# li199603/easy_gaussian_splatting

Measured on AMD Instinct MI355X. Metric: train iters/sec + forward render fps, 1M Gaussians @ 1080p, higher is better.
Workload: dtype f32

## Files before the change

easy_gaussian_splatting_amd/csrc/gs_binning.hip:

```cpp

#include "gs_common.h"

namespace gs {

#define GS_BIN_PER_GROUP 4096
#define GS_BIN_MAX_GROUPS 256
constexpr int kBinThreads = 1024;
constexpr int kCoopTiles = 32;

BinLayout bin_layout(int C, int64_t N, int tiles) {
    BinLayout L;
    int64_t g = (N + GS_BIN_PER_GROUP - 1) / GS_BIN_PER_GROUP;
    if (g < 1) g = 1;
    if (g > GS_BIN_MAX_GROUPS) g = GS_BIN_MAX_GROUPS;
    L.groups = (int)g;
    L.per_group = (N + g - 1) / g;
    auto align = [](size_t x) { return (x + 255) & ~(size_t)255; };
    size_t off = 0;
    L.hist_off = off; off = align(off + sizeof(uint32_t) * (size_t)C * L.groups * tiles);
    L.tile_cnt_off = off; off = align(off + sizeof(uint32_t) * (size_t)C * tiles);
    L.grp_tot_off = off; off = align(off + sizeof(uint32_t) * (size_t)C * L.groups);
    L.grp_base_off = off; off = align(off + sizeof(uint32_t) * (size_t)C * L.groups);
    L.items_off = off; off = align(off + sizeof(int32_t) * (64 + (size_t)10 * (size_t)C * tiles));
    L.total = off;
    return L;
}

__device__ __forceinline__ void unpack_bbox(uint4 b, int& x0, int& x1, int& y0, int& y1) {
    x0 = b.x & 0xffff; x1 = b.x >> 16; y0 = b.y & 0xffff; y1 = b.y >> 16;
}

__global__ __launch_bounds__(kBinThreads) void bin_hist_kernel(int64_t N, int tw, int tiles,
                                                               int64_t per_group,
                                                               const uint4* __restrict__ bbox,
                                                               uint32_t* __restrict__ hist_mat,
                                                               uint32_t* __restrict__ grp_tot, const int64_t* __restrict__ rblk, int phase) {
    extern __shared__ __attribute__((aligned(16))) uint32_t lds[];
    if (round_idle(rblk, phase)) return;
    uint32_t* hist = lds;
    uint32_t* scratch = lds + tiles;
    const int grp = blockIdx.x, c = blockIdx.y, G = gridDim.x;
    for (int t = threadIdx.x; t < tiles; t += blockDim.x) hist[t] = 0;
    __syncthreads();
    const int64_t g0 = grp * per_group, g1 = min(N, g0 + per_group);
    uint32_t local = 0;
    for (int64_t base = g0; base < g1; base += blockDim.x) {
        const int64_t n = base + threadIdx.x;
        int x0 = 0, x1 = 0, y0 = 0, y1 = 0;
        uint4 fp = make_uint4(0u, 0u, 0u, 0u);
        if (n < g1) { fp = bbox[(int64_t)c * N + n]; unpack_bbox(fp, x0, x1, y0, y1); }
        const int w = x1 - x0, rect = w * (y1 - y0), cnt = (int)fp.w;
        const float inv_w = 1.0f / (float)max(w, 1);
        local += cnt;
        if (rect <= kCoopTiles)
            for (uint32_t mb = fp.z; mb; mb &= mb - 1) {
                const int i = __ffs((int)mb) - 1, yy = div_by_width(i, inv_w);
                atomicAdd(&hist[(y0 + yy) * tw + x0 + (i - yy * w)], 1u);
            }
        unsigned long long big = __ballot(rect > kCoopTiles);
        while (big) {
            const int src = __ffsll((long long)big) - 1;
            big &= big - 1;
            const int bx0 = __shfl(x0, src, 64), by0 = __shfl(y0, src, 64), bw = __shfl(w, src, 64),
                      bcnt = __shfl(cnt, src, 64);
            const float binv = __shfl(inv_w, src, 64);
            for (int i = lane_id(); i < bcnt; i += 64) {
                const int yy = div_by_width(i, binv);
                atomicAdd(&hist[(by0 + yy) * tw + bx0 + (i - yy * bw)], 1u);
            }
        }
    }
    __syncthreads();
    uint32_t* out = hist_mat + ((size_t)c * G + grp) * tiles;
    for (int t = threadIdx.x; t < tiles; t += blockDim.x) out[t] = hist[t];
    uint32_t wsum = wave_reduce_add(local);
    if (lane_id() == 0) scratch[threadIdx.x >> 6] = wsum;
    __syncthreads();
    if (threadIdx.x == 0) {
        uint32_t s = 0;
        for (int i = 0; i < (int)(blockDim.x >> 6); ++i) s += scratch[i];
        grp_tot[c * G + grp] = s;
    }
}

constexpr int kColTiles = GS_BIN_MAX_GROUPS > 256 ? 32 : 64, kColChunks = GS_BIN_MAX_GROUPS > 256 ? 32 : 16;
__global__ __launch_bounds__(kColTiles * kColChunks) void bin_colscan_kernel(int C, int G, int tiles, uint32_t* __restrict__ hist_mat,
                                                                              uint32_t* __restrict__ tile_cnt) {
    __shared__ uint32_t part[kColChunks][kColTiles + 1];
    const int tl = threadIdx.x % kColTiles, ch = threadIdx.x / kColTiles;
    const int64_t i = (int64_t)blockIdx.x * kColTiles + tl;
    const bool in = i < (int64_t)C * tiles;
    const int c = in ? (int)(i / tiles) : 0, t = in ? (int)(i % tiles) : 0;
    const int per = (G + kColChunks - 1) / kColChunks;
    const int g0 = ch * per, g1 = min(G, g0 + per);
    uint32_t* col = hist_mat + (size_t)c * G * tiles + t;
    constexpr int kMax = 16;
    uint32_t v[kMax];
    uint32_t sum = 0;
#pragma unroll
    for (int k = 0; k < kMax; ++k) {
        v[k] = (in && g0 + k < g1) ? col[(size_t)(g0 + k) * tiles] : 0u;
        sum += v[k];
    }
    uint32_t extra = 0;
    for (int g = g0 + kMax; in && g < g1; ++g) extra += col[(size_t)g * tiles];
    part[ch][tl] = sum + extra;
    __syncthreads();
    uint32_t run = 0, total = 0;
#pragma unroll
    for (int k = 0; k < kColChunks; ++k) {
        const uint32_t p = part[k][tl];
        run += k < ch ? p : 0u;
        total += p;
    }
    if (in) {
#pragma unroll
        for (int k = 0; k < kMax; ++k) {
            if (g0 + k < g1) col[(size_t)(g0 + k) * tiles] = run;
            run += v[k];
        }
        for (int g = g0 + kMax; g < g1; ++g) { const uint32_t x = col[(size_t)g * tiles]; col[(size_t)g * tiles] = run; run += x; }
        if (ch == 0) tile_cnt[i] = total;
    }
}

constexpr int kScanItems = 16;
__global__ __launch_bounds__(kBinThreads) void bin_tilescan_kernel(
    int n_tiles_total, int n_groups_total, const uint32_t* __restrict__ tile_cnt,
    const uint32_t* __restrict__ grp_tot, int32_t* __restrict__ isect_offsets,
    int32_t* __restrict__ bucket_offsets, uint32_t* __restrict__ grp_base,
    int64_t* __restrict__ info, int32_t* __restrict__ tile_order, int64_t cap_isects, int64_t cap_tile,
    int64_t keep_mask, int32_t* __restrict__ sort_counts, int64_t* __restrict__ info_mirror, int per_call,
    int64_t* __restrict__ rblk, int phase) {
    __shared__ unsigned long long scratch[17];
    const int chunk = kBinThreads * kScanItems;
    if (round_idle(rblk, phase)) return;
    if (blockIdx.x == 2) {
        if (sort_counts && threadIdx.x < 64) sort_counts[threadIdx.x] = 0;
        unsigned long long gcarry = 0;
        for (int base = 0; base < n_groups_total; base += kBinThreads) {
            const int i = base + threadIdx.x;
            unsigned long long v = i < n_groups_total ? grp_tot[i] : 0ull, total;
            unsigned long long ex = block_excl_scan_add(v, scratch, &total);
            if (i < n_groups_total) grp_base[i] = (uint32_t)(gcarry + ex);
            gcarry += total;
        }
        return;
    }
    if (blockIdx.x == 1) {
        if (!tile_order) return;
        if (n_tiles_total > chunk) {
            for (int i = threadIdx.x; i < n_tiles_total; i += kBinThreads) tile_order[i] = i;
            return;
        }
        constexpr int kW = kBinThreads / 64;
        __shared__ uint32_t cls_cnt[64][kW + 1];
        auto cls_of = [](uint32_t x) -> int {
            if (x < 2u) return 0;
            const int lg = 31 - __clz((int)x);
            return min(63, (lg << 2) | (int)((x << (31 - lg)) >> 29 & 3u));
        };
        const int wv = threadIdx.x >> 6;
        const int first = threadIdx.x * kScanItems;
        uint32_t v[kScanItems];
#pragma unroll
        for (int k = 0; k < kScanItems; ++k) v[k] = (first + k < n_tiles_total) ? tile_cnt[first + k] : 0u;
        for (int i = threadIdx.x; i < 64 * (kW + 1); i += kBinThreads) (&cls_cnt[0][0])[i] = 0u;
        __syncthreads();
#pragma unroll
        for (int k = 0; k < kScanItems; ++k)
            if (first + k < n_tiles_total) atomicAdd(&cls_cnt[cls_of(v[k])][wv], 1u);
        __syncthreads();
        if (threadIdx.x < 64) {
            const int c = 63 - (int)threadIdx.x;
            uint32_t n = 0, cw[kW];
#pragma unroll
            for (int w = 0; w < kW; ++w) { cw[w] = cls_cnt[c][w]; n += cw[w]; }
            uint32_t run = wave_incl_scan_add(n) - n;
#pragma unroll
            for (int w = 0; w < kW; ++w) { cls_cnt[c][w] = run; run += cw[w]; }
        }
        __syncthreads();
#pragma unroll
        for (int k = 0; k < kScanItems; ++k)
            if (first + k < n_tiles_total) tile_order[atomicAdd(&cls_cnt[cls_of(v[k])][wv], 1u)] = first + k;
        return;
    }
    unsigned long long carry_i = phase == 2 ? (unsigned long long)rblk[GS_ROUND_BASE] : 0ull, carry_b = 0;
    uint32_t max_cnt = 0;
    for (int base = 0; base < n_tiles_total; base += chunk) {
        const int first = base + threadIdx.x * kScanItems;
        uint32_t v[kScanItems];
        unsigned long long si = 0, sb = 0;
#pragma unroll
        for (int k = 0; k < kScanItems; ++k) {
            v[k] = (first + k < n_tiles_total) ? tile_cnt[first + k] : 0u;
            si += v[k];
            sb += (v[k] + GS_BUCKET - 1) / GS_BUCKET;
            max_cnt = max(max_cnt, v[k]);
        }
        unsigned long long packed = si | (sb << 36), total;
        unsigned long long ex = block_excl_scan_add(packed, scratch, &total);
        unsigned long long ri = carry_i + (ex & ((1ull << 36) - 1)), rb = carry_b + (ex >> 36);
#pragma unroll
        for (int k = 0; k < kScanItems; ++k) {
            if (first + k < n_tiles_total) {
                isect_offsets[first + k] = (int32_t)ri;
                bucket_offsets[first + k] = (int32_t)rb;
            }
            ri += v[k];
            rb += (v[k] + GS_BUCKET - 1) / GS_BUCKET;
        }
        carry_i += total & ((1ull << 36) - 1);
        carry_b += total >> 36;
    }
    uint32_t m = max_cnt;
#pragma unroll
    for (int d = 32; d > 0; d >>= 1) m = max(m, (uint32_t)__shfl_xor((int)m, d, 64));
    __shared__ uint32_t smax[16];
    if (lane_id() == 0) smax[threadIdx.x >> 6] = m;
    __syncthreads();
    if (threadIdx.x == 0) {
        uint32_t mm = 0;
        for (int i = 0; i < kBinThreads / 64; ++i) mm = max(mm, smax[i]);
        isect_offsets[n_tiles_total] = (int32_t)carry_i;
        bucket_offsets[n_tiles_total] = (int32_t)carry_b;
        if (phase == 1) rblk[GS_ROUND_BASE] = (int64_t)carry_i;
        if (phase != 0) {
            info[7] = rblk[GS_ROUND_LISTED_ALL];
            info[6] = phase == 2 ? rblk[GS_ROUND_LIVE] : 0;
        }
        if (phase == 2) mm = max(mm, (uint32_t)info[2]);
        info[0] = (int64_t)carry_i; info[1] = (int64_t)carry_b; info[2] = (int64_t)mm;
        if (cap_isects > 0) {
            const int64_t f = ((int64_t)carry_i > cap_isects ? 1 : 0) | ((int64_t)mm > cap_tile ? 2 : 0);
            if (per_call && phase != 2) info[3] = (info[3] & keep_mask) | f;
            else if (f) info[3] |= f;
        } else {
            info[3] = keep_mask ? (info[3] & keep_mask) : 0;
        }
        if (info_mirror) {
#pragma unroll
            for (int i = 0; i < 8; ++i) info_mirror[i] = info[i];
            __threadfence_system();
        }
    }
}

__global__ __launch_bounds__(kBinThreads) void bin_emit_kernel(
    int64_t N, int tw, int tiles, int64_t per_group, const uint4* __restrict__ bbox,
    const float* __restrict__ depths, const uint32_t* __restrict__ hist_mat,
    const int32_t* __restrict__ isect_offsets, const uint32_t* __restrict__ grp_base,
    unsigned long long* __restrict__ keys, int32_t* __restrict__ slot_gid,
    int32_t* __restrict__ cum_tiles, const int64_t* __restrict__ guard, const int64_t* __restrict__ rblk, int phase) {
    extern __shared__ __attribute__((aligned(16))) uint32_t lds[];
    if (guard_tripped(guard) || round_idle(rblk, phase)) return;
    uint32_t* cursor = lds;
    uint32_t* scratch = lds + tiles;
    const int grp = blockIdx.x, c = blockIdx.y, G = gridDim.x;
    const uint32_t* mine = hist_mat + ((size_t)c * G + grp) * tiles;
    const int32_t* toff = isect_offsets + (size_t)c * tiles;
    for (int t0 = 0; t0 < tiles; t0 += 8 * (int)blockDim.x) {
        uint32_t v[8];
#pragma unroll
        for (int k = 0; k < 8; ++k) {
            const int t = t0 + k * (int)blockDim.x + (int)threadIdx.x;
            v[k] = t < tiles ? mine[t] + (uint32_t)toff[t] : 0u;
        }
#pragma unroll
        for (int k = 0; k < 8; ++k) {
            const int t = t0 + k * (int)blockDim.x + (int)threadIdx.x;
            if (t < tiles) cursor[t] = v[k];
        }
    }
    __syncthreads();
    uint32_t running = grp_base[c * G + grp] + (phase == 2 ? (uint32_t)rblk[GS_ROUND_BASE] : 0u);
    const int64_t g0 = grp * per_group, g1 = min(N, g0 + per_group);
    uint4 fp_next = make_uint4(0u, 0u, 0u, 0u);
    float d_next = 0.f;
    if (g0 + threadIdx.x < g1) { fp_next = bbox[(int64_t)c * N + g0 + threadIdx.x]; d_next = depths[(int64_t)c * N + g0 + threadIdx.x]; }
    for (int64_t base = g0; base < g1; base += blockDim.x) {
        const int64_t n = base + threadIdx.x;
        const int64_t f = (int64_t)c * N + n;
        int x0 = 0, x1 = 0, y0 = 0, y1 = 0;
        const uint4 fp = fp_next;
        const float dcur = d_next;
        if (n < g1) unpack_bbox(fp, x0, x1, y0, y1);
        const int w = x1 - x0, rect = w * (y1 - y0), cnt = (int)fp.w;
        const float inv_w = 1.0f / (float)max(w, 1);
        uint32_t total;
        const uint32_t slot0 = running + block_excl_scan_add((uint32_t)cnt, scratch, &total);
        running += total;
        fp_next = make_uint4(0u, 0u, 0u, 0u);
        if (n + blockDim.x < g1) { fp_next = bbox[f + blockDim.x]; d_next = depths[f + blockDim.x]; }
        if (n < g1 && (phase != 2 || cnt > 0)) cum_tiles[f] = (int32_t)slot0;
        const uint32_t dbits = cnt > 0 ? __float_as_uint(dcur) : 0u;
        if (rect <= kCoopTiles) {
            uint32_t k = 0;
            for (uint32_t mb = fp.z; mb; mb &= mb - 1, ++k) {
                const int i = __ffs((int)mb) - 1, yy = div_by_width(i, inv_w);
                const uint32_t pos = atomicAdd(&cursor[(y0 + yy) * tw + x0 + (i - yy * w)], 1u);
                keys[pos] = ((unsigned long long)dbits << 32) | (slot_gid ? slot0 + k : (uint32_t)f);
                if (slot_gid) slot_gid[slot0 + k] = (int32_t)f;
            }
        }
        unsigned long long big = __ballot(rect > kCoopTiles);
        while (big) {
            const int src = __ffsll((long long)big) - 1;
            big &= big - 1;
            const int bx0 = __shfl(x0, src, 64), by0 = __shfl(y0, src, 64), bw = __shfl(w, src, 64),
                      bcnt = __shfl(cnt, src, 64);
            const uint32_t bslot = __shfl((int)slot0, src, 64), bd = __shfl((int)dbits, src, 64);
            const int32_t bf = (int32_t)(c * N + base) + (src + (threadIdx.x & ~63));
            const float binv = __shfl(inv_w, src, 64);
            for (int i = lane_id(); i < bcnt; i += 64) {
                const int yy = div_by_width(i, binv);
                const uint32_t pos = atomicAdd(&cursor[(by0 + yy) * tw + bx0 + (i - yy * bw)], 1u);
                keys[pos] = ((unsigned long long)bd << 32) | (slot_gid ? bslot + i : (uint32_t)bf);
                if (slot_gid) slot_gid[bslot + i] = bf;
            }
        }
    }
}

template <typename KeyPtr>
__device__ __forceinline__ void bitonic_sort_keys(KeyPtr key, int n, int P) {
    for (int k = 2; k <= P; k <<= 1) {
        const int half = k >> 1;
        for (int idx = threadIdx.x; idx < (P >> 1); idx += blockDim.x) {
            const int blk = idx / half, off = idx - blk * half;
            const int a = blk * k + off, b = blk * k + k - 1 - off;
            if (b < n) {
                const unsigned long long ka = key[a], kb = key[b];
                if (ka > kb) { key[a] = kb; key[b] = ka; }
            }
        }
        __syncthreads();
        for (int j = half >> 1; j > 0; j >>= 1) {
            for (int idx = threadIdx.x; idx < (P >> 1); idx += blockDim.x) {
                const int a = ((idx & ~(j - 1)) << 1) | (idx & (j - 1)), b = a + j;
                if (b < n) {
                    const unsigned long long ka = key[a], kb = key[b];
                    if (ka > kb) { key[a] = kb; key[b] = ka; }
                }
            }
            __syncthreads();
        }
    }
}

struct SortArgs {
    int tiles, tile_bits, lo_excl, hi_incl;
    const int32_t* isect_offsets;
    unsigned long long* keys;
    const int32_t* slot_gid;
    int64_t* isect_ids;
    int32_t* flatten_ids;
    int32_t* slots;
    const int64_t* guard;
    int coarse;
    int seg;
    unsigned long long* merged;
    const int64_t* rblk;
    int phase;
};
__device__ __forceinline__ bool sort_off(const SortArgs& a) { return guard_tripped(a.guard) || round_idle(a.rblk, a.phase); }

constexpr int kSegLen = 8192;
constexpr int kSegMax = 8;

template <bool IN_LDS>
__global__ void tile_sort_kernel(const SortArgs a) {
    extern __shared__ __attribute__((aligned(16))) unsigned long long skeys[];
    const int t = blockIdx.x;
    if (sort_off(a)) return;
    const int lo = a.isect_offsets[t], hi = a.isect_offsets[t + 1];
    const int n = hi - lo;
    if (n <= a.lo_excl || n > a.hi_incl) return;
    int P = 1;
    while (P < n) P <<= 1;
    unsigned long long* gk = a.keys + lo;
    if (IN_LDS) {
        for (int i = threadIdx.x; i < n; i += blockDim.x) skeys[i] = gk[i];
        __syncthreads();
        bitonic_sort_keys(skeys, n, P);
    } else {
        bitonic_sort_keys(gk, n, P);
    }
    if (a.coarse) {
        if (IN_LDS) for (int i = threadIdx.x; i < n; i += blockDim.x) gk[i] = skeys[i];
        return;
    }
    const int cam = t / a.tiles, tid = t - cam * a.tiles;
    const long long hi_bits = ((long long)cam << (32 + a.tile_bits)) | ((long long)tid << 32);
    for (int i = threadIdx.x; i < n; i += blockDim.x) {
        const unsigned long long k = IN_LDS ? skeys[i] : gk[i];
        const uint32_t slot = (uint32_t)k;
        if (a.slot_gid) { a.slots[lo + i] = (int32_t)slot; a.flatten_ids[lo + i] = a.slot_gid[slot]; }
        else a.flatten_ids[lo + i] = (int32_t)slot;
        if (a.isect_ids) a.isect_ids[lo + i] = hi_bits | (long long)(k >> 32);
    }
}

template <int T>
__device__ __forceinline__ void radix_sort_list(const SortArgs& a, const int vblock) {
    extern __shared__ __attribute__((aligned(16))) unsigned long long skeys[];
    constexpr int W = T / 64;
    const int tile = a.seg ? vblock / kSegMax : vblock;
    int lo = a.isect_offsets[tile], n = a.isect_offsets[tile + 1] - lo;
    if (n <= a.lo_excl || n > a.hi_incl) return;
    if (a.seg) {
        const int sg = vblock - tile * kSegMax;
        lo += sg * kSegLen;
        n = min(kSegLen, n - sg * kSegLen);
        if (n <= 0) return;
    }
    const int cap = a.seg ? kSegLen : a.hi_incl;
    unsigned long long* src = skeys;
    unsigned long long* dst = skeys + cap;
    uint32_t* cnt = reinterpret_cast<uint32_t*>(skeys + 2 * cap);
    uint32_t* nxt = cnt + W * 256;
    __shared__ int s_flag;
    const int tid = threadIdx.x, lane = tid & 63, wave = tid >> 6;
    const unsigned long long* gk = a.keys + lo;
    const int per_wave = ((n + W * 64 - 1) / (W * 64)) * 64;
    const int w_lo = min(n, wave * per_wave), w_hi = min(n, w_lo + per_wave);
    const float inv_pw64 = 1.0f / (float)(per_wave >> 6);
    auto owner = [inv_pw64](int pos) { return (int)(((float)(pos >> 6) + 0.5f) * inv_pw64); };
    const unsigned long long lt_mask = (1ull << lane) - 1ull;
    for (int i = tid; i < 2 * W * 256; i += T) cnt[i] = 0u;
    __syncthreads();
    for (int i = tid; i < n; i += T) {
        const unsigned long long k = gk[i];
        src[i] = k;
        atomicAdd(&cnt[owner(i) * 256 + (int)((k >> 32) & 255ull)], 1u);
    }
    for (int pass = 0; pass < 4; ++pass) {
        const int shift = 32 + 8 * pass;
        __syncthreads();
        if (wave == 0) {
            uint32_t c[4][W], tot[4], mine = 0;
            bool all_in_one = false;
#pragma unroll
            for (int q = 0; q < 4; ++q) {
                tot[q] = 0;
#pragma unroll
                for (int w = 0; w < W; ++w) { c[q][w] = cnt[w * 256 + 4 * lane + q]; tot[q] += c[q][w]; }
                all_in_one |= (int)tot[q] == n;
                mine += tot[q];
            }
            uint32_t run = wave_incl_scan_add(mine) - mine;
#pragma unroll
            for (int q = 0; q < 4; ++q)
#pragma unroll
                for (int w = 0; w < W; ++w) { cnt[w * 256 + 4 * lane + q] = run; run += c[q][w]; }
            const bool skip = __any(all_in_one);
            if (lane == 0) s_flag = skip ? 1 : 0;
        } else {
            for (int i = tid - 64; i < W * 256; i += T - 64) nxt[i] = 0u;
        }
        __syncthreads();
        const bool skip = s_flag != 0;
        const int nshift = shift + 8;
        if (skip) {
            if (pass < 3)
                for (int i = w_lo + lane; i < w_hi; i += 64) atomicAdd(&nxt[wave * 256 + (int)((src[i] >> nshift) & 255ull)], 1u);
        } else {
            for (int base = w_lo; base < w_hi; base += 64) {
                const int i = base + lane;
                const bool valid = i < w_hi;
                const unsigned long long k = valid ? src[i] : 0ull;
                const int d = (int)((k >> shift) & 255ull);
                uint32_t mlo = 0u, mhi = 0u;
#pragma unroll
                for (int b = 0; b < 8; ++b) {
                    const int e = __builtin_amdgcn_sbfe(d, b, 1);
                    const unsigned long long bm = __ballot(e != 0);
                    mlo |= (uint32_t)bm ^ (uint32_t)e;
                    mhi |= (uint32_t)(bm >> 32) ^ (uint32_t)e;
                }
                const unsigned long long peers = __ballot(valid) & ~(((unsigned long long)mhi << 32) | (unsigned long long)mlo);
                if (valid) {
                    const int rank = __popcll(peers & lt_mask);
                    const uint32_t off = cnt[wave * 256 + d];
                    const uint32_t pos = off + (uint32_t)rank;
                    dst[pos] = k;
                    if (rank == 0) cnt[wave * 256 + d] = off + (uint32_t)__popcll(peers);
                    if (pass < 3) atomicAdd(&nxt[owner((int)pos) * 256 + (int)((k >> nshift) & 255ull)], 1u);
                }
            }
            unsigned long long* t = src; src = dst; dst = t;
        }
        uint32_t* tc = cnt; cnt = nxt; nxt = tc;
    }
    __syncthreads();
    if (tid == 0) s_flag = 0;
    __syncthreads();
    bool bad = false;
    for (int i = tid + 1; i < n; i += T) bad |= src[i] < src[i - 1];
    if (bad) s_flag = 1;
    __syncthreads();
    if (s_flag) {
        int P = 1;
        while (P < n) P <<= 1;
        bitonic_sort_keys(src, n, P);
    }
    if (a.coarse || a.seg) {
        unsigned long long* out = a.keys + lo;
        for (int i = tid; i < n; i += T) out[i] = src[i];
        return;
    }
    const int cam = tile / a.tiles, tix = tile - cam * a.tiles;
    const long long hi_bits = ((long long)cam << (32 + a.tile_bits)) | ((long long)tix << 32);
    for (int i = tid; i < n; i += T) {
        const unsigned long long k = src[i];
        const uint32_t slot = (uint32_t)k;
        if (a.slot_gid) { a.slots[lo + i] = (int32_t)slot; a.flatten_ids[lo + i] = a.slot_gid[slot]; }
        else a.flatten_ids[lo + i] = (int32_t)slot;
        if (a.isect_ids) a.isect_ids[lo + i] = hi_bits | (long long)(k >> 32);
    }
}

template <int T>
__global__ __launch_bounds__(T) void tile_radix_sort_kernel(const SortArgs a) {
    if (sort_off(a)) return;
    radix_sort_list<T>(a, blockIdx.x);
}

template <int T>
__global__ __launch_bounds__(T) void tile_radix_sort_items_kernel(const SortArgs a, const int32_t* __restrict__ items,
                                                                  const int32_t* __restrict__ n_items) {
    if (sort_off(a)) return;
    const int n = *n_items;
    for (int it = blockIdx.x; it < n; it += gridDim.x) {
        radix_sort_list<T>(a, items[it]);
        __syncthreads();
    }
}

__global__ __launch_bounds__(256) void class_items_kernel(int n_lists, const int32_t* __restrict__ offsets,
                                                          int32_t* __restrict__ items, int32_t* __restrict__ counts,
                                                          const int64_t* __restrict__ guard, const int64_t* __restrict__ rblk, int phase) {
    if (guard_tripped(guard) || round_idle(rblk, phase)) return;
    const int i = blockIdx.x * blockDim.x + threadIdx.x;
    if (i >= n_lists) return;
    const int n = offsets[i + 1] - offsets[i];
    if (n > 1024 && n <= 4096) items[atomicAdd(&counts[0], 1)] = i;
    else if (n > 4096 && n <= kSegLen) items[n_lists + atomicAdd(&counts[1], 1)] = i;
    else if (n > kSegLen && n <= kSegLen * kSegMax) {
        const int ns = (n + kSegLen - 1) / kSegLen;
        const int p = atomicAdd(&counts[2], ns);
        for (int sg = 0; sg < ns; ++sg) items[2 * n_lists + p + sg] = i * kSegMax + sg;
    }
}

static size_t sort_items_bytes(int64_t n_lists) {
    return sizeof(int32_t) * (64 + (size_t)(2 + kSegMax) * (size_t)n_lists);
}


struct BinsLayout {
    int groups, shift, bw, bh, nbins;
    int64_t per_group;
    size_t hist_off;
    size_t bin_cnt_off;
    size_t grp_tot_off;
    size_t grp_base_off;
    size_t coff_off;
    size_t choff_off;
    size_t tile_cnt_off;
    size_t chunk_bin_off;
    int chunk_shift;
    size_t rec_off;
    size_t staged_off;
    size_t cnt_ct_off;
    size_t items_off;
    int64_t max_chunks;
    size_t total;
};

static BinsLayout bins_layout(int C, int64_t N, int tw, int th, int bin_shift, int64_t coarse_cap) {
    BinsLayout L;
    int64_t g = (N + GS_BIN_PER_GROUP - 1) / GS_BIN_PER_GROUP;
    if (g < 1) g = 1;
    if (g > GS_BIN_MAX_GROUPS) g = GS_BIN_MAX_GROUPS;
    L.groups = (int)g;
    L.per_group = (N + g - 1) / g;
    const int64_t nb2 = (int64_t)((tw + 3) / 4) * ((th + 3) / 4);
    L.shift = bin_shift ? bin_shift : ((N / nb2 > 2500) ? 1 : 2);
    const int B = 1 << L.shift;
    L.bw = (tw + B - 1) / B; L.bh = (th + B - 1) / B; L.nbins = L.bw * L.bh;
    auto align = [](size_t x) { return (x + 255) & ~(size_t)255; };
    size_t off = 0;
    L.hist_off = off; off = align(off + sizeof(uint32_t) * (size_t)C * L.groups * L.nbins);
    L.bin_cnt_off = off; off = align(off + sizeof(uint32_t) * (size_t)C * L.nbins);
    L.grp_tot_off = off; off = align(off + sizeof(uint32_t) * (size_t)C * L.groups);
    L.grp_base_off = off; off = align(off + sizeof(uint32_t) * (size_t)C * L.groups);
    L.coff_off = off; off = align(off + sizeof(int32_t) * ((size_t)C * L.nbins + 1));
    L.choff_off = off; off = align(off + sizeof(int32_t) * ((size_t)C * L.nbins + 1));
    L.tile_cnt_off = off; off = align(off + sizeof(uint32_t) * (size_t)C * tw * th);
    L.chunk_shift = 10 + (L.shift - 1);
    L.max_chunks = (coarse_cap >> L.chunk_shift) + (int64_t)C * L.nbins;
    L.chunk_bin_off = off; off = align(off + sizeof(int4) * (size_t)L.max_chunks);
    L.rec_off = off; off = align(off + sizeof(uint4) * (size_t)C * (size_t)N);
    L.staged_off = off; off = align(off + sizeof(uint4) * (size_t)coarse_cap);
    L.cnt_ct_off = off; off = align(off + sizeof(uint32_t) * (size_t)L.max_chunks * B * B);
    L.items_off = off; off = align(off + sort_items_bytes((int64_t)C * L.nbins));
    L.total = off;
    return L;
}

__device__ __forceinline__ void coarse_rect(uint4 fp, int shift, int& cx0, int& cw, int& cy0, int& crect) {
    int x0, x1, y0, y1;
    unpack_bbox(fp, x0, x1, y0, y1);
    if (fp.w == 0u) { cx0 = cy0 = cw = crect = 0; return; }
    const int r = (1 << shift) - 1;
    cx0 = x0 >> shift; cy0 = y0 >> shift;
    cw = ((x1 + r) >> shift) - cx0;
    crect = cw * (((y1 + r) >> shift) - cy0);
}

__global__ __launch_bounds__(kBinThreads) void bins_hist_kernel(int64_t N, int shift, int bw, int nbins, int64_t per_group,
                                                                const uint4* __restrict__ bbox,
                                                                uint32_t* __restrict__ hist_mat,
                                                                uint32_t* __restrict__ grp_tot, const int64_t* __restrict__ rblk, int phase) {
    extern __shared__ __attribute__((aligned(16))) uint32_t lds[];
    if (round_idle(rblk, phase)) return;
    uint32_t* hist = lds;
    uint32_t* scratch = lds + nbins;
    const int grp = blockIdx.x, c = blockIdx.y, G = gridDim.x;
    for (int t = threadIdx.x; t < nbins; t += blockDim.x) hist[t] = 0;
    __syncthreads();
    const int64_t g0 = grp * per_group, g1 = min(N, g0 + per_group);
    uint32_t local = 0;
    for (int64_t base = g0; base < g1; base += blockDim.x) {
        const int64_t n = base + threadIdx.x;
        uint4 fp = make_uint4(0u, 0u, 0u, 0u);
        if (n < g1) fp = bbox[(int64_t)c * N + n];
        int cx0, cw, cy0, crect;
        coarse_rect(fp, shift, cx0, cw, cy0, crect);
        local += fp.w;
        if (crect <= kCoopTiles)
            for (int i = 0, xx = 0, row = cy0 * bw + cx0; i < crect; ++i) {
                atomicAdd(&hist[row + xx], 1u);
                if (++xx == cw) { xx = 0; row += bw; }
            }
        unsigned long long big = __ballot(crect > kCoopTiles);
        while (big) {
            const int src = __ffsll((long long)big) - 1;
            big &= big - 1;
            const int bx0 = __shfl(cx0, src, 64), by0 = __shfl(cy0, src, 64), bcw = __shfl(cw, src, 64), bcnt = __shfl(crect, src, 64);
            for (int i = lane_id(); i < bcnt; i += 64) {
                const int yy = i / bcw;
                atomicAdd(&hist[(by0 + yy) * bw + bx0 + (i - yy * bcw)], 1u);
            }
        }
    }
    __syncthreads();
    uint32_t* out = hist_mat + ((size_t)c * G + grp) * nbins;
    for (int t = threadIdx.x; t < nbins; t += blockDim.x) out[t] = hist[t];
    uint32_t wsum = wave_reduce_add(local);
    if (lane_id() == 0) scratch[threadIdx.x >> 6] = wsum;
    __syncthreads();
    if (threadIdx.x == 0) {
        uint32_t s = 0;
        for (int i = 0; i < (int)(blockDim.x >> 6); ++i) s += scratch[i];
        grp_tot[c * G + grp] = s;
    }
}

__global__ __launch_bounds__(256) void bins_colscan_kernel(int C, int G, int nbins, uint32_t* __restrict__ hist_mat,
                                                          uint32_t* __restrict__ bin_cnt) {
    const int64_t i = (int64_t)blockIdx.x * 4 + (threadIdx.x >> 6);
    if (i >= (int64_t)C * nbins) return;
    const int c = (int)(i / nbins), t = (int)(i % nbins), lane = lane_id();
    uint32_t* col = hist_mat + (size_t)c * G * nbins + t;
    uint32_t v[4];
#pragma unroll
    for (int k = 0; k < 4; ++k) { const int g = 64 * k + lane; v[k] = g < G ? col[(size_t)g * nbins] : 0u; }
    uint32_t carry = 0;
#pragma unroll
    for (int k = 0; k < 4; ++k) {
        const uint32_t incl = wave_incl_scan_add(v[k]);
        const int g = 64 * k + lane;
        if (g < G) col[(size_t)g * nbins] = carry + incl - v[k];
        carry += __shfl(incl, 63, 64);
    }
    if (lane == 0) bin_cnt[i] = carry;
}

__global__ __launch_bounds__(kBinThreads) void bins_scan_kernel(int n_bins_total, int n_groups_total,
                                                                const uint32_t* __restrict__ bin_cnt,
                                                                const uint32_t* __restrict__ grp_tot,
                                                                int32_t* __restrict__ coff, int32_t* __restrict__ choff,
                                                                int4* __restrict__ chunk_desc, int64_t max_chunks,
                                                                int chunk_shift, uint32_t* __restrict__ grp_base,
                                                                int64_t* __restrict__ info, int64_t coarse_cap, int64_t list_cap,
                                                                int guarded, int32_t* __restrict__ sort_counts,
                                                                const int64_t* __restrict__ rblk, int phase) {
    __shared__ unsigned long long scratch[17];
    __shared__ uint32_t smax[16];
    if (round_idle(rblk, phase)) return;
    if (blockIdx.x == 1) {
        if (threadIdx.x < 64) sort_counts[threadIdx.x] = 0;
        unsigned long long gcarry = 0;
        for (int base = 0; base < n_groups_total; base += kBinThreads) {
// ... 177 lines not shown
    }
    if (!WRITE) {
#pragma unroll
        for (int p = 0; p < PER; ++p) {
            const int e = p * T + (int)threadIdx.x;
            fp[p] = e < m ? a.rec[(uint32_t)key[p]] : make_uint4(0u, 0u, 0u, 0u);
        }
    }
#pragma unroll
    for (int p = 0; p < PER; ++p) {
        const int e = p * T + (int)threadIdx.x;
        if (e < m) {
            if (!WRITE) a.staged[base + e] = fp[p];
            if (WRITE) { s_cum[e] = fp[p].w; s_d[e] = (uint32_t)(key[p] >> 32); }
            fp[p].w = (uint32_t)key[p];
            s_box[e] = fp[p];
        }
    }
    __syncthreads();
    if (!tile_ok) return;
    const unsigned long long lt_mask = (1ull << lane) - 1ull;
    const long long hi_bits = ((long long)cam << (32 + a.tile_bits)) | ((long long)(ty * a.tw + tx) << 32);
    uint32_t count = 0;
    for (int j = 0; j < m; j += 64) {
        const int e = j + lane;
        bool hit = false;
        int k = 0;
        uint32_t f = 0;
        if (e < m) {
            const uint4 q = s_box[e];
            int x0, x1, y0, y1;
            unpack_bbox(q, x0, x1, y0, y1);
            f = q.w;
            if (tx >= x0 && tx < x1 && ty >= y0 && ty < y1) {
                const int w = x1 - x0, idx = (ty - y0) * w + (tx - x0);
                if (w * (y1 - y0) <= kCoopTiles) { hit = (q.z >> idx) & 1u; k = __popc(q.z & ((1u << idx) - 1u)); }
                else { hit = true; k = idx; }
            }
        }
        const unsigned long long bal = __ballot(hit);
        if (WRITE) {
            if (hit) {
                const int64_t pos = out + __popcll(bal & lt_mask);
                a.flatten_ids[pos] = (int32_t)f;
                if (a.isect_ids) a.isect_ids[pos] = hi_bits | (long long)s_d[e];
                if (a.slots) a.slots[pos] = (int32_t)(s_cum[e] + (uint32_t)k);
            }
            out += __popcll(bal);
        } else {
            count += (uint32_t)__popcll(bal);
        }
    }
    if (!WRITE && lane == 0) a.cnt_ct[(size_t)chunk * (B * B) + wave] = count;
}

template <int SHIFT>
__global__ __launch_bounds__(256) void bins_chunkscan_kernel(const RefineArgs a, int C) {
    constexpr int B = 1 << SHIFT;
    const int i = blockIdx.x * blockDim.x + threadIdx.x;
    if (i >= C * a.tiles) return;
    if (a.info[3] != 0 || round_idle(a.rblk, a.phase)) return;
    const int cam = i / a.tiles, t = i - cam * a.tiles;
    const int ty = t / a.tw, tx = t - ty * a.tw;
    const int bin = cam * a.nbins + (ty >> SHIFT) * a.bw + (tx >> SHIFT);
    const int w = ((ty & (B - 1)) << SHIFT) | (tx & (B - 1));
    const int c0 = a.choff[bin], c1 = a.choff[bin + 1];
    uint32_t run = 0;
    constexpr int kBatch = 8;
    for (int c = c0; c < c1; c += kBatch) {
        uint32_t v[kBatch];
#pragma unroll
        for (int k = 0; k < kBatch; ++k) v[k] = c + k < c1 ? a.cnt_ct[(size_t)(c + k) * (B * B) + w] : 0u;
#pragma unroll
        for (int k = 0; k < kBatch; ++k) {
            if (c + k < c1) a.cnt_ct[(size_t)(c + k) * (B * B) + w] = run;
            run += v[k];
        }
    }
    a.tile_cnt[i] = run;
}

__global__ __launch_bounds__(1024) void seg_merge_kernel(const SortArgs a, const int32_t* __restrict__ items,
                                                         const int32_t* __restrict__ n_items) {
    if (sort_off(a)) return;
    const int n_it = *n_items;
    for (int it = blockIdx.x; it < n_it; it += gridDim.x) {
    const int vblock = items[it];
    const int list = vblock / kSegMax, sg = vblock - list * kSegMax;
    const int lo = a.isect_offsets[list], n = a.isect_offsets[list + 1] - lo;
    const int s_lo = sg * kSegLen, s_n = min(kSegLen, n - s_lo);
    const int n_seg = (n + kSegLen - 1) / kSegLen;
    const unsigned long long* gk = a.keys + lo;
    const int cam = list / max(a.tiles, 1), tix = list - cam * a.tiles;
    const long long hi_bits = ((long long)cam << (32 + a.tile_bits)) | ((long long)tix << 32);
    for (int i = threadIdx.x; i < s_n; i += blockDim.x) {
        const unsigned long long k = gk[s_lo + i];
        int pos = i;
        for (int o = 0; o < n_seg; ++o) {
            if (o == sg) continue;
            const unsigned long long* seg = gk + o * kSegLen;
            int l = 0, r = min(kSegLen, n - o * kSegLen);
            while (l < r) {
                const int mid = (l + r) >> 1;
                if (seg[mid] < k) l = mid + 1; else r = mid;
            }
            pos += l;
        }
        if (a.coarse) {
            a.merged[lo + pos] = k;
        } else {
            const uint32_t slot = (uint32_t)k;
            if (a.slot_gid) { a.slots[lo + pos] = (int32_t)slot; a.flatten_ids[lo + pos] = a.slot_gid[slot]; }
            else a.flatten_ids[lo + pos] = (int32_t)slot;
            if (a.isect_ids) a.isect_ids[lo + pos] = hi_bits | (long long)(k >> 32);
        }
    }
    }
}

__global__ __launch_bounds__(1024) void seg_copy_kernel(const SortArgs a, const int32_t* __restrict__ items,
                                                        const int32_t* __restrict__ n_items) {
    if (sort_off(a)) return;
    const int n_it = *n_items;
    for (int it = blockIdx.x; it < n_it; it += gridDim.x) {
        const int vblock = items[it];
        const int list = vblock / kSegMax, sg = vblock - list * kSegMax;
        const int lo = a.isect_offsets[list], n = a.isect_offsets[list + 1] - lo;
        const int s_lo = sg * kSegLen, s_n = min(kSegLen, n - s_lo);
        for (int i = threadIdx.x; i < s_n; i += blockDim.x) a.keys[lo + s_lo + i] = a.merged[lo + s_lo + i];
    }
}

constexpr int kSortLarge = kSegLen * kSegMax;

}

using namespace gs;

extern "C" int gs_bin_groups(int64_t N) { return bin_layout(1, N, 1).groups; }

static int list_round(int64_t*& rblk) {
    const Rounds R = current_rounds();
    const int phase = (R.phase == 1 || R.phase == 4) ? 1 : (R.phase == 2 ? 2 : 0);
    rblk = phase ? R.blk : nullptr;
    return phase;
}

extern "C" size_t gs_bin_workspace_bytes(int C, int64_t N, int tile_w, int tile_h) {
    return bin_layout(C, N, tile_w * tile_h).total;
}

#define GS_SORT1K_THREADS 256
#define GS_SORT4K_THREADS 256
static int launch_list_sorts(hipStream_t st, SortArgs& a, unsigned grid, int64_t max_tile_count, int32_t* items_ws) {
    int lo_excl = 0;
    int32_t* counts = items_ws;
    int32_t* items = items_ws + 64;
    const size_t radix_lds = 2 * sizeof(uint32_t) * 256;
    a.lo_excl = 0; a.hi_incl = 1024;
    if (max_tile_count > 0) {
        const size_t lds_k = 2 * sizeof(uint64_t) * 1024 + radix_lds * (GS_SORT1K_THREADS / 64);
        hipLaunchKernelGGL(tile_radix_sort_kernel<GS_SORT1K_THREADS>, dim3(grid), dim3(GS_SORT1K_THREADS), lds_k, st, a);
        GS_LAUNCH_CHECK("tile_radix_sort_kernel");
    }
    if (max_tile_count <= 1024) return GS_OK;
    hipLaunchKernelGGL(class_items_kernel, dim3((grid + 255) / 256), dim3(256), 0, st, (int)grid, a.isect_offsets, items, counts, a.guard, a.rblk, a.phase);
    GS_LAUNCH_CHECK("class_items_kernel");
    {
        a.lo_excl = 1024; a.hi_incl = 4096;
        const size_t lds_k = 2 * sizeof(uint64_t) * 4096 + radix_lds * (GS_SORT4K_THREADS / 64);
        if (int rc = ensure_lds((const void*)tile_radix_sort_items_kernel<GS_SORT4K_THREADS>, lds_k)) return rc;
        hipLaunchKernelGGL(tile_radix_sort_items_kernel<GS_SORT4K_THREADS>, dim3(grid < 512u ? grid : 512u), dim3(GS_SORT4K_THREADS), lds_k, st, a,
                           (const int32_t*)items, (const int32_t*)counts);
        GS_LAUNCH_CHECK("tile_radix_sort_items_kernel<4096>");
    }
    if (max_tile_count > 4096) {
        a.lo_excl = 4096; a.hi_incl = kSegLen;
        const size_t lds_k = 2 * sizeof(uint64_t) * (size_t)kSegLen + radix_lds * (768 / 64);
        if (int rc = ensure_lds((const void*)tile_radix_sort_items_kernel<768>, lds_k)) return rc;
        hipLaunchKernelGGL(tile_radix_sort_items_kernel<768>, dim3(grid < 256u ? grid : 256u), dim3(768), lds_k, st, a,
                           (const int32_t*)(items + grid), (const int32_t*)(counts + 1));
        GS_LAUNCH_CHECK("tile_radix_sort_items_kernel<8192>");
    }
    if (max_tile_count > kSegLen) {
        a.lo_excl = kSegLen; a.hi_incl = kSortLarge; a.seg = 1;
        const size_t lds_k = 2 * sizeof(uint64_t) * (size_t)kSegLen + radix_lds * (768 / 64);
        if (int rc = ensure_lds((const void*)tile_radix_sort_items_kernel<768>, lds_k)) return rc;
        const int32_t* it = items + 2 * (size_t)grid;
        const int32_t* nit = counts + 2;
        hipLaunchKernelGGL(tile_radix_sort_items_kernel<768>, dim3(256), dim3(768), lds_k, st, a, it, nit);
        GS_LAUNCH_CHECK("tile_radix_sort_items_kernel<segments>");
        hipLaunchKernelGGL(seg_merge_kernel, dim3(512), dim3(1024), 0, st, a, it, nit);
        GS_LAUNCH_CHECK("seg_merge_kernel");
        if (a.coarse) {
            hipLaunchKernelGGL(seg_copy_kernel, dim3(512), dim3(1024), 0, st, a, it, nit);
            GS_LAUNCH_CHECK("seg_copy_kernel");
        }
        a.seg = 0;
    }
    if (max_tile_count > kSortLarge) {
        a.lo_excl = kSortLarge; a.hi_incl = 0x7fffffff;
        hipLaunchKernelGGL(tile_sort_kernel<false>, dim3(grid), dim3(1024), 0, st, a);
        GS_LAUNCH_CHECK("tile_sort_kernel<global>");
    }
    (void)lo_excl;
    return GS_OK;
}

extern "C" int gs_bin_count(void* stream, int C, int64_t N, int tile_w, int tile_h, const uint32_t* bbox,
                            void* workspace, size_t workspace_bytes, int32_t* isect_offsets,
                            int32_t* bucket_offsets, int32_t* tile_order, int64_t* info_dev, int64_t* info_host) {
    GS_REQUIRE(C >= 1 && N >= 0 && tile_w > 0 && tile_h > 0, "C>=1, N>=0, positive tile grid");
    const int tiles = tile_w * tile_h;
    GS_REQUIRE((size_t)tiles * 4 + 128 <= 160 * 1024, "tile grid too large for the LDS histogram (max 40928 tiles per camera)");
    GS_REQUIRE((int64_t)C * tiles < (1ll << 31), "too many tiles");
    const BinLayout L = bin_layout(C, N, tiles);
    GS_REQUIRE(workspace && workspace_bytes >= L.total, "workspace too small (see gs_bin_workspace_bytes)");
    GS_REQUIRE(isect_offsets && bucket_offsets && info_dev, "null output pointer");
    GS_REQUIRE(N == 0 || bbox, "null bbox");
    int64_t* rblk;
    const int phase = list_round(rblk);
    GS_REQUIRE(phase == 0 || C == 1, "depth rounds: one camera per call");
    hipStream_t st = (hipStream_t)stream;
    char* ws = (char*)workspace;
    uint32_t* hist = (uint32_t*)(ws + L.hist_off);
    uint32_t* tile_cnt = (uint32_t*)(ws + L.tile_cnt_off);
    uint32_t* grp_tot = (uint32_t*)(ws + L.grp_tot_off);
    uint32_t* grp_base = (uint32_t*)(ws + L.grp_base_off);
    const size_t lds = sizeof(uint32_t) * ((size_t)tiles + 32);
    if (int rc = ensure_lds((const void*)bin_hist_kernel, lds)) return rc;
    hipLaunchKernelGGL(bin_hist_kernel, dim3(L.groups, C), dim3(kBinThreads), lds, st, N, tile_w, tiles,
                       L.per_group, (const uint4*)bbox, hist, grp_tot, (const int64_t*)rblk, phase);
    GS_LAUNCH_CHECK("bin_hist_kernel");
    const int64_t ct = (int64_t)C * tiles;
    hipLaunchKernelGGL(bin_colscan_kernel, dim3((unsigned)((ct + kColTiles - 1) / kColTiles)), dim3(kColTiles * kColChunks), 0, st, C, L.groups,
                       tiles, hist, tile_cnt);
    GS_LAUNCH_CHECK("bin_colscan_kernel");
    const Guard gd = current_guard();
    GS_REQUIRE(gd.info == nullptr || gd.info == info_dev, "the guard set by gs_guard_set must be this call's info_dev");
    hipLaunchKernelGGL(bin_tilescan_kernel, dim3(3), dim3(kBinThreads), 0, st, (int)ct, C * L.groups, tile_cnt,
                       grp_tot, isect_offsets, bucket_offsets, grp_base, info_dev, tile_order, gd.cap_isects, gd.cap_tile,
                       (int64_t)0, (int32_t*)(ws + L.items_off), current_info_mirror(), gd.per_call, rblk, phase);
    GS_LAUNCH_CHECK("bin_tilescan_kernel");
    if (info_host) {
        GS_HIP_CHECK(hipMemcpyAsync(info_host, info_dev, 4 * sizeof(int64_t), hipMemcpyDeviceToHost, st));
        GS_HIP_CHECK(hipStreamSynchronize(st));
    }
    return GS_OK;
}

extern "C" int gs_bin_emit_sort(void* stream, int C, int64_t N, int tile_w, int tile_h, const uint32_t* bbox,
                                const float* depths, void* workspace, size_t workspace_bytes,
                                const int32_t* isect_offsets, int64_t n_isects, int64_t max_tile_count,
                                uint64_t* keys_tmp, int32_t* slot_gid, int32_t* cum_tiles,
                                int64_t* isect_ids, int32_t* flatten_ids, int32_t* slots) {
    GS_REQUIRE(C >= 1 && N >= 0 && tile_w > 0 && tile_h > 0, "C>=1, N>=0, positive tile grid");
    const int tiles = tile_w * tile_h;
    const BinLayout L = bin_layout(C, N, tiles);
    GS_REQUIRE(workspace && workspace_bytes >= L.total, "workspace too small (see gs_bin_workspace_bytes)");
    GS_REQUIRE(n_isects >= 0 && n_isects < (1ll << 31), "intersection count must fit int32");
    if (N == 0) return GS_OK;
    GS_REQUIRE(bbox && depths && isect_offsets && cum_tiles, "null pointer");
    GS_REQUIRE(n_isects == 0 || (keys_tmp && flatten_ids), "null intersection buffer");
    GS_REQUIRE((slot_gid == nullptr) == (slots == nullptr), "slot_gid and slots: both (training lists) or neither (inference lists)");
    int64_t* rblk;
    const int phase = list_round(rblk);
    GS_REQUIRE(phase == 0 || C == 1, "depth rounds: one camera per call");
    hipStream_t st = (hipStream_t)stream;
    char* ws = (char*)workspace;
    const uint32_t* hist = (const uint32_t*)(ws + L.hist_off);
    const uint32_t* grp_base = (const uint32_t*)(ws + L.grp_base_off);
    const size_t lds = sizeof(uint32_t) * ((size_t)tiles + 32);
    if (int rc = ensure_lds((const void*)bin_emit_kernel, lds)) return rc;
    hipLaunchKernelGGL(bin_emit_kernel, dim3(L.groups, C), dim3(kBinThreads), lds, st, N, tile_w, tiles,
                       L.per_group, (const uint4*)bbox, depths, hist, isect_offsets, grp_base,
                       (unsigned long long*)keys_tmp, slot_gid, cum_tiles, current_guard().info, (const int64_t*)rblk, phase);
    GS_LAUNCH_CHECK("bin_emit_kernel");
    if (n_isects == 0) return GS_OK;
    SortArgs a;
    a.tiles = tiles;
    int tb = 0;
    for (int v = tiles; v > 0; v >>= 1) ++tb;
    a.tile_bits = tb;
    a.isect_offsets = isect_offsets; a.keys = (unsigned long long*)keys_tmp; a.slot_gid = slot_gid;
    a.isect_ids = isect_ids; a.flatten_ids = flatten_ids; a.slots = slots;
    a.guard = current_guard().info;
    a.coarse = 0; a.seg = 0; a.merged = nullptr; a.rblk = rblk; a.phase = phase;
    static_assert(2 + kSegMax == 10, "bin_layout sizes the work lists for kSegMax == 8");
    return launch_list_sorts(st, a, (unsigned)(C * tiles), max_tile_count, (int32_t*)(ws + L.items_off));
}

extern "C" size_t gs_bins_workspace_bytes(int C, int64_t N, int tile_w, int tile_h, int bin_shift, int64_t coarse_cap) {
    if (bin_shift < 0 || bin_shift > 2 || coarse_cap < 0) return 0;
    return bins_layout(C, N, tile_w, tile_h, bin_shift, coarse_cap).total;
}

template <bool WRITE>
static int launch_refine(hipStream_t st, const BinsLayout& L, const RefineArgs& a) {
    const unsigned grid = (unsigned)L.max_chunks;
    if (L.shift == 2) hipLaunchKernelGGL((bins_refine_kernel<WRITE, 2>), dim3(grid), dim3(1024), 0, st, a);
    else hipLaunchKernelGGL((bins_refine_kernel<WRITE, 1>), dim3(grid), dim3(256), 0, st, a);
    GS_LAUNCH_CHECK("bins_refine_kernel");
    return GS_OK;
}

static void fill_refine_args(RefineArgs& r, const BinsLayout& L, int C, int tile_w, int tile_h, char* ws, const uint64_t* coarse_keys,
                             const uint32_t* bbox, const int64_t* info_dev) {
    r.tw = tile_w; r.th = tile_h; r.tiles = tile_w * tile_h; r.n_bins_total = C * L.nbins;
    r.choff = (const int32_t*)(ws + L.choff_off);
    r.chunk_desc = (const int4*)(ws + L.chunk_bin_off);
    r.cnt_ct = (uint32_t*)(ws + L.cnt_ct_off);
    int tb = 0;
    for (int v = r.tiles; v > 0; v >>= 1) ++tb;
    r.tile_bits = tb; r.bw = L.bw; r.nbins = L.nbins;
    r.coff = (const int32_t*)(ws + L.coff_off);
    r.keys = (const unsigned long long*)coarse_keys;
    r.rec = (const uint4*)(ws + L.rec_off);
    r.staged = (uint4*)(ws + L.staged_off);
    r.tile_cnt = (uint32_t*)(ws + L.tile_cnt_off);
    r.isect_offsets = nullptr; r.isect_ids = nullptr; r.flatten_ids = nullptr; r.slots = nullptr;
    r.info = info_dev;
    int64_t* rblk;
    r.phase = list_round(rblk);
    r.rblk = rblk;
}

extern "C" int gs_bins_count(void* stream, int C, int64_t N, int tile_w, int tile_h, int bin_shift, const uint32_t* bbox,
                             const float* depths, void* workspace, size_t workspace_bytes, uint64_t* coarse_keys,
                             int64_t coarse_cap, int64_t coarse_list_cap,
                             int32_t* cum_tiles, int32_t* isect_offsets, int32_t* bucket_offsets, int32_t* tile_order,
                             int64_t* info_dev, int64_t* info_host) {
    GS_REQUIRE(C >= 1 && N >= 0 && tile_w > 0 && tile_h > 0, "C>=1, N>=0, positive tile grid");
    const int tiles = tile_w * tile_h;
    GS_REQUIRE((int64_t)C * tiles < (1ll << 31) && (int64_t)C * N < (1ll << 31), "too many tiles or flatten ids");
    GS_REQUIRE(bin_shift >= 0 && bin_shift <= 2, "bin_shift: 0 (library default), 1 (2x2 tiles) or 2 (4x4 tiles)");
    GS_REQUIRE(coarse_cap >= 0 && coarse_cap < (1ll << 31) && (coarse_cap == 0 || coarse_keys), "coarse key buffer");
    const BinsLayout L = bins_layout(C, N, tile_w, tile_h, bin_shift, coarse_cap);
    GS_REQUIRE((size_t)L.nbins * 4 + 128 <= 160 * 1024, "tile grid too large for the LDS bin histogram");
    GS_REQUIRE(workspace && workspace_bytes >= L.total, "workspace too small (see gs_bins_workspace_bytes)");
    GS_REQUIRE(isect_offsets && bucket_offsets && info_dev, "null output pointer");
    GS_REQUIRE(N == 0 || (bbox && depths && cum_tiles), "null bbox / depths / cum_tiles");
    hipStream_t st = (hipStream_t)stream;
    char* ws = (char*)workspace;
    uint32_t* hist = (uint32_t*)(ws + L.hist_off);
    uint32_t* bin_cnt = (uint32_t*)(ws + L.bin_cnt_off);
    uint32_t* grp_tot = (uint32_t*)(ws + L.grp_tot_off);
    uint32_t* grp_base = (uint32_t*)(ws + L.grp_base_off);
    int32_t* coff = (int32_t*)(ws + L.coff_off);
    uint32_t* tile_cnt = (uint32_t*)(ws + L.tile_cnt_off);
    const Guard gd = current_guard();
    GS_REQUIRE(gd.info == nullptr || gd.info == info_dev, "the guard set by gs_guard_set must be this call's info_dev");
    int64_t* rblk;
    const int phase = list_round(rblk);
    GS_REQUIRE(phase == 0 || C == 1, "depth rounds: one camera per call");
    int64_t list_cap = 0x7fffffff;
    if (coarse_list_cap > 0) list_cap = coarse_list_cap <= 1024 ? 1024 : coarse_list_cap <= 4096 ? 4096 : coarse_list_cap <= kSegLen ? kSegLen
                                        : coarse_list_cap <= kSortLarge ? kSortLarge : 0x7fffffff;
    const size_t lds = sizeof(uint32_t) * ((size_t)L.nbins + 32);
    if (int rc = ensure_lds((const void*)bins_hist_kernel, lds)) return rc;
    hipLaunchKernelGGL(bins_hist_kernel, dim3(L.groups, C), dim3(kBinThreads), lds, st, N, L.shift, L.bw, L.nbins, L.per_group,
                       (const uint4*)bbox, hist, grp_tot, (const int64_t*)rblk, phase);
    GS_LAUNCH_CHECK("bins_hist_kernel");
    const int64_t cb = (int64_t)C * L.nbins;
    hipLaunchKernelGGL(bins_colscan_kernel, dim3((unsigned)((cb + 3) / 4)), dim3(256), 0, st, C, L.groups, L.nbins, hist, bin_cnt);
    GS_LAUNCH_CHECK("bins_colscan_kernel");
    hipLaunchKernelGGL(bins_scan_kernel, dim3(2), dim3(kBinThreads), 0, st, (int)cb, C * L.groups, bin_cnt, grp_tot, coff,
                       (int32_t*)(ws + L.choff_off), (int4*)(ws + L.chunk_bin_off), L.max_chunks, L.chunk_shift, grp_base,
                       info_dev, coarse_cap, list_cap,
                       (gd.info != nullptr && !gd.per_call) ? 1 : 0, (int32_t*)(ws + L.items_off), (const int64_t*)rblk, phase);
    GS_LAUNCH_CHECK("bins_scan_kernel");
    if (N > 0) {
        if (int rc = ensure_lds((const void*)bins_emit_kernel, lds)) return rc;
        hipLaunchKernelGGL(bins_emit_kernel, dim3(L.groups, C), dim3(kBinThreads), lds, st, N, L.shift, L.bw, L.nbins, L.per_group,
                           (const uint4*)bbox, depths, hist, coff, grp_base, (unsigned long long*)coarse_keys, cum_tiles,
                           (uint4*)(ws + L.rec_off), (const int64_t*)info_dev, (const int64_t*)rblk, phase);
        GS_LAUNCH_CHECK("bins_emit_kernel");
        SortArgs a;
        a.tiles = L.nbins; a.tile_bits = 0;
        a.isect_offsets = coff; a.keys = (unsigned long long*)coarse_keys; a.slot_gid = nullptr;
        a.isect_ids = nullptr; a.flatten_ids = nullptr; a.slots = nullptr;
        a.guard = info_dev; a.coarse = 1; a.seg = 0; a.rblk = rblk; a.phase = phase;
        a.merged = (unsigned long long*)(ws + L.staged_off);
        if (int rc = launch_list_sorts(st, a, (unsigned)cb, list_cap < coarse_cap ? list_cap : coarse_cap, (int32_t*)(ws + L.items_off))) return rc;
    }
    RefineArgs r;
    fill_refine_args(r, L, C, tile_w, tile_h, ws, coarse_keys, bbox, info_dev);
    if (int rc = launch_refine<false>(st, L, r)) return rc;
    {
        const unsigned g = (unsigned)(((int64_t)C * tiles + 255) / 256);
        if (L.shift == 2) hipLaunchKernelGGL(bins_chunkscan_kernel<2>, dim3(g), dim3(256), 0, st, r, C);
        else hipLaunchKernelGGL(bins_chunkscan_kernel<1>, dim3(g), dim3(256), 0, st, r, C);
        GS_LAUNCH_CHECK("bins_chunkscan_kernel");
    }
    hipLaunchKernelGGL(bin_tilescan_kernel, dim3(2), dim3(kBinThreads), 0, st, C * tiles, 0, tile_cnt, (const uint32_t*)nullptr,
                       isect_offsets, bucket_offsets, (uint32_t*)nullptr, info_dev, tile_order, gd.cap_isects,
                       (int64_t)0x7fffffffffffffffll, (int64_t)12, (int32_t*)nullptr, current_info_mirror(), gd.per_call, rblk, phase);
    GS_LAUNCH_CHECK("bin_tilescan_kernel");
    if (info_host) {
        GS_HIP_CHECK(hipMemcpyAsync(info_host, info_dev, 8 * sizeof(int64_t), hipMemcpyDeviceToHost, st));
        GS_HIP_CHECK(hipStreamSynchronize(st));
    }
    return GS_OK;
}

extern "C" int gs_bins_lists(void* stream, int C, int64_t N, int tile_w, int tile_h, int bin_shift, const uint32_t* bbox, void* workspace,
                             size_t workspace_bytes, const uint64_t* coarse_keys, int64_t coarse_cap, const int32_t* cum_tiles,
                             const int32_t* isect_offsets, int64_t* isect_ids, int32_t* flatten_ids, int32_t* slots,
                             const int64_t* info_dev) {
    GS_REQUIRE(C >= 1 && N >= 0 && tile_w > 0 && tile_h > 0, "C>=1, N>=0, positive tile grid");
    GS_REQUIRE(bin_shift >= 0 && bin_shift <= 2 && coarse_cap >= 0, "bin_shift: 0, 1 or 2; coarse_cap as given to gs_bins_count");
    const BinsLayout L = bins_layout(C, N, tile_w, tile_h, bin_shift, coarse_cap);
    GS_REQUIRE(workspace && workspace_bytes >= L.total, "workspace too small (see gs_bins_workspace_bytes)");
    GS_REQUIRE(info_dev && isect_offsets, "null pointer");
    if (N == 0) return GS_OK;
    GS_REQUIRE(cum_tiles && bbox && flatten_ids, "null list buffer");
    RefineArgs r;
    fill_refine_args(r, L, C, tile_w, tile_h, (char*)workspace, coarse_keys, bbox, info_dev);
    r.isect_offsets = isect_offsets; r.isect_ids = isect_ids; r.flatten_ids = flatten_ids; r.slots = slots;
    return launch_refine<true>((hipStream_t)stream, L, r);
}
```

easy_gaussian_splatting_amd/csrc/gs_blend.hip:

```cpp
#include <algorithm>

#include "gs_common.h"
#include "gs_math.h"

namespace gs {

#ifdef GS_BWD_CHECK
struct BwdCheck {
    float* fwd_T;
    int32_t* fwd_cnt;
    float2* unit_out;
    int2* unit_hdr;
};
static BwdCheck g_bwd_check = {nullptr, nullptr, nullptr, nullptr};
#define GS_IF_CHECK(...) __VA_ARGS__
#else
#define GS_IF_CHECK(...)
#endif

constexpr int kUnit = GS_UNIT;
constexpr int kChunk = 8;
constexpr int kUnitLog = 128;
constexpr int kWalkUnits = GS_WALK_UNITS, kWalkStorage = GS_WALK_STORAGE, kWalkRows = GS_WALK_ROWS,
              kWalkFlags = GS_WALK_FLAGS, kWalkSkip = GS_WALK_SKIP;
// ... 113 lines not shown
        const int64_t tail0 = head + (n16 << 4);
        if (tail0 + (int64_t)threadIdx.x < n) q[tail0 + threadIdx.x] = 0;
    }
}

template <bool CKPT, int WAVES, int ROUND, int NC>
__device__ __forceinline__ void blend_fwd_body(const BlendFwdArgs& a, float* __restrict__ ckpt_ext) {
    static_assert(NC >= 1 && NC <= 4 && (NC == 3 || ROUND == 0), "channels 1..4; depth rounds with 3 channels only");
    __shared__ float4 srec_all[WAVES][GS_BUCKET * 3];
    __shared__ int2 ulog_all[CKPT ? WAVES : 1][CKPT ? kUnitLog : 1];
    __shared__ int uring_all[CKPT ? WAVES : 1][CKPT ? 16 : 1];
    float4* srec = srec_all[threadIdx.x >> 6];
    int2* ulog = ulog_all[CKPT ? (threadIdx.x >> 6) : 0];
    int* uring = uring_all[CKPT ? (threadIdx.x >> 6) : 0];
    const int ti = CKPT ? __builtin_amdgcn_readfirstlane((int)blockIdx.x * WAVES + (int)(threadIdx.x >> 6))
                        : (int)blockIdx.x * WAVES + (int)(threadIdx.x >> 6);
    if (ti >= a.C * a.tiles) return;
    if (CKPT ? a.walk[kWalkSkip] != 0 : guard_tripped(a.guard)) return;
    if (ROUND == 2 && a.rblk[GS_ROUND_LIVE] == 0) return;
    GS_CLOCK_PROBE_SCOPE(0);
    const int t = a.tile_order ? a.tile_order[ti] : ti;
    const int cam = t / a.tiles, tt = t - cam * a.tiles;
    const int tyi = tt / a.tw, txi = tt - tyi * a.tw;
    const int lane = threadIdx.x & 63;
    const int x0 = txi * GS_TILE, y0 = tyi * GS_TILE;
    const int px0 = x0 + (lane & 7), py0 = y0 + (lane >> 3);
    const float fx0 = (float)px0 + 0.5f, fy0 = (float)py0 + 0.5f, fx1 = fx0 + 8.f, fy1 = fy0 + 8.f;
    const int lo = a.isect_offsets[t], hi = a.isect_offsets[t + 1];
    const int len = hi - lo;
    const int nb = (len + GS_BUCKET - 1) / GS_BUCKET;
    const unsigned long long lt_mask = (1ull << lane) - 1ull;
    if (ROUND == 2 && (len == 0 || a.live[t] == 0)) return;

    float T[4], cr[4], cg[4], cb[4];
    float ca[4];
    int cnt[4] = {0, 0, 0, 0};
    int pool_next = 0, pool_left = 0, log_n = 0;
    int room[4] = {0, 0, 0, 0};
    const int range_len = (a.cap_units / GS_WALK_RANGES) & ~(kChunk - 1), range0 = (ti & (GS_WALK_RANGES - 1)) * range_len;
    int32_t* range_ctr = a.walk + GS_WALK_RANGE0 + 32 * (ti & (GS_WALK_RANGES - 1));
    GS_IF_CHECK(int taken[4] = {0, 0, 0, 0};)
#pragma unroll
    for (int k = 0; k < 4; ++k) {
        cr[k] = cg[k] = cb[k] = 0.f;
        ca[k] = 0.f;
        T[k] = ((px0 + 8 * (k & 1)) < a.W && (py0 + 8 * (k >> 1)) < a.H) ? 1.f : kDoneScale;
    }
    if (ROUND == 2) {
#pragma unroll
        for (int k = 0; k < 4; ++k) {
            const float4 s4 = a.tstate[((size_t)t * 4 + k) * 64 + lane];
            T[k] = s4.x; cr[k] = s4.y; cg[k] = s4.z; cb[k] = s4.w;
        }
        if (CKPT) {
            const int4 rc = a.trec[2 * (size_t)t], ru = a.trec[2 * (size_t)t + 1];
            cnt[0] = __builtin_amdgcn_readfirstlane(rc.x); cnt[1] = __builtin_amdgcn_readfirstlane(rc.y);
            cnt[2] = __builtin_amdgcn_readfirstlane(rc.z); cnt[3] = __builtin_amdgcn_readfirstlane(rc.w);
            const int ru4[4] = {ru.x, ru.y, ru.z, ru.w};
#pragma unroll
            for (int k = 0; k < 4; ++k) {
                room[k] = -cnt[k] & (kUnit - 1);
                if (lane == 0 && cnt[k] > 0) uring[4 * k + (((cnt[k] - 1) / kUnit) & 3)] = ru4[k];
            }
        }
    }
    const float qxlo[2] = {(float)x0 + 0.5f, (float)x0 + 8.5f}, qxhi[2] = {(float)x0 + 7.5f, (float)x0 + 15.5f};
    const float qylo[2] = {(float)y0 + 0.5f, (float)y0 + 8.5f}, qyhi[2] = {(float)y0 + 7.5f, (float)y0 + 15.5f};

    auto publish = [&]() {
        if (log_n == 0) return;
        int base = 0;
        if (lane == 0) base = atomicAdd(a.walk + kWalkUnits, log_n);
        base = __builtin_amdgcn_readfirstlane(base);
        __builtin_amdgcn_wave_barrier();
        for (int j = lane; j < log_n; j += 64) {
            const int2 e = ulog[j];
            if (base + j < a.cap_units) a.unit_desc[base + j] = make_int4(4 * t + (e.y & 3), e.y >> 2, e.x, 0);
        }
        __builtin_amdgcn_wave_barrier();
        log_n = 0;
    };

    for (int b = 0; b < nb; ++b) {
        bool qa[4];
#pragma unroll
        for (int k = 0; k < 4; ++k) qa[k] = __builtin_amdgcn_ballot_w64(px_live(T[k])) != 0ull;
        if (!(qa[0] || qa[1] || qa[2] || qa[3])) break;
        if (CKPT && log_n > kUnitLog - 8) publish();
        const int first = lo + b * GS_BUCKET;
        const int m = min(GS_BUCKET, hi - first);
        bool hx[2] = {false, false}, hy[2] = {false, false};
        int my_gid = 0, my_slot = 0;
        if (lane < m) {
            my_gid = a.flatten_ids[first + lane];
            if (CKPT) my_slot = a.slots[first + lane];
            const float4* r = a.rec + 3 * (size_t)my_gid;
            const float4 q0 = r[0], q1 = r[1], q2 = r[2];
            srec[lane * 3] = q0; srec[lane * 3 + 1] = q1; srec[lane * 3 + 2] = q2;
            const float ex = q1.z, ey = q1.w;
#pragma unroll
            for (int h = 0; h < 2; ++h) {
                hx[h] = ex >= 0.f && q0.x + ex >= qxlo[h] && q0.x - ex <= qxhi[h];
                hy[h] = ey >= 0.f && q0.y + ey >= qylo[h] && q0.y - ey <= qyhi[h];
            }
        }
        bool bit[4] = {qa[0] && hx[0] && hy[0], qa[1] && hx[1] && hy[0], qa[2] && hx[0] && hy[1], qa[3] && hx[1] && hy[1]};
        if (bit[0] || bit[1] || bit[2] || bit[3]) {
            const float4 q0 = srec[lane * 3], q1 = srec[lane * 3 + 1];
            const float tau = __log2f(255.f * q1.y) + 0.02f;
#pragma unroll
            for (int k = 0; k < 4; ++k) {
                if (bit[k]) {
                    const float ms = quad_min_on_rect(q0.z, q0.w, q1.x, qxlo[k & 1] - q0.x, qxhi[k & 1] - q0.x,
                                                      qylo[k >> 1] - q0.y, qyhi[k >> 1] - q0.y);
                    bit[k] = ms <= tau + 1e-4f * fabsf(tau);
                }
            }
        }
        unsigned long long mq[4], cq[4] = {0ull, 0ull, 0ull, 0ull};
#pragma unroll
        for (int k = 0; k < 4; ++k) mq[k] = __ballot(bit[k]);
        __builtin_amdgcn_wave_barrier();
        for (unsigned long long rem = mq[0] | mq[1] | mq[2] | mq[3]; rem; rem &= rem - 1) {
            const int j = __builtin_ctzll(rem);
            const float4 q0 = srec[j * 3], q1 = srec[j * 3 + 1], q2 = srec[j * 3 + 2];
            const float op = q1.y, r = q2.x, g = q2.y, bl = q2.z;
#pragma unroll
            for (int k = 0; k < 4; ++k) {
                if ((mq[k] >> j) & 1) {
                    const float dx = q0.x - ((k & 1) ? fx1 : fx0), dy = q0.y - ((k >> 1) ? fy1 : fy0);
                    const float sigma = fmaf(dy, fmaf(q1.x, dy, q0.w * dx), q0.z * dx * dx);
                    const float alpha = fminf(kAlphaMax, op * fast_exp2(-sigma));
                    const bool ok = px_live(T[k]) && sigma >= 0.f && alpha >= kAlphaMin;
                    const float am = ok ? alpha : 0.f;
                    if (CKPT) {
                        if (__builtin_amdgcn_ballot_w64(ok) != 0ull) {
                            if (__builtin_expect(room[k] == 0, 0)) {
                                const int pos = cnt[k] + (int)__popcll(cq[k]);
                                if (pool_left == 0) {
                                    int base = 0;
                                    if (lane == 0) base = atomicAdd(range_ctr, kChunk);
                                    base = __builtin_amdgcn_readfirstlane(base);
                                    if (base + kChunk > range_len) {
                                        if (lane == 0) {
                                            atomicOr(a.walk + kWalkFlags, GS_FLAG_UNITS);
                                            if (ROUND != 1 && a.flags) atomicOr(a.flags, (unsigned long long)GS_FLAG_UNITS);
                                        }
                                        base = 0;
                                    }
                                    pool_next = range0 + base; pool_left = kChunk;
                                }
                                const int su = pool_next++;
                                --pool_left;
                                a.ckpt[(size_t)su * 64 + lane] = make_float4(px_live(T[k]) ? T[k] : -1.f, cr[k], cg[k], cb[k]);
                                if constexpr (NC == 4) ckpt_ext[(size_t)su * 64 + lane] = ca[k];
                                if (lane == 0) ulog[log_n] = make_int2(su, (pos / kUnit) * 4 + k);
                                ++log_n;
                                if (lane == 0) uring[4 * k + ((pos / kUnit) & 3)] = su;
                                room[k] = kUnit;
                            }
                            --room[k];
                            cq[k] |= 1ull << j;
                        }
                    }
                    GS_IF_CHECK(const float T_before = T[k];)
                    if constexpr (NC == 4) blend_masked4(am, r, g, bl, q2.w, T[k], cr[k], cg[k], cb[k], ca[k]);
                    else blend_masked(am, r, g, bl, T[k], cr[k], cg[k], cb[k]);
                    GS_IF_CHECK(taken[k] += T[k] < T_before ? 1 : 0;)
                }
            }
        }
        if (CKPT) {
            int mybits = 0;
#pragma unroll
            for (int k = 0; k < 4; ++k) {
                const int n_new = (int)__popcll(cq[k]);
                if ((cq[k] >> lane) & 1) {
                    const int p = cnt[k] + (int)__popcll(cq[k] & lt_mask);
                    const int su = uring[4 * k + ((p / kUnit) & 3)];
                    a.qlist[(size_t)su * kUnit + (p & (kUnit - 1))] = make_int2(my_gid, my_slot);
                    mybits |= 1 << k;
                }
                cnt[k] += n_new;
            }
            if (mybits) a.qmask[my_slot] = (uint8_t)mybits;
        }
        __builtin_amdgcn_wave_barrier();
    }
    if (CKPT) {
        if (lane < 4) a.qcnt[4 * t + lane] = lane == 0 ? cnt[0] : (lane == 1 ? cnt[1] : (lane == 2 ? cnt[2] : cnt[3]));
        publish();
    }
    if (ROUND == 1) {
        const bool lv = __builtin_amdgcn_ballot_w64(px_live(T[0]) || px_live(T[1]) || px_live(T[2]) || px_live(T[3])) != 0ull;
        if (lane == 0) {
            a.live[t] = lv ? 1 : 0;
            if (lv) atomicAdd(reinterpret_cast<unsigned long long*>(a.rblk + GS_ROUND_LIVE), 1ull);
            if (lv && a.solo && a.flags) atomicOr(a.flags, (unsigned long long)GS_FLAG_BACK);
        }
        if (lv && !a.solo) {
#pragma unroll
            for (int k = 0; k < 4; ++k) a.tstate[((size_t)t * 4 + k) * 64 + lane] = make_float4(T[k], cr[k], cg[k], cb[k]);
            if (CKPT && lane == 0) {
                a.trec[2 * (size_t)t] = make_int4(cnt[0], cnt[1], cnt[2], cnt[3]);
                int ru[4];
#pragma unroll
                for (int k = 0; k < 4; ++k) ru[k] = cnt[k] > 0 ? uring[4 * k + (((cnt[k] - 1) / kUnit) & 3)] : 0;
                a.trec[2 * (size_t)t + 1] = make_int4(ru[0], ru[1], ru[2], ru[3]);
            }
        }
    }
    float bgr = 0.f, bgg = 0.f, bgb = 0.f, bga = 0.f;
    if (a.bg) {
        bgr = a.bg[NC * cam];
        if (NC > 1) bgg = a.bg[NC * cam + 1];
        if (NC > 2) bgb = a.bg[NC * cam + 2];
        if (NC > 3) bga = a.bg[NC * cam + 3];
    }
#pragma unroll
    for (int k = 0; k < 4; ++k) {
        const int px = px0 + 8 * (k & 1), py = py0 + 8 * (k >> 1);
        if (px < a.W && py < a.H) {
            const size_t o = ((size_t)cam * a.H + py) * a.W + px;
            const float Tf = px_final_T(T[k]);
            a.out_colors[NC * o] = cr[k] + Tf * bgr;
            if (NC > 1) a.out_colors[NC * o + 1] = cg[k] + Tf * bgg;
            if (NC > 2) a.out_colors[NC * o + 2] = cb[k] + Tf * bgb;
            if (NC > 3) a.out_colors[NC * o + 3] = ca[k] + Tf * bga;
            a.out_alphas[o] = 1.f - Tf;
            GS_IF_CHECK(if (CKPT && a.chk.fwd_T) { a.chk.fwd_T[o] = Tf; a.chk.fwd_cnt[o] = taken[k]; })
        }
    }
}

template <bool CKPT, int WAVES, int ROUND>
__global__ __launch_bounds__(64 * WAVES) GS_FWD_ATTR void blend_fwd_kernel(const BlendFwdArgs a) {
    blend_fwd_body<CKPT, WAVES, ROUND, 3>(a, nullptr);
}
template <bool CKPT, int WAVES, int NC>
__global__ __launch_bounds__(64 * WAVES) __attribute__((amdgpu_waves_per_eu(CKPT ? (NC == 4 ? 4 : 5) : 1, 8))) void chan_fwd_kernel(const BlendFwdArgs a, float* ckpt_ext) {
    blend_fwd_body<CKPT, WAVES, 0, NC>(a, ckpt_ext);
}

struct RowScanArgs {
    const uint8_t* qmask;
    int32_t* row_base;
    int32_t* walk;
    int64_t n_cap, cap_rows;
    unsigned long long* flags;
    const int64_t* guard;
    volatile int64_t* mirror;
};

__device__ __forceinline__ int32_t row_counts32(const uint8_t* __restrict__ qmask, int64_t i0, int64_t n, uint32_t (&w)[8]) {
#pragma unroll
    for (int j = 0; j < 8; ++j) w[j] = 0u;
    if (i0 + kScanPerThread <= n) {
        const uint4 x = reinterpret_cast<const uint4*>(qmask + i0)[0], y = reinterpret_cast<const uint4*>(qmask + i0)[1];
        w[0] = x.x; w[1] = x.y; w[2] = x.z; w[3] = x.w; w[4] = y.x; w[5] = y.y; w[6] = y.z; w[7] = y.w;
    } else {
        for (int j = 0; j < kScanPerThread; ++j)
            if (i0 + j < n) w[j >> 2] |= (uint32_t)qmask[i0 + j] << (8 * (j & 3));
    }
    int32_t tot = 0;
#pragma unroll
    for (int j = 0; j < 8; ++j) {
        uint32_t v = w[j] & 0x0f0f0f0fu;
        v = v - ((v >> 1) & 0x55555555u);
        v = (v & 0x33333333u) + ((v >> 2) & 0x33333333u);
        w[j] = v;
        tot += (int32_t)((v * 0x01010101u) >> 24);
    }
    return tot;
}

__global__ __launch_bounds__(kScanThreads) void row_count_kernel(const RowScanArgs a) {
    __shared__ int32_t scratch[20];
    if (a.walk[kWalkSkip] != 0) return;
    const int64_t n = slots_in_use(a.n_cap, a.guard);
    const int64_t c0 = (int64_t)blockIdx.x * kScanChunk;
    if (c0 > n) return;
    uint32_t w[8];
    const int32_t tot = row_counts32(a.qmask, c0 + (int64_t)threadIdx.x * kScanPerThread, n, w);
    int32_t block_tot;
    block_excl_scan_add<int32_t>(tot, scratch, &block_tot);
    if (threadIdx.x == 0) a.walk[GS_WALK_WORDS + blockIdx.x] = block_tot;
}

__global__ __launch_bounds__(1024) void row_chunk_scan_kernel(const RowScanArgs a) {
    __shared__ int32_t scratch[20];
    if (a.walk[kWalkSkip] != 0) return;
    const int64_t n = slots_in_use(a.n_cap, a.guard);
    const int nb = (int)(n / kScanChunk) + 1;
    int32_t* part = a.walk + GS_WALK_WORDS;
    const int per = (nb + 1023) / 1024;
    const int j0 = (int)threadIdx.x * per, j1 = min(nb, j0 + per);
    int32_t mine = 0;
    for (int j = j0; j < j1; ++j) mine += part[j];
    int32_t total;
    int32_t run = block_excl_scan_add<int32_t>(mine, scratch, &total);
    for (int j = j0; j < j1; ++j) { const int32_t c = part[j]; part[j] = run; run += c; }
    if (threadIdx.x == 0) {
        int32_t fullest = 0;
        for (int r = 0; r < GS_WALK_RANGES; ++r) fullest = max(fullest, a.walk[GS_WALK_RANGE0 + 32 * r]);
        a.walk[kWalkStorage] = GS_WALK_RANGES * fullest;
        a.walk[kWalkRows] = total;
        int fl = a.walk[kWalkFlags];
        if (a.flags && (fl & GS_FLAG_UNITS)) atomicOr(a.flags, (unsigned long long)GS_FLAG_UNITS);
        if ((int64_t)total > a.cap_rows) {
            fl |= GS_FLAG_ROWS;
            a.walk[kWalkFlags] = fl;
            if (a.flags) atomicOr(a.flags, (unsigned long long)GS_FLAG_ROWS);
        }
        if (a.mirror) {
            a.mirror[0] = a.walk[kWalkUnits]; a.mirror[1] = a.walk[kWalkStorage]; a.mirror[2] = total; a.mirror[3] = fl;
            __threadfence_system();
        }
    }
}

__global__ __launch_bounds__(kScanThreads) void row_base_kernel(const RowScanArgs a) {
    __shared__ int32_t scratch[20];
    if (a.walk[kWalkSkip] != 0) return;
    const int64_t n = slots_in_use(a.n_cap, a.guard);
    const int64_t c0 = (int64_t)blockIdx.x * kScanChunk;
    if (c0 > n) return;
    const int64_t i0 = c0 + (int64_t)threadIdx.x * kScanPerThread;
    uint32_t w[8];
    const int32_t tot = row_counts32(a.qmask, i0, n, w);
    int32_t block_tot;
    const int32_t run = block_excl_scan_add<int32_t>(tot, scratch, &block_tot) + a.walk[GS_WALK_WORDS + blockIdx.x];
    int32_t first16 = 0;
#pragma unroll
    for (int j = 0; j < 4; ++j) first16 += (int32_t)((w[j] * 0x01010101u) >> 24);
    if (i0 <= n) a.row_base[i0 >> 4] = run;
    if (i0 + 16 <= n) a.row_base[(i0 >> 4) + 1] = run + first16;
}

struct BlendBwdArgs {
    int C, W, H, tw, tiles;
    const float4* rec;
    const int32_t* walk;
    const int2* qlist;
    const int32_t* qcnt;
    const int4* unit_desc;
    const float4* ckpt;
    const uint8_t* qmask;
    const int32_t* row_base;
    int cap_units;
    const int32_t* cls_hdr;
    const int4* cls_desc;
    int cls_cap;
    const float *out_colors, *out_alphas, *v_colors, *v_alphas;
    float4* rows;
    const int64_t* guard;
    GS_IF_CHECK(BwdCheck chk;)
};

constexpr int kBwdWaves = 4;
constexpr int kPipeLanes = 8;
constexpr int kPerLane = kUnit / kPipeLanes;
static_assert(kPerLane == 4, "bwd_wave is instantiated for 1 .. 4 entries per lane");
constexpr int kUnitsPerWave = 64 / kPipeLanes;
constexpr int kUnitPixels = 64;
constexpr int kBwdSteps = kUnitPixels + kPipeLanes - 1;

__device__ __forceinline__ float dpp_row_shr1(float v) {
    return __builtin_bit_cast(float, __builtin_amdgcn_update_dpp(__builtin_bit_cast(int, v), __builtin_bit_cast(int, v), 0x111, 0xf, 0xf, false));
}


#ifdef GS_BWD_ACC64
typedef double acc_t;
#define GS_ACC_FMA(a, b, c) ((double)(a) * (double)(b) + (c))
#else
typedef float acc_t;
#define GS_ACC_FMA(a, b, c) fmaf((a), (b), (c))
#endif
struct EntryState {
    float mx, my, hA, Bc, hC, op, colr, colg, colb, At, Bt, Ct;
    acc_t s_mx, s_my, s_ax, s_ay, s_A, s_B, s_C, s_vs, s_r, s_g, s_b;
    bool has;
    float col3; acc_t s_3;
};

template <int NC>
__device__ __forceinline__ void bwd_pair(EntryState& e, const float4 d0, const float v3, const float2 d1, float& T, float& P) {
    const float dx = e.mx - d1.x, dy = e.my - d1.y;
    const float sigma = fmaf(dy, fmaf(e.hC, dy, e.Bc * dx), e.hA * dx * dx);
    const float vis = fast_exp2(-sigma);
    const float ov = e.op * vis;
    const float alpha = fminf(kAlphaMax, ov);
    const bool ok = T > 0.f && sigma >= 0.f && alpha >= kAlphaMin;
    const float w = alpha * T;
    const float Tn = fmaf(-alpha, T, T);
    const bool stop = ok && Tn <= kTMin;
    const bool contrib = ok && !stop;
    float cv = e.colr * d0.x + e.colg * d0.y + e.colb * d0.z;
    if constexpr (NC == 4) cv = fmaf(e.col3, v3, cv);
    const float wm = contrib ? w : 0.f;
    const float Pn = fmaf(wm, cv, P);
    const float ra = fast_rcp(1.f - alpha);
    const float v_alpha = fmaf(T, cv, ra * (d0.w + Pn));
    e.s_r = GS_ACC_FMA(wm, d0.x, e.s_r); e.s_g = GS_ACC_FMA(wm, d0.y, e.s_g); e.s_b = GS_ACC_FMA(wm, d0.z, e.s_b);
    if constexpr (NC == 4) e.s_3 = GS_ACC_FMA(wm, v3, e.s_3);
    const float vs = (contrib && ov <= kAlphaMax) ? -ov * v_alpha : 0.f;
    const float hx = vs * dx, hy = vs * dy;
    e.s_A = GS_ACC_FMA(hx, dx, e.s_A); e.s_B = GS_ACC_FMA(hx, dy, e.s_B); e.s_C = GS_ACC_FMA(hy, dy, e.s_C);
    const float gx = fmaf(e.At, hx, e.Bt * hy), gy = fmaf(e.Bt, hx, e.Ct * hy);
    e.s_mx += (acc_t)gx; e.s_my += (acc_t)gy; e.s_ax += (acc_t)fabsf(gx); e.s_ay += (acc_t)fabsf(gy);
    e.s_vs += (acc_t)vs;
    T = contrib ? Tn : (stop ? -1.f : T);
    P = Pn;
}

template <int E, int NC>
__device__ __forceinline__ void bwd_wave(const BlendBwdArgs& a, const int4 ud, const bool valid, const int unit, float4* sd0, float* sd1,
                                         float2* sck, const int r, const float* __restrict__ ckpt_ext) {
    const int tq = ud.x, su = ud.z;
    const bool first_unit = ud.y == 0;
    const int t = tq >> 2, q = tq & 3;
    const int cam = t / a.tiles, tt = t - cam * a.tiles;
    const int tyi = tt / a.tw, txi = tt - tyi * a.tw;
    const int qx0 = txi * GS_TILE + 8 * (q & 1), qy0 = tyi * GS_TILE + 8 * (q >> 1);
    const float fx0 = (float)qx0 + 0.5f, fy0 = (float)qy0 + 0.5f;
    const float4* ckp = a.ckpt + (size_t)su * 64;

    const int n_sub = valid ? a.qcnt[tq] : 0;
    int2 gs[E];
    {
        const int2* qp2 = a.qlist + (size_t)su * kUnit + E * r;
        if constexpr (E == 4) {
            const int4* qp = reinterpret_cast<const int4*>(qp2);
            const int4 g0 = qp[0], g1 = qp[1];
            gs[0] = make_int2(g0.x, g0.y); gs[1] = make_int2(g0.z, g0.w); gs[2] = make_int2(g1.x, g1.y); gs[3] = make_int2(g1.z, g1.w);
        } else if constexpr (E == 2) {
            const int4 g0 = *reinterpret_cast<const int4*>(qp2);
            gs[0] = make_int2(g0.x, g0.y); gs[1] = make_int2(g0.z, g0.w);
        } else {
#pragma unroll
            for (int i = 0; i < E; ++i) gs[i] = qp2[i];
        }
    }
    constexpr int kPix = kUnitPixels / kPipeLanes;
    float l_vr[kPix], l_vg[kPix], l_vb[kPix], l_oa[kPix], l_cr[kPix], l_cg[kPix], l_cb[kPix], l_va[kPix];
    float l_v3[kPix], l_c3[kPix], l_k3[kPix];
    float4 l_ck[kPix];
    const float* vap = a.v_alphas ? a.v_alphas : a.out_alphas;
#pragma unroll
    for (int i = 0; i < kPix; ++i) {
        const int p = r + kPipeLanes * i;
        const int px = min(qx0 + (p & 7), a.W - 1), py = min(qy0 + (p >> 3), a.H - 1);
        const size_t o = ((size_t)cam * a.H + py) * a.W + px;
        l_vr[i] = a.v_colors[NC * o];
        l_vg[i] = NC > 1 ? a.v_colors[NC * o + 1] : 0.f;
        l_vb[i] = NC > 2 ? a.v_colors[NC * o + 2] : 0.f;
        l_oa[i] = a.out_alphas[o];
        l_cr[i] = a.out_colors[NC * o];
        l_cg[i] = NC > 1 ? a.out_colors[NC * o + 1] : 0.f;
        l_cb[i] = NC > 2 ? a.out_colors[NC * o + 2] : 0.f;
        l_va[i] = vap[o];
        l_ck[i] = ckp[p];
        if constexpr (NC == 4) { l_v3[i] = a.v_colors[NC * o + 3]; l_c3[i] = a.out_colors[NC * o + 3]; l_k3[i] = ckpt_ext[(size_t)su * 64 + p]; }
    }
    const int n_in = min(kPipeLanes * E, n_sub - ud.y * kUnit);
    float4 rq[E][3];
#pragma unroll
    for (int i = 0; i < E; ++i) {
        const bool has = E * r + i < n_in;
        const float4* rp = a.rec + 3 * (size_t)(has ? gs[i].x : 0);
        rq[i][0] = rp[0]; rq[i][1] = rp[1]; rq[i][2] = rp[2];
    }
#pragma unroll
    for (int i = 0; i < kPix; ++i) {
        const int p = r + kPipeLanes * i;
        const bool inside = valid && (qx0 + (p & 7)) < a.W && (qy0 + (p >> 3)) < a.H;
        const float vr = l_vr[i], vg = l_vg[i], vb = l_vb[i];
        const float Tf = 1.f - l_oa[i];
        const float va = a.v_alphas ? l_va[i] : 0.f;
        float Ev = Tf * va - (l_cr[i] * vr + l_cg[i] * vg + l_cb[i] * vb);
        const float4 ck = first_unit ? make_float4(1.f, 0.f, 0.f, 0.f) : l_ck[i];
        float Pk = ck.y * vr + ck.z * vg + ck.w * vb;
        if constexpr (NC == 4) {
            const float v3 = l_v3[i];
            Ev = Tf * va - fmaf(l_c3[i], v3, l_cr[i] * vr + l_cg[i] * vg + l_cb[i] * vb);
            Pk = fmaf(first_unit ? 0.f : l_k3[i], v3, Pk);
            sd1[p] = inside ? v3 : 0.f;
        }
        sd0[p] = inside ? make_float4(vr, vg, vb, Ev) : make_float4(0.f, 0.f, 0.f, 0.f);
        sck[p] = inside ? make_float2(ck.x, Pk) : make_float2(-1.f, 0.f);
    }

    EntryState e[E];
    int slot[E];
#pragma unroll
    for (int i = 0; i < E; ++i) {
        const int en = E * r + i;
        e[i].has = en < n_in;
        slot[i] = e[i].has ? gs[i].y : 0;
        const float4 z4 = make_float4(0.f, 0.f, 0.f, 0.f);
        const float4 q0 = e[i].has ? rq[i][0] : z4, q1 = e[i].has ? rq[i][1] : z4, q2 = e[i].has ? rq[i][2] : z4;
        e[i].mx = q0.x; e[i].my = q0.y; e[i].hA = q0.z; e[i].Bc = q0.w; e[i].hC = q1.x; e[i].op = q1.y;
        e[i].colr = q2.x; e[i].colg = q2.y; e[i].colb = q2.z;
        e[i].col3 = q2.w; e[i].s_3 = (acc_t)0;
        e[i].At = 2.f * kLn2 * q0.z; e[i].Bt = kLn2 * q0.w; e[i].Ct = 2.f * kLn2 * q1.x;
        e[i].s_mx = e[i].s_my = e[i].s_ax = e[i].s_ay = e[i].s_A = e[i].s_B = e[i].s_C = e[i].s_vs = (acc_t)0;
        e[i].s_r = e[i].s_g = e[i].s_b = (acc_t)0;
    }
    __builtin_amdgcn_wave_barrier();

    float T_out = -1.f, P_out = 0.f;
    GS_IF_CHECK(float D_out = -1.f, C_out = 0.f; if (valid && r == 0 && a.chk.unit_hdr) a.chk.unit_hdr[unit] = make_int2(tq, ud.y);)
    for (int s = 0; s < kBwdSteps; ++s) {
        float T = dpp_row_shr1(T_out), P = dpp_row_shr1(P_out);
        const int p = s - r;
        const bool act = (unsigned)p < (unsigned)kUnitPixels;
        const int pc = min(max(p, 0), kUnitPixels - 1);
        const float4 d0 = sd0[pc];
        const float v3 = NC == 4 ? sd1[pc] : 0.f;
        const float2 ck = sck[pc];
        const float2 d1 = make_float2(fx0 + (float)(pc & 7), fy0 + (float)(pc >> 3));
        if (r == 0) { T = ck.x; P = ck.y; }
        T = act ? T : -1.f;
        GS_IF_CHECK(float D = dpp_row_shr1(D_out), Cn = dpp_row_shr1(C_out); if (r == 0) { D = ck.x; Cn = 0.f; } if (!act) { D = -1.f; Cn = 0.f; })
#pragma unroll
        for (int i = 0; i < E; ++i) {
            GS_IF_CHECK(const float T_before = T;)
            bwd_pair<NC>(e[i], d0, v3, d1, T, P);
            GS_IF_CHECK(if (T > 0.f && T < T_before) { D = T; Cn += 1.f; })
        }
        GS_IF_CHECK(D_out = D; C_out = Cn;
                    if (valid && act && r == kPipeLanes - 1 && a.chk.unit_out) a.chk.unit_out[(size_t)unit * 64 + p] = make_float2(D, Cn);)
        T_out = T; P_out = P;
    }

    int row[E];
#pragma unroll
    for (int i = 0; i < E; ++i) {
        int m;
        row[i] = rows_before(a.row_base, a.qmask, slot[i], &m);
        row[i] += __popc((unsigned)m & ((1u << q) - 1u));
    }
#pragma unroll
    for (int i = 0; i < E; ++i) {
        if (e[i].has) {
            float4* rp = a.rows + (GS_ROW_FLOATS / 4) * (size_t)row[i];
            const float v_op = e[i].op > 0.f ? (float)(-e[i].s_vs / (acc_t)e[i].op) : 0.f;
            rp[0] = make_float4((float)e[i].s_mx, (float)e[i].s_my, (float)e[i].s_ax, (float)e[i].s_ay);
            rp[1] = make_float4((float)((acc_t)0.5f * e[i].s_A), (float)e[i].s_B, (float)((acc_t)0.5f * e[i].s_C), v_op);
            rp[2] = make_float4((float)e[i].s_r, (float)e[i].s_g, (float)e[i].s_b, NC == 4 ? (float)e[i].s_3 : 0.f);
        }
    }
}

constexpr int kClsHdrInts = 16, kClsThreads = 1024;
__global__ __launch_bounds__(64) void unit_classes_clear_kernel(int32_t* __restrict__ hdr) {
    if (threadIdx.x < kClsHdrInts) hdr[threadIdx.x] = 0;
}
__global__ __launch_bounds__(kClsThreads) void unit_classes_kernel(const int32_t* __restrict__ walk, const int4* __restrict__ unit_desc,
                                                                   const int32_t* __restrict__ qcnt, int cap_units, int cls_cap,
                                                                   int32_t* __restrict__ hdr, int4* __restrict__ cls, const int64_t* __restrict__ guard) {
    __shared__ int s_cnt[kClsThreads / 64][4], s_base[kClsThreads / 64][4];
    if (guard_tripped(guard)) return;
    const int n_units = min(walk[kWalkUnits], cap_units);
    if ((int)blockIdx.x * kClsThreads >= n_units) return;
    const int u = (int)blockIdx.x * kClsThreads + (int)threadIdx.x, wave = threadIdx.x >> 6, lane = threadIdx.x & 63;
    int c = 0;
    int4 ud = make_int4(0, 0, 0, 0);
    if (u < n_units) {
        ud = unit_desc[u];
        const int n_in = min(kUnit, qcnt[ud.x] - ud.y * kUnit);
        c = min(max((n_in + kPipeLanes - 1) / kPipeLanes, 1), 4);
        ud.w = u;
    }
    unsigned long long m[4];
#pragma unroll
    for (int k = 0; k < 4; ++k) m[k] = __ballot(c == k + 1);
    if (lane < 4) s_cnt[wave][lane] = (int)__popcll(lane == 0 ? m[0] : (lane == 1 ? m[1] : (lane == 2 ? m[2] : m[3])));
    __syncthreads();
    if (threadIdx.x < 4) {
        int tot = 0;
        for (int w = 0; w < kClsThreads / 64; ++w) { s_base[w][threadIdx.x] = tot; tot += s_cnt[w][threadIdx.x]; }
        const int base = tot ? atomicAdd(hdr + 1 + threadIdx.x, tot) : 0;
        for (int w = 0; w < kClsThreads / 64; ++w) s_base[w][threadIdx.x] += base;
    }
    __syncthreads();
    if (c) {
        const unsigned long long mine = c == 1 ? m[0] : (c == 2 ? m[1] : (c == 3 ? m[2] : m[3]));
        const int i = s_base[wave][c - 1] + (int)__popcll(mine & ((1ull << lane) - 1ull));
        if (i < (c == 4 ? cap_units : cls_cap)) cls[(c == 4 ? 0 : cap_units + (3 - c) * cls_cap) + i] = ud;
    }
}

template <int NC>
__device__ __forceinline__ void blend_bwd_body(const BlendBwdArgs& a, const float* __restrict__ ckpt_ext) {
    __shared__ float4 sd0_all[kBwdWaves][kUnitsPerWave][64];
    __shared__ float2 sck_all[kBwdWaves][kUnitsPerWave][64];
    const int wave = threadIdx.x >> 6, lane = threadIdx.x & 63;
    const int pipe = lane / kPipeLanes, r = lane & (kPipeLanes - 1);
    if (guard_tripped(a.guard)) return;
    constexpr int kPerBlock = kBwdWaves * kUnitsPerWave;
    int cls = 4, blk = (int)blockIdx.x, n_units, first = 0;
    if (a.cls_hdr == nullptr) {
        n_units = min(a.walk[kWalkUnits], a.cap_units);
    } else {
        const int b4 = (a.cap_units + kPerBlock - 1) / kPerBlock, bt = (a.cls_cap + kPerBlock - 1) / kPerBlock;
        if (blk >= b4) {
            const int k = (blk - b4) / bt;
            cls = 3 - k; blk -= b4 + k * bt; first = a.cap_units + k * a.cls_cap;
        }
        n_units = min(a.cls_hdr[cls], cls == 4 ? a.cap_units : a.cls_cap);
    }
    const int in_class = (blk * kBwdWaves + wave) * kUnitsPerWave + pipe;
    if ((blk * kBwdWaves + wave) * kUnitsPerWave >= n_units) return;
    GS_CLOCK_PROBE_SCOPE(2);
    const bool valid = in_class < n_units;
    float4* sd0 = sd0_all[wave][pipe];
    float2* sck = sck_all[wave][pipe];
    float* sd1 = nullptr;
    if constexpr (NC == 4) {
        __shared__ float sd1_all[kBwdWaves][kUnitsPerWave][64];
        sd1 = sd1_all[wave][pipe];
    }

    int4 ud = make_int4(0, 0, 0, 0);
    if (valid) ud = a.cls_hdr ? a.cls_desc[first + in_class] : a.unit_desc[in_class];
    const int unit = a.cls_hdr ? ud.w : in_class;
    if (cls == 4) bwd_wave<4, NC>(a, ud, valid, unit, sd0, sd1, sck, r, ckpt_ext);
    else if (cls == 3) bwd_wave<3, NC>(a, ud, valid, unit, sd0, sd1, sck, r, ckpt_ext);
    else if (cls == 2) bwd_wave<2, NC>(a, ud, valid, unit, sd0, sd1, sck, r, ckpt_ext);
    else bwd_wave<1, NC>(a, ud, valid, unit, sd0, sd1, sck, r, ckpt_ext);
}

__global__ __launch_bounds__(kBwdWaves * 64) void blend_bwd_kernel(const BlendBwdArgs a) {
    blend_bwd_body<3>(a, nullptr);
}
template <int NC>
__global__ __launch_bounds__(kBwdWaves * 64) void chan_bwd_kernel(const BlendBwdArgs a, const float* ckpt_ext) {
    blend_bwd_body<NC>(a, ckpt_ext);
}

}

using namespace gs;

#ifdef GS_BWD_CHECK
extern "C" int gs_debug_bwd_check_set(float* fwd_T, int32_t* fwd_cnt, float* unit_out, int32_t* unit_hdr) {
    g_bwd_check.fwd_T = fwd_T; g_bwd_check.fwd_cnt = fwd_cnt;
    g_bwd_check.unit_out = reinterpret_cast<float2*>(unit_out); g_bwd_check.unit_hdr = reinterpret_cast<int2*>(unit_hdr);
    return GS_OK;
}
#endif

#ifdef GS_CLOCK_PROBE
extern "C" int gs_debug_clock_probe(int64_t* out4, int reset) {
    unsigned long long h[4] = {0, 0, 0, 0};
    if (out4) { GS_HIP_CHECK(hipMemcpyFromSymbol(h, HIP_SYMBOL(gs_clk_acc), sizeof(h))); for (int i = 0; i < 4; ++i) out4[i] = (int64_t)h[i]; }
    if (reset) { unsigned long long z[4] = {0, 0, 0, 0}; GS_HIP_CHECK(hipMemcpyToSymbol(HIP_SYMBOL(gs_clk_acc), z, sizeof(z))); }
    return GS_OK;
}
#endif

extern "C" size_t gs_walk_state_ints(int64_t n_isects) {
    if (n_isects < 0) return 0;
    return (size_t)GS_WALK_WORDS + (size_t)(n_isects / kScanChunk + 1);
}

template <int NC>
static int blend_fwd_launch(void* stream, int C, int width, int height, const float* rec,
                            const float* backgrounds, const int32_t* isect_offsets, const int32_t* tile_order,
                            const int32_t* flatten_ids, const int32_t* slots, int64_t n_isects, float* render_colors,
                            float* render_alphas, float* ckpt, int32_t* qlist, int32_t* qcnt, uint8_t* qmask,
                            int32_t* unit_desc, int64_t cap_units, int32_t* row_base, int64_t cap_rows, int32_t* walk_state,
                            float* ckpt_ext) {
    GS_REQUIRE(C >= 1 && width > 0 && height > 0 && n_isects >= 0, "C>=1, positive image size, n_isects>=0");
    GS_REQUIRE(isect_offsets && render_colors && render_alphas, "null pointer");
    const bool train = ckpt != nullptr;
    GS_REQUIRE(!train || (qlist && qcnt && qmask && unit_desc && row_base && walk_state && slots), "training mode needs every list output");
    GS_REQUIRE(!train || (cap_units >= kChunk * GS_WALK_RANGES && cap_units < (1ll << 26) && cap_rows >= 0 && cap_rows < (1ll << 31)),
               "training mode: 256 <= cap_units < 2^26 work units, cap_rows < 2^31 gradient rows");
    GS_REQUIRE(!train || n_isects < (1ll << 31) - kScanChunk, "training mode: the slots of a call are indexed by int32");
    static_assert(kScanPerThread == 32, "row_base_kernel writes two groups of 16 slots per thread");
    GS_REQUIRE(!train || (((uintptr_t)qmask & 15) == 0 && ((uintptr_t)row_base & 15) == 0 && ((uintptr_t)walk_state & 7) == 0),
               "training mode: qmask / row_base 16-byte aligned, walk_state 8-byte aligned");
    BlendFwdArgs a;
    a.C = C; a.W = width; a.H = height;
    a.tw = (width + GS_TILE - 1) / GS_TILE;
    a.tiles = a.tw * ((height + GS_TILE - 1) / GS_TILE);
    a.rec = reinterpret_cast<const float4*>(rec); a.bg = backgrounds; a.isect_offsets = isect_offsets;
    a.flatten_ids = flatten_ids; a.slots = slots;
    a.out_colors = render_colors; a.out_alphas = render_alphas;
    a.ckpt = reinterpret_cast<float4*>(ckpt); a.qlist = reinterpret_cast<int2*>(qlist); a.qcnt = qcnt; a.qmask = qmask;
    a.unit_desc = reinterpret_cast<int4*>(unit_desc); a.walk = walk_state; a.cap_units = (int)cap_units;
    a.tile_order = tile_order;
    a.guard = current_guard().info;
    a.flags = a.guard ? reinterpret_cast<unsigned long long*>(const_cast<int64_t*>(a.guard) + 3) : nullptr;
    const Rounds R = current_rounds();
    const int phase = (R.phase == 1 || R.phase == 4) ? 1 : (R.phase == 2 ? 2 : 0);
    a.solo = R.phase == 4 ? 1 : 0;
    GS_REQUIRE(R.phase != 4 || a.flags != nullptr, "depth rounds, front round alone: needs a step guard (gs_guard_set)");
    GS_REQUIRE(phase == 0 || C == 1, "depth rounds: one camera per call");
    GS_REQUIRE(phase == 0 || !train || R.tile_rec, "depth rounds, training mode: gs_rounds_set needs tile_rec");
    GS_REQUIRE(NC == 3 || phase == 0, "depth rounds render 3 channels only (tile_state holds T, r, g, b): clear gs_rounds_set");
    GS_REQUIRE(NC != 4 || !train || ckpt_ext, "channels = 4, training mode: ckpt_ext (cap_units * 64 floats) is required");
    a.rblk = R.blk; a.live = R.live; a.tstate = R.state; a.trec = reinterpret_cast<int4*>(R.tile_rec);
    GS_IF_CHECK(a.chk = g_bwd_check;)
    const unsigned n_tiles = (unsigned)(C * a.tiles);
    hipStream_t st = (hipStream_t)stream;
    constexpr int kFwdWaves = 4;
    const dim3 grid((n_tiles + kFwdWaves - 1) / kFwdWaves), block(64 * kFwdWaves);
    if (train) {
        const int walk_ints = (int)gs_walk_state_ints(n_isects);
        const unsigned cg = (unsigned)std::min<int64_t>(1024, std::max<int64_t>(1, (n_isects / 16 + 255) / 256));
        hipLaunchKernelGGL(qmask_clear_kernel, dim3(cg), dim3(256), 0, st, qmask, n_isects, walk_state, walk_ints, a.guard,
                           (const int64_t*)R.blk, phase);
        GS_LAUNCH_CHECK("qmask_clear_kernel");
        if constexpr (NC != 3) hipLaunchKernelGGL((chan_fwd_kernel<true, kFwdWaves, NC>), grid, block, 0, st, a, ckpt_ext);
        else if (phase == 1) hipLaunchKernelGGL((blend_fwd_kernel<true, kFwdWaves, 1>), grid, block, 0, st, a);
        else if (phase == 2) hipLaunchKernelGGL((blend_fwd_kernel<true, kFwdWaves, 2>), grid, block, 0, st, a);
        else hipLaunchKernelGGL((blend_fwd_kernel<true, kFwdWaves, 0>), grid, block, 0, st, a);
        GS_LAUNCH_CHECK("blend_fwd_kernel");
        if (phase == 1 && !a.solo) return GS_OK;
        RowScanArgs s;
        s.qmask = qmask; s.row_base = row_base; s.walk = walk_state; s.n_cap = n_isects; s.cap_rows = cap_rows;
        s.flags = a.flags; s.guard = a.guard; s.mirror = current_walk_mirror();
        const unsigned chunks = (unsigned)(n_isects / kScanChunk + 1);
        hipLaunchKernelGGL(row_count_kernel, dim3(chunks), dim3(kScanThreads), 0, st, s);
        hipLaunchKernelGGL(row_chunk_scan_kernel, dim3(1), dim3(1024), 0, st, s);
        hipLaunchKernelGGL(row_base_kernel, dim3(chunks), dim3(kScanThreads), 0, st, s);
        GS_LAUNCH_CHECK("row_base_kernel");
    } else {
        if constexpr (NC != 3) hipLaunchKernelGGL((chan_fwd_kernel<false, kFwdWaves, NC>), grid, block, 0, st, a, nullptr);
        else if (phase == 1) hipLaunchKernelGGL((blend_fwd_kernel<false, kFwdWaves, 1>), grid, block, 0, st, a);
        else if (phase == 2) hipLaunchKernelGGL((blend_fwd_kernel<false, kFwdWaves, 2>), grid, block, 0, st, a);
        else hipLaunchKernelGGL((blend_fwd_kernel<false, kFwdWaves, 0>), grid, block, 0, st, a);
        GS_LAUNCH_CHECK("blend_fwd_kernel");
    }
    return GS_OK;
}

extern "C" int gs_blend_fwd(void* stream, int C, int width, int height, const float* rec,
                            const float* backgrounds, const int32_t* isect_offsets, const int32_t* tile_order,
                            const int32_t* flatten_ids, const int32_t* slots, int64_t n_isects, float* render_colors,
                            float* render_alphas, float* ckpt, int32_t* qlist, int32_t* qcnt, uint8_t* qmask,
                            int32_t* unit_desc, int64_t cap_units, int32_t* row_base, int64_t cap_rows, int32_t* walk_state) {
    return blend_fwd_launch<3>(stream, C, width, height, rec, backgrounds, isect_offsets, tile_order, flatten_ids, slots, n_isects,
                               render_colors, render_alphas, ckpt, qlist, qcnt, qmask, unit_desc, cap_units, row_base, cap_rows,
                               walk_state, nullptr);
}

extern "C" int gs_blend_fwd_ch(void* stream, int C, int width, int height, int channels, const float* rec,
                               const float* backgrounds, const int32_t* isect_offsets, const int32_t* tile_order,
                               const int32_t* flatten_ids, const int32_t* slots, int64_t n_isects, float* render_colors,
                               float* render_alphas, float* ckpt, int32_t* qlist, int32_t* qcnt, uint8_t* qmask,
                               int32_t* unit_desc, int64_t cap_units, int32_t* row_base, int64_t cap_rows, int32_t* walk_state,
                               float* ckpt_ext) {
    GS_REQUIRE(channels >= 1 && channels <= 4, "channels must be 1, 2, 3 or 4");
#define GS_FWD_CH(NC) blend_fwd_launch<NC>(stream, C, width, height, rec, backgrounds, isect_offsets, tile_order, flatten_ids, slots, \
                                           n_isects, render_colors, render_alphas, ckpt, qlist, qcnt, qmask, unit_desc, cap_units,   \
                                           row_base, cap_rows, walk_state, ckpt_ext)
    switch (channels) {
        case 1: return GS_FWD_CH(1);
        case 2: return GS_FWD_CH(2);
        case 3: return GS_FWD_CH(3);
        default: return GS_FWD_CH(4);
    }
#undef GS_FWD_CH
}

static int64_t cls_region(int C, int width, int height) {
    const int64_t tiles = (int64_t)((width + GS_TILE - 1) / GS_TILE) * ((height + GS_TILE - 1) / GS_TILE);
    const int64_t per_block = kBwdWaves * kUnitsPerWave;
    return (4 * (int64_t)C * tiles + per_block - 1) / per_block * per_block;
}

extern "C" size_t gs_unit_classes_ints(int64_t cap_units, int C, int width, int height) {
    if (cap_units < 0 || C < 1 || width <= 0 || height <= 0) return 0;
    return (size_t)kClsHdrInts + 4 * ((size_t)cap_units + 3 * (size_t)cls_region(C, width, height));
}

template <int NC>
static int blend_bwd_launch(void* stream, int C, int width, int height, const float* rec,
                            const int32_t* qlist, const int32_t* qcnt, const int32_t* unit_desc, int64_t cap_units,
                            const float* ckpt, const uint8_t* qmask, const int32_t* row_base, const int32_t* walk_state,
                            const float* render_colors, const float* render_alphas, const float* v_render_colors,
                            const float* v_render_alphas, float* rows, int32_t* unit_classes, const float* ckpt_ext) {
    GS_REQUIRE(C >= 1 && width > 0 && height > 0 && cap_units >= 0 && cap_units < (1ll << 26), "C>=1, positive image size, 0 <= cap_units < 2^26");
    if (cap_units == 0) return GS_OK;
    GS_REQUIRE(rec && qlist && qcnt && unit_desc && ckpt && qmask && row_base && walk_state, "null list pointer");
    GS_REQUIRE(render_colors && render_alphas && v_render_colors && rows, "null image pointer");
    GS_REQUIRE(NC != 4 || ckpt_ext, "channels = 4: ckpt_ext (gs_blend_fwd_ch's fourth-channel checkpoints) is required");
    BlendBwdArgs a;
    a.C = C; a.W = width; a.H = height;
    a.tw = (width + GS_TILE - 1) / GS_TILE;
    a.tiles = a.tw * ((height + GS_TILE - 1) / GS_TILE);
    a.rec = reinterpret_cast<const float4*>(rec);
    a.qlist = reinterpret_cast<const int2*>(qlist); a.qcnt = qcnt; a.walk = walk_state;
    a.unit_desc = reinterpret_cast<const int4*>(unit_desc); a.cap_units = (int)cap_units;
    a.ckpt = reinterpret_cast<const float4*>(ckpt); a.qmask = qmask; a.row_base = row_base;
    a.out_colors = render_colors;
    a.out_alphas = render_alphas; a.v_colors = v_render_colors; a.v_alphas = v_render_alphas;
    a.rows = reinterpret_cast<float4*>(rows);
    a.guard = current_guard().info;
    GS_IF_CHECK(a.chk = g_bwd_check;)
    unsigned grid = (unsigned)((cap_units + kUnitsPerWave * kBwdWaves - 1) / (kUnitsPerWave * kBwdWaves));
    a.cls_hdr = nullptr; a.cls_desc = nullptr; a.cls_cap = 0;
    if (unit_classes) {
        GS_REQUIRE(((uintptr_t)unit_classes & 15) == 0, "unit_classes must be 16-byte aligned");
        a.cls_hdr = unit_classes; a.cls_desc = reinterpret_cast<const int4*>(unit_classes + kClsHdrInts);
        a.cls_cap = (int)cls_region(C, width, height);
        hipLaunchKernelGGL(unit_classes_clear_kernel, dim3(1), dim3(64), 0, (hipStream_t)stream, unit_classes);
        hipLaunchKernelGGL(unit_classes_kernel, dim3((unsigned)((cap_units + kClsThreads - 1) / kClsThreads)), dim3(kClsThreads), 0, (hipStream_t)stream,
                           walk_state, a.unit_desc, qcnt, (int)cap_units, a.cls_cap, unit_classes, reinterpret_cast<int4*>(unit_classes + kClsHdrInts),
                           a.guard);
        GS_LAUNCH_CHECK("unit_classes_kernel");
        grid += 3u * (unsigned)(a.cls_cap / (kUnitsPerWave * kBwdWaves));
    }
    if constexpr (NC == 3) hipLaunchKernelGGL(blend_bwd_kernel, dim3(grid), dim3(kBwdWaves * 64), 0, (hipStream_t)stream, a);
    else hipLaunchKernelGGL((chan_bwd_kernel<NC>), dim3(grid), dim3(kBwdWaves * 64), 0, (hipStream_t)stream, a, ckpt_ext);
    GS_LAUNCH_CHECK("blend_bwd_kernel");
    return GS_OK;
}

extern "C" int gs_blend_bwd(void* stream, int C, int width, int height, const float* rec,
                            const int32_t* qlist, const int32_t* qcnt, const int32_t* unit_desc, int64_t cap_units,
                            const float* ckpt, const uint8_t* qmask, const int32_t* row_base, const int32_t* walk_state,
                            const float* render_colors, const float* render_alphas, const float* v_render_colors,
                            const float* v_render_alphas, float* rows, int32_t* unit_classes) {
    return blend_bwd_launch<3>(stream, C, width, height, rec, qlist, qcnt, unit_desc, cap_units, ckpt, qmask, row_base, walk_state,
                               render_colors, render_alphas, v_render_colors, v_render_alphas, rows, unit_classes, nullptr);
}

extern "C" int gs_blend_bwd_ch(void* stream, int C, int width, int height, int channels, const float* rec,
                               const int32_t* qlist, const int32_t* qcnt, const int32_t* unit_desc, int64_t cap_units,
                               const float* ckpt, const uint8_t* qmask, const int32_t* row_base, const int32_t* walk_state,
                               const float* render_colors, const float* render_alphas, const float* v_render_colors,
                               const float* v_render_alphas, float* rows, int32_t* unit_classes, const float* ckpt_ext) {
    GS_REQUIRE(channels >= 1 && channels <= 4, "channels must be 1, 2, 3 or 4");
#define GS_BWD_CH(NC) blend_bwd_launch<NC>(stream, C, width, height, rec, qlist, qcnt, unit_desc, cap_units, ckpt, qmask, row_base, \
                                           walk_state, render_colors, render_alphas, v_render_colors, v_render_alphas, rows,         \
                                           unit_classes, ckpt_ext)
    switch (channels) {
        case 1: return GS_BWD_CH(1);
        case 2: return GS_BWD_CH(2);
        case 3: return GS_BWD_CH(3);
        default: return GS_BWD_CH(4);
    }
#undef GS_BWD_CH
}
```

easy_gaussian_splatting_amd/csrc/gs_loss.hip:

```cpp
#include "gs_common.h"

namespace gs {

constexpr int kLT = 32;
constexpr int kHalo = 5;
constexpr int kLR = kLT + 2 * kHalo;
constexpr int kLRP = kLR + 1;
constexpr int kHP = kLT + 1;
static_assert(kLT * (kLT / 4) == 256 && kLR * 6 <= 256 && kLR % 6 == 0, "thread mapping of the staging and the separable passes");
static_assert(kLR % 2 == 0 && kLR * 3 <= 128, "backward staging: two 128-thread halves, one staged row each");
constexpr int64_t kLossMaxPixels = (int64_t)1 << 28;
constexpr int kLossMaxWidth = 1 << 20;
constexpr float kC1 = 0.01f * 0.01f, kC2 = 0.03f * 0.03f;

#define GS_WIN_TAPS {1.0283800845e-03f, 7.5987581352e-03f, 3.6000772128e-02f, 1.0936068951e-01f, 2.1300553771e-01f, \
                     2.6601172486e-01f, 2.1300553771e-01f, 1.0936068951e-01f, 3.6000772128e-02f, 7.5987581352e-03f, 1.0283800845e-03f}

struct LossArgs {
    int H, W;
    int clamp_input;
    float lambda_ssim;
    const float *render, *gt, *mask;
    const float* const* slots;
    float* maps;
    float* partial;
    const float* gout;
    float* v_render;
};

__device__ __forceinline__ int clampi(int v, int lo, int hi) { return v < lo ? lo : (v > hi ? hi : v); }
__device__ __forceinline__ float ld_off(const float* base, unsigned byte_off) {
    return *reinterpret_cast<const float*>(reinterpret_cast<const char*>(base) + byte_off);
}
__device__ __forceinline__ void st_off(float* base, unsigned byte_off, float v) {
    *reinterpret_cast<float*>(reinterpret_cast<char*>(base) + byte_off) = v;
}

struct F3 { float x, y, z; };
__device__ __forceinline__ F3 ld3_off(const float* base, unsigned byte_off) {
    return *reinterpret_cast<const F3*>(reinterpret_cast<const char*>(base) + byte_off);
}
__device__ __forceinline__ void st3_off(float* base, unsigned byte_off, float x, float y, float z) {
    *reinterpret_cast<F3*>(reinterpret_cast<char*>(base) + byte_off) = F3{x, y, z};
}

__device__ __forceinline__ bool loss_tile(const LossArgs& a, int& x0, int& y0) {
    const int ntx = (a.W + kLT - 1) / kLT, nt = ntx * ((a.H + kLT - 1) / kLT), per = (nt + 7) >> 3;
    const int id = blockIdx.x, t = (id & 7) * per + (id >> 3);
    if ((id >> 3) >= per || t >= nt) return false;
    const int ty = t / ntx;
    x0 = (t - ty * ntx) * kLT; y0 = ty * kLT;
    return true;
}

__device__ __forceinline__ bool loss_tile_channel(const LossArgs& a, int& x0, int& y0, int& ch) {
    const int ntx = (a.W + kLT - 1) / kLT, nt = ntx * ((a.H + kLT - 1) / kLT), per = (nt + 7) >> 3;
    const int id = blockIdx.x, k = id >> 3, local = k / 3, t = (id & 7) * per + local;
    ch = k - 3 * local;
    if (t >= nt) return false;
    const int ty = t / ntx;
    x0 = (t - ty * ntx) * kLT; y0 = ty * kLT;
    return true;
}

constexpr int kHOut = 6, kHWin = kHOut + 10;

template <bool MASK>
__global__ __launch_bounds__(256) void l1_ssim_fwd_kernel(const LossArgs a) {
    constexpr float kWin[11] = GS_WIN_TAPS;
    extern __shared__ __attribute__((aligned(16))) float lds[];
    float* sx = lds;
    float* sy = sx + kLR * kLRP;
    float* hp = sy + kLR * kLRP;
    __shared__ float red[2][4];
    int x0, y0;
    if (!loss_tile(a, x0, y0)) {
        if (threadIdx.x == 0) { a.partial[2 * blockIdx.x] = 0.f; a.partial[2 * blockIdx.x + 1] = 0.f; }
        return;
    }
    const int tid = threadIdx.x;
    const unsigned row_bytes = 12u * (unsigned)a.W;
    const float* gt_img = a.slots ? a.slots[0] : a.gt;
    const float* mask_img = a.slots ? a.slots[1] : a.mask;
    constexpr int kPer = kLR / 6;
    float rv[kPer][3], gv[kPer][3], mv[MASK ? kPer : 1];
    if (tid < kLR * 6) {
        const int rg = tid / kLR, col = tid - rg * kLR;
        const int cx = clampi(x0 - kHalo + col, 0, a.W - 1), ytop = y0 - kHalo + rg;
#pragma unroll
        for (int i = 0; i < kPer; ++i) {
            const unsigned cy = (unsigned)clampi(ytop + 6 * i, 0, a.H - 1);
            const unsigned o = __umul24(cy, row_bytes) + 12u * (unsigned)cx;
            const F3 g3 = ld3_off(gt_img, o), r3 = ld3_off(a.render, o);
            gv[i][0] = g3.x; gv[i][1] = g3.y; gv[i][2] = g3.z;
            rv[i][0] = r3.x; rv[i][1] = r3.y; rv[i][2] = r3.z;
            if (MASK) mv[i] = ld_off(mask_img, __umul24(cy, 4u * (unsigned)a.W) + 4u * (unsigned)cx);
        }
    }
    float l1 = 0.f, ssim_sum = 0.f;
#pragma unroll 1
    for (int ch = 0; ch < 3; ++ch) {
        int t = tid;
        asm volatile("" : "+v"(t));
        const bool st_on = t < kLR * 6;
        const int rg = t / kLR, col = t - rg * kLR;
        if (st_on) {
            const int gx = x0 - kHalo + col;
            const bool col_own = col >= kHalo && col < kHalo + kLT && gx < a.W;
            float* dx = sx + rg * kLRP + col;
            float* dy = sy + rg * kLRP + col;
#pragma unroll
            for (int i = 0; i < kPer; ++i) {
                const int row = rg + 6 * i, gy = y0 - kHalo + row;
                const float g = gv[i][0];
                float r = rv[i][0];
                if (a.clamp_input) r = fminf(fmaxf(r, 0.f), 1.f);
                if (MASK) r = mv[i] * g + (1.f - mv[i]) * r;
                dx[6 * i * kLRP] = r;
                dy[6 * i * kLRP] = g;
                if (col_own && row >= kHalo && row < kHalo + kLT && gy < a.H) l1 += fabsf(r - g);
                gv[i][0] = gv[i][1]; gv[i][1] = gv[i][2];
                rv[i][0] = rv[i][1]; rv[i][1] = rv[i][2];
            }
        }
        __syncthreads();
        float* maps_c = a.maps + (size_t)ch * a.H * a.W * 3;
        {
            const bool h_on = st_on;
            const int row = col, c0 = min(kHOut * rg, kLT - kHOut);
            if (h_on) {
                float* h = hp + row * kHP + c0;
                float xv[kHWin], yv[kHWin];
#pragma unroll
                for (int i = 0; i < kHWin; ++i) { xv[i] = sx[row * kLRP + c0 + i]; yv[i] = sy[row * kLRP + c0 + i]; }
#pragma unroll
                for (int j = 0; j < kHOut; ++j) {
                    float m0 = kWin[0] * xv[j], m1 = kWin[0] * yv[j], m2 = kWin[0] * fmaf(xv[j], xv[j], yv[j] * yv[j]),
                          m3 = kWin[0] * (xv[j] * yv[j]);
#pragma unroll
                    for (int kk = 1; kk < 11; ++kk) {
                        const float w = kWin[kk], x = xv[j + kk], y = yv[j + kk];
                        m0 = fmaf(w, x, m0); m1 = fmaf(w, y, m1); m2 = fmaf(w, fmaf(x, x, y * y), m2); m3 = fmaf(w, x * y, m3);
                    }
                    h[j] = m0; h[kLR * kHP + j] = m1; h[2 * kLR * kHP + j] = m2; h[3 * kLR * kHP + j] = m3;
                }
            }
        }
        __syncthreads();
        {
            const int q = t / kLT, vcol = t - q * kLT, r0 = 4 * q;
            float mom[4][4];
#pragma unroll
            for (int mi = 0; mi < 4; ++mi) {
                float hv[14];
#pragma unroll
                for (int i = 0; i < 14; ++i) hv[i] = hp[mi * kLR * kHP + (r0 + i) * kHP + vcol];
#pragma unroll
                for (int j = 0; j < 4; ++j) {
                    float acc = kWin[0] * hv[j];
#pragma unroll
                    for (int kk = 1; kk < 11; ++kk) acc = fmaf(kWin[kk], hv[j + kk], acc);
                    mom[mi][j] = acc;
                }
            }
            const int gx = x0 + vcol;
#pragma unroll
            for (int j = 0; j < 4; ++j) {
                const int gy = y0 + r0 + j;
                const float mu_x = mom[0][j], mu_y = mom[1][j], ess = mom[2][j], exy = mom[3][j];
                const bool interior = gy >= kHalo && gy < a.H - kHalo && gx >= kHalo && gx < a.W - kHalo;
                if (gy < a.H && gx < a.W) {
                    float dmu = 0.f, dxx = 0.f, dxy = 0.f;
                    if (interior) {
                        const float mm = mu_x * mu_x + mu_y * mu_y, sxy = exy - mu_x * mu_y;
                        const float n1 = 2.f * mu_x * mu_y + kC1, n2 = 2.f * sxy + kC2;
                        const float d1 = mm + kC1, d2 = (ess - mm) + kC2;
                        const float i1 = __builtin_amdgcn_rcpf(d1), i2 = __builtin_amdgcn_rcpf(d2), inv = i1 * i2;
                        const float sv = n1 * n2 * inv;
                        ssim_sum += sv;
                        dxx = -sv * i2;
                        dxy = 2.f * n1 * inv;
                        dmu = 2.f * mu_y * (n2 - n1) * inv + 2.f * mu_x * sv * (i2 - i1);
                    }
                    st3_off(maps_c, __umul24((unsigned)gy, row_bytes) + 12u * (unsigned)gx, dmu, dxx, dxy);
                }
            }
        }
        if (ch < 2) __syncthreads();
    }
    l1 = wave_reduce_add(l1);
    ssim_sum = wave_reduce_add(ssim_sum);
    if (lane_id() == 0) { red[0][tid >> 6] = l1; red[1][tid >> 6] = ssim_sum; }
    __syncthreads();
    if (tid == 0) {
        a.partial[2 * blockIdx.x] = red[0][0] + red[0][1] + red[0][2] + red[0][3];
        a.partial[2 * blockIdx.x + 1] = red[1][0] + red[1][1] + red[1][2] + red[1][3];
    }
}

__global__ __launch_bounds__(256) void loss_reduce_kernel(int nblocks, const float* __restrict__ partial, int H, int W,
                                                          float lambda_ssim, float* __restrict__ out) {
    __shared__ double red[2][4];
    double s0 = 0.0, s1 = 0.0;
    for (int i = threadIdx.x; i < nblocks; i += 256) { s0 += partial[2 * i]; s1 += partial[2 * i + 1]; }
#pragma unroll
    for (int d = 32; d > 0; d >>= 1) { s0 += __shfl_xor(s0, d, 64); s1 += __shfl_xor(s1, d, 64); }
    if (lane_id() == 0) { red[0][threadIdx.x >> 6] = s0; red[1][threadIdx.x >> 6] = s1; }
    __syncthreads();
    if (threadIdx.x == 0) {
        const double l1 = (red[0][0] + red[0][1] + red[0][2] + red[0][3]) / ((double)H * W * 3.0);
        const double cnt = (double)(H - 2 * kHalo) * (double)(W - 2 * kHalo) * 3.0;
        const double ssim = (red[1][0] + red[1][1] + red[1][2] + red[1][3]) / cnt;
        out[0] = (float)l1; out[1] = (float)(1.0 - ssim);
        out[2] = (float)((1.0 - lambda_ssim) * l1 + lambda_ssim * (1.0 - ssim));
    }
}

__global__ __launch_bounds__(256) void l1_ssim_bwd_kernel(const LossArgs a) {
    constexpr float kWin[11] = GS_WIN_TAPS;
    extern __shared__ __attribute__((aligned(16))) float lds[];
    float* sm = lds;
    float* hp = lds;
    int x0, y0, ch;
    if (!loss_tile_channel(a, x0, y0, ch)) return;
    const int tid = threadIdx.x;
    const size_t plane = (size_t)a.H * a.W;
    const float g = a.gout[0];
    const float cnt = (float)(a.H - 2 * kHalo) * (float)(a.W - 2 * kHalo) * 3.f;
    const float k_ssim = -g * a.lambda_ssim / cnt;
    const float k_l1 = g * (1.f - a.lambda_ssim) / ((float)a.H * (float)a.W * 3.f);
    const unsigned row_bytes = 12u * (unsigned)a.W;
    const int q = tid / kLT, ocol = tid - q * kLT, r0 = 4 * q, ogx = x0 + ocol;
    const bool col_in = ogx < a.W;
    const unsigned o0 = __umul24((unsigned)min(y0 + r0, a.H - 1), row_bytes) + 12u * (unsigned)min(ogx, a.W - 1);
    const float* mask_img = a.slots ? a.slots[1] : a.mask;
    const float* gt_c = (a.slots ? a.slots[0] : a.gt) + ch;
    const float* render_c = a.render + ch;
    float gtv[4], rr[4], mk[4];
#pragma unroll
    for (int j = 0; j < 4; ++j) {
        const unsigned o = o0 + (y0 + r0 + j < a.H ? j * row_bytes : 0u);
        gtv[j] = ld_off(gt_c, o); rr[j] = ld_off(render_c, o);
        if (mask_img) mk[j] = ld_off(mask_img, o / 3u);
    }
    {
        constexpr int kRowsPer = kLR / 2;
        const int half = __builtin_amdgcn_readfirstlane(tid >> 7), jj = tid & 127;
        const int scol = jj / 3, smi = jj - scol * 3;
        const int sgx = x0 - kHalo + scol;
        const float* maps_c = a.maps + (size_t)ch * plane * 3;
        if (jj < kLR * 3) {
            const bool col_ok = sgx >= 0 && sgx < a.W;
            const unsigned lane_off = 4u * (unsigned)(clampi(sgx, 0, a.W - 1) * 3 + smi);
            float v[kRowsPer];
            const int gy0 = y0 - kHalo + half;
            const char* rowp = reinterpret_cast<const char*>(maps_c) + (int64_t)gy0 * row_bytes;
#pragma unroll
            for (int i = 0; i < kRowsPer; ++i) {
                const int gy = gy0 + 2 * i;
                v[i] = 0.f;
                if (gy >= 0 && gy < a.H) v[i] = ld_off(reinterpret_cast<const float*>(rowp), lane_off);
                rowp += 2 * row_bytes;
            }
            float* d = sm + (smi * kLR + half) * kLRP + scol;
#pragma unroll
            for (int i = 0; i < kRowsPer; ++i) d[2 * i * kLRP] = col_ok ? v[i] : 0.f;
        }
    }
    __syncthreads();
    {
        const bool h_on = tid < kLR * 6;
        const int hg = tid / kLR, row = tid - hg * kLR, c0 = min(kHOut * hg, kLT - kHOut);
        float ho[3][kHOut];
        if (h_on) {
#pragma unroll
            for (int mi = 0; mi < 3; ++mi) {
                float w[kHWin];
#pragma unroll
                for (int i = 0; i < kHWin; ++i) w[i] = sm[(mi * kLR + row) * kLRP + c0 + i];
#pragma unroll
                for (int j = 0; j < kHOut; ++j) {
                    float acc = kWin[0] * w[j];
#pragma unroll
                    for (int k = 1; k < 11; ++k) acc = fmaf(kWin[k], w[j + k], acc);
                    ho[mi][j] = acc;
                }
            }
        }
        __syncthreads();
        if (h_on) {
#pragma unroll
            for (int mi = 0; mi < 3; ++mi)
#pragma unroll
                for (int j = 0; j < kHOut; ++j) hp[mi * kLR * kHP + row * kHP + c0 + j] = ho[mi][j];
        }
    }
    __syncthreads();
    {
        float c[3][4];
#pragma unroll
        for (int mi = 0; mi < 3; ++mi) {
            float hv[14];
#pragma unroll
            for (int i = 0; i < 14; ++i) hv[i] = hp[mi * kLR * kHP + (r0 + i) * kHP + ocol];
#pragma unroll
            for (int j = 0; j < 4; ++j) {
                float acc = kWin[0] * hv[j];
#pragma unroll
                for (int k = 1; k < 11; ++k) acc = fmaf(kWin[k], hv[j + k], acc);
                c[mi][j] = acc;
            }
        }
        float* out_c = a.v_render + ch;
#pragma unroll
        for (int j = 0; j < 4; ++j) {
            if (y0 + r0 + j >= a.H || !col_in) continue;
            float r = rr[j], keep = 1.f;
            if (a.clamp_input) { keep = (r >= 0.f && r <= 1.f) ? 1.f : 0.f; r = fminf(fmaxf(r, 0.f), 1.f); }
            if (mask_img) { r = mk[j] * gtv[j] + (1.f - mk[j]) * r; keep *= 1.f - mk[j]; }
            const float d = r - gtv[j];
            const float sgn = d > 0.f ? 1.f : (d < 0.f ? -1.f : 0.f);
            st_off(out_c, o0 + j * row_bytes, keep * (k_ssim * (c[0][j] + 2.f * r * c[1][j] + gtv[j] * c[2][j]) + k_l1 * sgn));
        }
    }
}

__global__ __launch_bounds__(256) void clamp01_kernel(int64_t n4, int64_t n, const float* __restrict__ x,
                                                      const float* __restrict__ v_out, float* __restrict__ out) {
    const int64_t i = (int64_t)blockIdx.x * blockDim.x + threadIdx.x;
    if (i < n4) {
        const float4 a = reinterpret_cast<const float4*>(x)[i];
        float4 r;
        if (v_out) {
            const float4 g = reinterpret_cast<const float4*>(v_out)[i];
            r.x = (a.x >= 0.f && a.x <= 1.f) ? g.x : 0.f; r.y = (a.y >= 0.f && a.y <= 1.f) ? g.y : 0.f;
            r.z = (a.z >= 0.f && a.z <= 1.f) ? g.z : 0.f; r.w = (a.w >= 0.f && a.w <= 1.f) ? g.w : 0.f;
        } else {
            r.x = fminf(fmaxf(a.x, 0.f), 1.f); r.y = fminf(fmaxf(a.y, 0.f), 1.f);
            r.z = fminf(fmaxf(a.z, 0.f), 1.f); r.w = fminf(fmaxf(a.w, 0.f), 1.f);
        }
        reinterpret_cast<float4*>(out)[i] = r;
    }
    if (i == 0)
        for (int64_t k = n4 * 4; k < n; ++k) {
            const float a = x[k];
            out[k] = v_out ? ((a >= 0.f && a <= 1.f) ? v_out[k] : 0.f) : fminf(fmaxf(a, 0.f), 1.f);
        }
}

}

using namespace gs;

extern "C" int gs_clamp01(void* stream, int64_t n, const float* x, const float* v_out, float* out) {
    GS_REQUIRE(n >= 0, "n >= 0");
    if (n == 0) return GS_OK;
    GS_REQUIRE(x && out, "null pointer");
    GS_REQUIRE((((uintptr_t)x | (uintptr_t)out | (uintptr_t)v_out) & 15) == 0, "buffers must be 16-byte aligned");
    const int64_t n4 = n >> 2, blocks = (n4 + 255) / 256;
    hipLaunchKernelGGL(clamp01_kernel, dim3((unsigned)(blocks > 0 ? blocks : 1)), dim3(256), 0, (hipStream_t)stream, n4, n, x, v_out, out);
    GS_LAUNCH_CHECK("clamp01_kernel");
    return GS_OK;
}

static int loss_tile_count(int height, int width) { return ((width + kLT - 1) / kLT) * ((height + kLT - 1) / kLT); }
static dim3 loss_grid(int nt) { return dim3((unsigned)(8 * ((nt + 7) / 8))); }

extern "C" size_t gs_loss_workspace_floats(int height, int width) {
    const size_t nb = (size_t)((width + kLT - 1) / kLT) * ((height + kLT - 1) / kLT);
    return 9 * (size_t)height * width + 2 * (nb + 8);
}

static int loss_fwd_launch(void* stream, int height, int width, float lambda_ssim, const float* render, const float* gt,
                           const float* mask, const float* const* slots, bool has_mask, int clamp_input, float* workspace, float* out3) {
    GS_REQUIRE(height > 2 * kHalo && width > 2 * kHalo, "image must be larger than the 11x11 window");
    GS_REQUIRE((int64_t)height * width <= kLossMaxPixels && width <= kLossMaxWidth && height <= (1 << 24),
               "image too large for the loss kernels' 32-bit byte offsets (H * W <= 2^28, W <= 2^20, H <= 2^24: row indices go through 24-bit multiplies)");
    GS_REQUIRE(render && (gt || slots) && workspace && out3, "null pointer");
    LossArgs a;
    a.H = height; a.W = width; a.lambda_ssim = lambda_ssim; a.render = render; a.gt = gt; a.mask = mask; a.slots = slots;
    a.clamp_input = clamp_input != 0;
    a.maps = workspace; a.partial = workspace + 9 * (size_t)height * width; a.gout = nullptr; a.v_render = nullptr;
    const int blocks = (int)loss_grid(loss_tile_count(height, width)).x;
    const size_t lds = sizeof(float) * (2 * kLR * kLRP + 4 * kLR * kHP);
    hipStream_t st = (hipStream_t)stream;
    if (has_mask) hipLaunchKernelGGL(l1_ssim_fwd_kernel<true>, dim3((unsigned)blocks), dim3(256), lds, st, a);
    else hipLaunchKernelGGL(l1_ssim_fwd_kernel<false>, dim3((unsigned)blocks), dim3(256), lds, st, a);
    GS_LAUNCH_CHECK("l1_ssim_fwd_kernel");
    hipLaunchKernelGGL(loss_reduce_kernel, dim3(1), dim3(256), 0, st, blocks, a.partial, height, width, lambda_ssim, out3);
    GS_LAUNCH_CHECK("loss_reduce_kernel");
    return GS_OK;
}

static int loss_bwd_launch(void* stream, int height, int width, float lambda_ssim, const float* render, const float* gt,
                           const float* mask, const float* const* slots, int clamp_input, const float* workspace,
                           const float* v_total, float* v_render) {
    GS_REQUIRE(height > 2 * kHalo && width > 2 * kHalo, "image must be larger than the 11x11 window");
    GS_REQUIRE((int64_t)height * width <= kLossMaxPixels && width <= kLossMaxWidth && height <= (1 << 24),
               "image too large for the loss kernels' 32-bit byte offsets (H * W <= 2^28, W <= 2^20, H <= 2^24: row indices go through 24-bit multiplies)");
    GS_REQUIRE(render && (gt || slots) && workspace && v_total && v_render, "null pointer");
    LossArgs a;
    a.H = height; a.W = width; a.lambda_ssim = lambda_ssim; a.render = render; a.gt = gt; a.mask = mask; a.slots = slots;
    a.clamp_input = clamp_input != 0;
    a.maps = const_cast<float*>(workspace); a.partial = nullptr; a.gout = v_total; a.v_render = v_render;
    const size_t lds = sizeof(float) * (3 * kLR * kLRP);
    hipLaunchKernelGGL(l1_ssim_bwd_kernel, dim3(3 * loss_grid(loss_tile_count(height, width)).x), dim3(256), lds, (hipStream_t)stream, a);
    GS_LAUNCH_CHECK("l1_ssim_bwd_kernel");
    return GS_OK;
}

extern "C" int gs_l1_ssim_fwd(void* stream, int height, int width, float lambda_ssim, const float* render,
                              const float* gt, const float* mask, int clamp_input, float* workspace, float* out3) {
    return loss_fwd_launch(stream, height, width, lambda_ssim, render, gt, mask, nullptr, mask != nullptr, clamp_input, workspace, out3);
}

extern "C" int gs_l1_ssim_bwd(void* stream, int height, int width, float lambda_ssim, const float* render,
                              const float* gt, const float* mask, int clamp_input, const float* workspace,
                              const float* v_total, float* v_render) {
    return loss_bwd_launch(stream, height, width, lambda_ssim, render, gt, mask, nullptr, clamp_input, workspace, v_total, v_render);
}

extern "C" int gs_l1_ssim_fwd_slots(void* stream, int height, int width, float lambda_ssim, const float* render,
                                    const float* const* slots_dev, int has_mask, int clamp_input, float* workspace, float* out3) {
    GS_REQUIRE(slots_dev != nullptr, "slots_dev is required");
    return loss_fwd_launch(stream, height, width, lambda_ssim, render, nullptr, nullptr, slots_dev, has_mask != 0, clamp_input, workspace, out3);
}

extern "C" int gs_l1_ssim_bwd_slots(void* stream, int height, int width, float lambda_ssim, const float* render,
                                    const float* const* slots_dev, int clamp_input, const float* workspace,
                                    const float* v_total, float* v_render) {
    GS_REQUIRE(slots_dev != nullptr, "slots_dev is required");
    return loss_bwd_launch(stream, height, width, lambda_ssim, render, nullptr, nullptr, slots_dev, clamp_input, workspace, v_total, v_render);
}
```

easy_gaussian_splatting_amd/train_graph.py:

```python
from __future__ import annotations

import ctypes as ct
import math
import time
from collections import deque
from collections.abc import Mapping
from typing import Any, Dict, Optional

import torch
from torch import Tensor

from . import _native as nat
from .optim import FusedAdam
from . import rendering
from .rendering import _SH_JAC


_TILE = nat.GS_TILE
_SORT_CLASSES = (1024, 4096, 8192, 16384)


def _p(t: Optional[Tensor]):
    return None if t is None else t.data_ptr()

# ... 337 lines not shown
                r.stream.wait_stream(self.outer)
            self.ctx = torch.cuda.stream(r.stream)
            self.ctx.__enter__()

        def __exit__(self, *exc):
            self.ctx.__exit__(*exc)
            if self.hand_back:
                self.outer.wait_stream(self.r.stream)
            return False

    def _on_stream(self, wait_outer: bool = True, hand_back: bool = True):
        return TrainStepGraph._OnStepStream(self, wait_outer, hand_back)

    def fence(self):
        torch.cuda.current_stream(self.dev).wait_stream(self.stream)

    class _StepOutputs(Mapping):

        def __init__(self, runner, items, lazy: bool):
            self._items, self._runner, self._pending = dict(items), runner, lazy

        def _touch(self):
            if self._pending:
                self._pending = False
                self._runner.fence()

        def __getitem__(self, k):
            self._touch()
            return self._items[k]

        def __iter__(self):
            return iter(self._items)

        def __len__(self):
            return len(self._items)

    stop_after = int(__import__('os').environ.get('GS_TG_STOP_AFTER', '0'))
    project_rebuilds = __import__('os').environ.get('GS_TG_PROJECT_REBUILDS', '1') != '0'
    debug_sync = False

    class _Stop(Exception):
        pass

    def _ck(self, rc: int, what: str) -> None:
        nat.check(rc, what)
        self._stage_no = getattr(self, "_stage_no", 0) + 1
        if self.stop_after and self._stage_no >= self.stop_after:
            raise TrainStepGraph._Stop()
        if self.debug_sync and not torch.cuda.is_current_stream_capturing():
            self.stream.synchronize()

    def _project(self):
        L, b, m = nat.lib(), self.buf, self.model
        culling = {"gsplat": 1, "tight": 1, "gsplat_eager": 0}[getattr(m, "tile_culling", "tight")]
        self._ck(L.gs_project_fwd(self._st(), 1, self.N, self.K, int(m.active_sh_degree), _p(m.means), _p(m.quats), _p(m.log_scales),
                                   _p(m.logit_opacities), _p(m.sh_0), _p(m.sh_rest) if self.K > 1 else None, 0,
                                   _p(b["viewmats"]), _p(b["Ks"]), self.W, self.H, 0.3, 0.01, 1e10, 0.0, culling, 0, 1,
                                   _p(b["radii"]), _p(b["means2d"]), _p(b["depths"]), _p(b["conics"]), _p(b["colors_post"]),
                                   _p(b["rec"]), _p(b["bbox"]), _p(b["tiles_per_gauss"]), None, _p(b["sh_jac"])), "gs_project_fwd")

    def _count(self, bbox: str = "bbox"):
        L, b = nat.lib(), self.buf
        if self.binning == "bins":
            self._ck(L.gs_bins_count(self._st(), 1, self.N, self.tw, self.th, self.bin_shift, _p(b[bbox]), _p(b["depths"]), _p(b["ws"]),
                                      self.ws_bytes, _p(b["coarse_keys"]), self.cap_coarse, self.cap_coarse_list, _p(b["cum_tiles"]),
                                      _p(b["isect_offsets"]), _p(b["bucket_offsets"]), _p(b["tile_order"]), _p(b["info"]), None),
                     "gs_bins_count")
        else:
            self._ck(L.gs_bin_count(self._st(), 1, self.N, self.tw, self.th, _p(b[bbox]), _p(b["ws"]), self.ws_bytes,
                                     _p(b["isect_offsets"]), _p(b["bucket_offsets"]), _p(b["tile_order"]), _p(b["info"]), None),
                     "gs_bin_count")

    def _probe(self):
        from .rendering import MAX_TILES_PER_TILE_PIPELINE, bin_shift_for, binning_choice
        L, b, dev = nat.lib(), self.buf, self.dev
        tiles = self.tw * self.th
        n_isects = max_tile = 0
        footprint = None
        if tiles <= MAX_TILES_PER_TILE_PIPELINE:
            self.binning = "tiles"
            self.ws_bytes = int(L.gs_bin_workspace_bytes(1, self.N, self.tw, self.th))
            b["ws"] = torch.empty((self.ws_bytes,), dtype=torch.uint8, device=dev)
            with torch.cuda.device(dev), self._on_stream():
                self._project()
                self._count()
            info = b["info"].tolist()
            n_isects, max_tile = int(info[nat.GS_INFO_ISECTS]), int(info[nat.GS_INFO_MAX_TILE])
            footprint = n_isects / max(1, self.N)
        else:
            with torch.cuda.device(dev), self._on_stream():
                self._project()
        self.binning = binning_choice(footprint, tiles)
        if self.binning == "bins":
            self.bin_shift = bin_shift_for(footprint) or 2
            self.cap_coarse, self.cap_coarse_list = 2 * self.N + 1024, 0
            while True:
                self._alloc_binning()
                with torch.cuda.device(dev), self._on_stream():
                    self._count()
                info = b["info"].tolist()
                if not int(info[nat.GS_INFO_FLAGS]) & (nat.GS_FLAG_COARSE | nat.GS_FLAG_COARSE_LIST):
                    break
                self.cap_coarse = int(int(info[nat.GS_INFO_COARSE]) * self.margin) + 4096
            self.cap_coarse = int(int(info[nat.GS_INFO_COARSE]) * self.margin) + 4096
            self.cap_coarse_list = int(int(info[nat.GS_INFO_MAX_BIN]) * 1.5) + 64
            self.probed_coarse = (int(info[nat.GS_INFO_COARSE]), int(info[nat.GS_INFO_MAX_BIN]))
            n_isects, max_tile = int(info[nat.GS_INFO_ISECTS]), int(info[nat.GS_INFO_MAX_TILE])
        b["info"].zero_()
        return n_isects, max_tile

    def _enqueue_forward(self):
        L, b = nat.lib(), self.buf
        self._project()
        if not self.rounds_on:
            self._lists_and_blend("bbox")
            return
        self._ck(L.gs_round_split(self._st(), self.N, _p(b["depths"]), _p(b["tiles_per_gauss"]), self.round_fraction, _p(b["depth_hist"]),
                                   _p(b["rounds"])), "gs_round_split")
        for phase in ((4,) if self.front_only else (1, 2)):
            self._rounds_phase(phase)
            self._ck(L.gs_round_footprints(self._st(), self.N, self.tw, self.th, _p(b["bbox"]), _p(b["depths"]), _p(b["bbox_round"]),
                                            _p(b["tpg_round"])), "gs_round_footprints")
            self._lists_and_blend("bbox_round")
        self._rounds_phase(3)

    def _lists_and_blend(self, bbox: str):
        L, b = nat.lib(), self.buf
        st = self._st()
        N, W, H = self.N, self.W, self.H
        self._count(bbox)
        if self.binning == "bins":
            self._ck(L.gs_bins_lists(st, 1, N, self.tw, self.th, self.bin_shift, _p(b[bbox]), _p(b["ws"]), self.ws_bytes,
                                      _p(b["coarse_keys"]), self.cap_coarse, _p(b["cum_tiles"]), _p(b["isect_offsets"]),
                                      None, _p(b["flatten_ids"]), _p(b["slots"]), _p(b["info"])), "gs_bins_lists")
        else:
            self._ck(L.gs_bin_emit_sort(st, 1, N, self.tw, self.th, _p(b[bbox]), _p(b["depths"]), _p(b["ws"]), self.ws_bytes,
                                         _p(b["isect_offsets"]), self.cap, self.cap_tile, _p(b["keys_tmp"]), _p(b["slot_gid"]),
                                         _p(b["cum_tiles"]), None, _p(b["flatten_ids"]), _p(b["slots"])), "gs_bin_emit_sort")
        self._ck(L.gs_blend_fwd(st, 1, W, H, _p(b["rec"]), _p(b["bg"]), _p(b["isect_offsets"]),
                                 _p(b["tile_order"]), _p(b["flatten_ids"]), _p(b["slots"]), self.cap, _p(b["render_colors"]),
                                 _p(b["render_alphas"]), _p(b["ckpt"]), _p(b["qlist"]), _p(b["qcnt"]), _p(b["qmask"]),
                                 _p(b["unit_desc"]), self.cap_units, _p(b["row_base"]), self.cap_rows, _p(b["walk_state"])),
                 "gs_blend_fwd")

    def _enqueue_step(self):
        L, b, m, opt = nat.lib(), self.buf, self.model, self.opt
        st = self._st()
        N, W, H = self.N, self.W, self.H
        nat.check(L.gs_guard_set(_p(b["info"]), self.cap, self.cap_tile), "gs_guard_set")
        self._stage_no = 0
        try:
            self._enqueue_forward()
            lam = float(self.lc.lambda_ssim)
            self._ck(L.gs_l1_ssim_fwd_slots(st, H, W, lam, _p(b["render_colors"]), _p(b["img_slots"]), int(self.has_mask), 1, _p(b["loss_ws"]),
                                             _p(b["loss3"])), "gs_l1_ssim_fwd_slots")
            self._ck(L.gs_l1_ssim_bwd_slots(st, H, W, lam, _p(b["render_colors"]), _p(b["img_slots"]), 1, _p(b["loss_ws"]),
                                             _p(b["one"]), _p(b["v_render"])), "gs_l1_ssim_bwd_slots")
            if self.scale_reg and self.fuse_adam:
                self._scale_reg(None)
            self._ck(L.gs_blend_bwd(st, 1, W, H, _p(b["rec"]), _p(b["qlist"]), _p(b["qcnt"]), _p(b["unit_desc"]), self.cap_units,
                                     _p(b["ckpt"]), _p(b["qmask"]), _p(b["row_base"]), _p(b["walk_state"]),
                                     _p(b["render_colors"]), _p(b["render_alphas"]), _p(b["v_render"]), None, _p(b["rows"]), _p(b["unit_cls"])),
                      "gs_blend_bwd")
            b1, b2 = opt.defaults["betas"]
            if self.fuse_adam:
                offs = (ct.c_int64 * 6)(*opt._offs)
                args = (st, N, self.K, int(m.active_sh_degree), _p(opt.flat_param), _p(opt.exp_avg),
                        _p(opt.exp_avg_sq), offs, _p(b["viewmats"]), _p(b["Ks"]), W, H, 0.3, 0.01, 1e10,
                        _p(b["radii"]), _p(b["colors_post"]), self._tpg(), _p(b["cum_tiles"]),
                        _p(b["rows"]), _p(b["row_base"]), _p(b["qmask"]), _p(b["v_abs"]), float(b1), float(b2),
                        float(opt.defaults["eps"]), _p(b["hyper"]), _p(b["applied"]), _p(m.max_radii),
                        _p(m.grad_norm_accum), _p(m.collecting_counts), _p(b["sh_jac"]))
                if self.scale_reg:
                    self._ck(L.gs_project_bwd_adam_reg(*args, self.max_scale_ratio, self.lambda_scale), "gs_project_bwd_adam_reg")
                else:
                    self._ck(L.gs_project_bwd_adam(*args), "gs_project_bwd_adam")
            else:
                g = self.grads
                self._ck(L.gs_project_bwd(st, 1, N, self.K, int(m.active_sh_degree), _p(m.means), _p(m.quats), _p(m.log_scales),
                                          _p(m.sh_0), _p(m.sh_rest) if self.K > 1 else None, 0, _p(b["viewmats"]), _p(b["Ks"]), W, H,
                                          0.3, 0.01, 1e10, _p(b["radii"]), _p(b["colors_post"]), self._tpg(),
                                          _p(b["cum_tiles"]), _p(b["rows"]), _p(b["row_base"]), _p(b["qmask"]), _p(g["means"]), _p(g["quats"]),
                                          _p(g["log_scales"]), _p(g["logit_opacities"]), _p(g["sh_0"]), _p(g["sh_rest"]), _p(b["v_abs"]),
                                          None, None, None, None, _p(m.logit_opacities), 1, _p(b["sh_jac"]), None, None, None), "gs_project_bwd")
                if self.scale_reg:
                    self._scale_reg(g["log_scales"])
                self._ck(L.gs_update_statistics(st, N, float(max(H, W)), _p(b["radii"]), _p(b["v_abs"]), _p(m.max_radii),
                                                _p(m.grad_norm_accum), _p(m.collecting_counts)), "gs_update_statistics")
                ns = len(opt._plist)
                ends = (ct.c_int64 * ns)(*opt._ends)
                lens = (ct.c_int64 * ns)(*opt._lens)
                gptr = (ct.c_void_p * ns)(*[_p(g[grp["name"]]) for grp, _ in opt._plist])
                self._ck(L.gs_adam_step_dev(st, opt.flat_param.numel(), _p(opt.flat_param), _p(opt.exp_avg), _p(opt.exp_avg_sq), ns,
                                            ends, lens, gptr, float(b1), float(b2), float(opt.defaults["eps"]), 1.0, _p(b["hyper"]),
                                            _p(b["applied"])), "gs_adam_step_dev")
            self._ck(L.gs_step_status(st, _p(b["info"]), _p(b["applied"]), self.status.data_ptr(), _p(b["loss3"]), _p(b["loss_ring"]),
                                      self.LOSS_RING, _p(b["walk_state"])), "gs_step_status")
        except TrainStepGraph._Stop:
            pass
        finally:
            L.gs_guard_set(None, 0, 0)
            L.gs_rounds_set(None, None, None, None, 0)

    def _scale_reg(self, v_log_scales: Optional[Any], check=None):
        b, m = self.buf, self.model
        v = v_log_scales if (v_log_scales is None or isinstance(v_log_scales, int)) else v_log_scales.data_ptr()
        (check or self._ck)(nat.lib().gs_scale_reg(self._st(), self.N, _p(m.log_scales), self.max_scale_ratio, self.lambda_scale, _p(b["loss3"]),
                                        _p(b["scale_reg"]), v), "gs_scale_reg")

    def _tail(self, t: int, lrs):
        """What a step enqueues behind its graph (nothing: the single-GPU step is the graph)."""

    def _hyper(self, t: int, lrs):
        L, opt = nat.lib(), self.opt
        ns = len(opt._plist)
        b1, b2 = opt.defaults["betas"]
        nat.check(L.gs_adam_hyper(self._st(), ns, (ct.c_float * ns)(*lrs), float(b1), float(b2), int(t), _p(self.buf["hyper"])),
                  "gs_adam_hyper")

    def _capture(self, warm_up: bool = True):
        opt, m = self.opt, self.model
        names = ("max_radii", "grad_norm_accum", "collecting_counts")
        with torch.cuda.device(self.dev), self._on_stream():
            if warm_up:
                self._warm.add((self.binning, self.cap_tile))
                saved = [opt.flat_param.clone(), opt.exp_avg.clone(), opt.exp_avg_sq.clone()] + [getattr(m, n).clone() for n in names]
                self._hyper(max(opt._step, 0) + 1, [float(grp["lr"]) for grp, _ in opt._plist])
                self._enqueue_step()
                self.stream.synchronize()
                info = self.buf["info"].tolist()
                with torch.no_grad():
                    opt.flat_param.copy_(saved[0]); opt.exp_avg.copy_(saved[1]); opt.exp_avg_sq.copy_(saved[2])
                    for n, s in zip(names, saved[3:]):
                        getattr(m, n).copy_(s)
                self.buf["applied"].zero_()
                if info[nat.GS_INFO_FLAGS] != 0:
                    self.buf["info"].zero_()
                    raise RuntimeError(f"TrainStepGraph: warm-up step overflowed its own capacities {info}")
            self.graph = None
            if self.use_graph:
                g = torch.cuda.CUDAGraph()
                with torch.cuda.graph(g, stream=self.stream):
                    self._enqueue_step()
                self.graph = g
                self.stats["captures"] += 1
            if warm_up:
                self.stream.synchronize()
        self.status.zero_()
        self.confirmed_at_build = self.confirmed

    def _issue(self, entry):
        t, lrs, w2c, K, gt, mask, ready = entry[:7]
        conv = entry[7] if len(entry) > 7 else None
        after = entry[8] if len(entry) > 8 else None
        with torch.cuda.device(self.dev), self._on_stream(wait_outer=not ready, hand_back=self.handback == "eager"):
            if conv is not None:
                self.stream.wait_event(conv)
                entry[7] = None
            if after is not None:
                for ev in (after if isinstance(after, (list, tuple)) else (after,)):
                    self.stream.wait_event(ev)
                entry[8] = None
            entry[4], entry[5] = self._stage_inputs(t, lrs, w2c, K, gt, mask)
            if self.graph is not None:
                self.graph.replay()
            else:
                self._enqueue_step()
            self._tail(t, lrs)
        self.pending.append(entry)
        self.issued += 1

    def step(self, data: Optional[Dict[str, Any]] = None, gt_img: Optional[Tensor] = None, mask: Optional[Tensor] = None,
             inputs_ready: bool = False, ready_event: Optional["torch.cuda.Event"] = None, host_src=None):
        _refuse_camera_grads(data)
        W, H = (self.W, self.H) if data is None else (int(data["width"]), int(data["height"]))
        if self._state_key(W, H) != self._key:
            self.finish()
            size_changed = (W, H) != (self.W, self.H)
            if size_changed:
                if gt_img is None or (self.has_mask and mask is None):
                    raise ValueError("TrainStepGraph.step: a change of image size needs gt_img (and mask) of the new size")
                cur = (data["w2c"], data["K"], gt_img, mask)
                self.W, self.H = W, H
            else:
                cur = self._last_inputs if data is None else (data["w2c"], data["K"], gt_img if gt_img is not None else self._last_inputs[2],
                                                              mask if mask is not None else self._last_inputs[3])
            n_new = self.model.means.shape[0]
            growth = max(1.0, n_new / max(self.N, 1))
            self.cap_floor = 0 if size_changed else min(int(self.seen_isects * growth * self.margin), (1 << 31) - (1 << 20))
            self.walk_floor = (0, 0) if size_changed else (int(self.seen_units * growth), int(self.seen_rows * growth))
            reset = getattr(self.model, "opacity_resets", 0) != self._opacity_resets
            if reset:
                self.walk_floor = (0, 0)
                self._walk_history_void = True
            projected = carried = None
            if (not size_changed and not reset and self.binning == "tiles" and self.seen_isects > 0 and growth <= 2.0 and self.project_rebuilds
                    and self._key is not None and self._state_key(W, H)[5:] == self._key[5:]):
                projected = (min(int(self.seen_isects * growth), 1 << 30), max(int(self.seen_tile * min(growth, 1.25)), 64),
                             int(self.seen_units * growth), int(self.seen_rows * growth))
                cls = next((c for c in _SORT_CLASSES if c >= int(projected[1] * self.margin)), 1 << 30)
                if (self.binning, cls) not in self._warm:
                    carried, projected = projected, None
            self.seen_isects = self.seen_tile = self.seen_units = self.seen_rows = 0
            self.cap = self.cap_units = self.cap_rows = 0
            if projected is None and carried is not None:
                self._build({"w2c": cur[0], "K": cur[1]}, cur[2], cur[3] if self.has_mask else None, min_cap=carried[0], min_cap_tile=carried[1],
                            min_walk=carried[2:4])
            else:
                self._build({"w2c": cur[0], "K": cur[1]}, cur[2], cur[3] if self.has_mask else None, projected=projected)
        b = self.buf
        w2c = b["viewmats"][0] if data is None else data["w2c"]
        K = b["Ks"][0] if data is None else data["K"]
        gt = self._last_inputs[2] if gt_img is None else gt_img
        mk = (self._last_inputs[3] if mask is None else mask) if self.has_mask else None
        gt_in, mk_in = gt, mk
        gt = self._image(gt, (self.H, self.W, 3))
        if self.has_mask:
            if mk is None:
                raise ValueError("this runner was built with a mask; pass one every step")
            mk = self._image(mk, (self.H, self.W))
        if self.copy_targets and gt_img is not None:
            gt = gt.clone() if gt is gt_in else gt
            mk = (mk.clone() if mk is mk_in else mk) if mk is not None else None
        conv = None
        if gt is not gt_in or mk is not mk_in:
            conv = torch.cuda.Event()
            conv.record(torch.cuda.current_stream(self.dev))
        self._last_inputs = (w2c, K, gt, mk)
        opt = self.opt
        opt._step += 1
        self._issue([opt._step, [float(grp["lr"]) for grp, _ in opt._plist], w2c, K, gt, mk, bool(inputs_ready), conv, ready_event, host_src])
        if self.issued % self.check_every == 0:
            self._poll(block=False)
        outs = {"render_img": b["render_colors"][0], "loss3": b["loss3"], "batch_radii": b["radii"], "absgrad": b["v_abs"]}
        if self.scale_reg:
            outs["scale_reg"] = b["scale_reg"][0]
        return TrainStepGraph._StepOutputs(self, outs, lazy=self.handback == "lazy")

    def _poll(self, block: bool):
        if block:
            self.stream.synchronize()
        n_isects, _, max_tile, flags, applied, units, rows, live = (int(v) for v in self.status[:8].tolist())
        if live >= 0 and applied > 0:
            self._live_sum, self._live_n = self._live_sum + live, self._live_n + 1
        self.seen_isects = max(self.seen_isects, n_isects)
        self.seen_tile = max(self.seen_tile, max_tile)
        self.seen_units, self.seen_rows = max(self.seen_units, units), max(self.seen_rows, rows)
        done = min(self.confirmed_at_build + applied - self.confirmed, len(self.pending))
        for _ in range(max(done, 0)):
            self.pending.popleft()
        self.confirmed += max(done, 0)
        if flags != 0:
            self._recover(n_isects, max_tile, (units, rows) if flags & (nat.GS_FLAG_UNITS | nat.GS_FLAG_ROWS) else (0, 0))

    def _recover(self, n_isects: int, max_tile: int, walk=(0, 0)):
        self.stream.synchronize()
        applied = int(self.buf["applied"].item())
        done = self.confirmed_at_build + applied - self.confirmed
        for _ in range(done):
            self.pending.popleft()
        self.confirmed += done
        redo = list(self.pending)
        self.pending.clear()
        self.issued -= len(redo)
        self.stats["overflows"] += 1
        self.stats["replayed_steps"] += len(redo)
        if int(self.status[nat.GS_INFO_FLAGS]) & nat.GS_FLAG_BACK:
            self._back_needed = True
            self.stats["back_round_needed"] = self.stats.get("back_round_needed", 0) + 1
        self.stats.setdefault("overflow_log", []).append({
            "step": self.confirmed + 1, "flags": int(self.status[nat.GS_INFO_FLAGS]), "isects": n_isects, "longest_list": max_tile, "work_units": walk[0], "rows": walk[1],
            "capacities": [self.cap, self.cap_tile, self.cap_units, self.cap_rows]})
        for e in redo:
            src = e[9] if len(e) > 9 else None
            if src is not None:
                e[2], e[3] = src["w2c"].to(self.dev, torch.float32), src["K"].to(self.dev, torch.float32)
                e[4] = HostFeed.to_target(src["image"], self.dev)
                e[5] = src["mask"].to(self.dev, torch.float32) if (self.has_mask and src.get("mask") is not None) else e[5]
        first = redo[0]
        self._build({"w2c": first[2], "K": first[3]}, first[4], first[5], min_cap=max(n_isects, 1), min_cap_tile=max_tile, min_walk=walk)
        for e in redo:
            self._issue(e)

    def finish(self):
        while self.pending:
            self._poll(block=True)

    LOSS_RING = 4096

    def loss_history(self, last_n: int) -> Tensor:
        applied = int(self.buf["applied"].item())
        n = max(0, min(int(last_n), applied, self.LOSS_RING))
        idx = (torch.arange(applied - n, applied, device=self.dev)) % self.LOSS_RING
        return self.buf["loss_ring"][idx]

    def report(self) -> Dict[str, Any]:
        extra = dict(scale_reg=True, max_scale_ratio=self.max_scale_ratio, lambda_scale=self.lambda_scale) if self.scale_reg else {}
        return dict(self.stats, **extra, binning=self.binning, probed_isects=self.probed[0], probed_longest_list=self.probed[1],
                    probed_coarse_entries=getattr(self, "probed_coarse", (0, 0))[0] if self.binning == "bins" else 0,
                    capacity_isects=self.cap, capacity_tile_list=self.cap_tile, capacity_work_units=self.cap_units,
                    capacity_rows=self.cap_rows, probed_work_units=self.probed_walk[0], probed_rows=self.probed_walk[1],
                    seen_work_units=self.seen_units, seen_rows=self.seen_rows, steps=self.confirmed,
                    graph=self.graph is not None, rounds=bool(self.rounds_on), round_fraction=self.round_fraction if self.rounds_on else None,
                    front_round_alone=bool(self.rounds_on and self.front_only))


class ViewParallelGraphStep(TrainStepGraph):

    def __init__(self, model, optimizer, loss_computer, data, gt_img, mask=None, vp=None, **kw):
        if vp is None or not vp.exchange or not vp.native or not vp.guard_words:
            raise ValueError("ViewParallelGraphStep needs a native ViewParallelStep(..., guard_words=True) with the exchange on")
        if not vp._raw_parameters():
            raise ValueError("ViewParallelGraphStep: the model must pass its raw parameters (fuse_activations)")
        self.vp = vp
        kw["fuse_adam"] = False
        super().__init__(model, optimizer, loss_computer, data, gt_img, mask, **kw)

    def _alloc_lists(self):
        super()._alloc_lists()
        self.buf["row_sums"] = self._take("row_sums", (self.N, 12), torch.float32)
        self.vp._records(); self.vp._bucket()

    def _enqueue_step(self):
        L, b, m, vp = nat.lib(), self.buf, self.model, self.vp
        st = self._st()
        N, W, H = self.N, self.W, self.H
        send, _ = vp._records()
        _, offs, flat = vp._bucket()
        nat.check(L.gs_guard_set(_p(b["info"]), self.cap, self.cap_tile), "gs_guard_set")
        self._stage_no = 0
        try:
            self._enqueue_forward()
            lam = float(self.lc.lambda_ssim)
            self._ck(L.gs_l1_ssim_fwd_slots(st, H, W, lam, _p(b["render_colors"]), _p(b["img_slots"]), int(self.has_mask), 1, _p(b["loss_ws"]),
                                             _p(b["loss3"])), "gs_l1_ssim_fwd_slots")
            self._ck(L.gs_l1_ssim_bwd_slots(st, H, W, lam, _p(b["render_colors"]), _p(b["img_slots"]), 1, _p(b["loss_ws"]),
                                             _p(b["one"]), _p(b["v_render"])), "gs_l1_ssim_bwd_slots")
            self._ck(L.gs_blend_bwd(st, 1, W, H, _p(b["rec"]), _p(b["qlist"]), _p(b["qcnt"]), _p(b["unit_desc"]), self.cap_units,
                                     _p(b["ckpt"]), _p(b["qmask"]), _p(b["row_base"]), _p(b["walk_state"]),
                                     _p(b["render_colors"]), _p(b["render_alphas"]), _p(b["v_render"]), None, _p(b["rows"]), _p(b["unit_cls"])), "gs_blend_bwd")
            sp = send.data_ptr()
            self._ck(L.gs_row_sums(st, 1, N, _p(b["radii"]), _p(b["colors_post"]), self._tpg(), _p(b["cum_tiles"]), _p(b["rows"]),
                                    _p(b["row_base"]), _p(b["qmask"]), _p(b["row_sums"]), sp, sp + 4 * 3 * N, float(max(H, W)), _p(b["viewmats"]),
                                    sp + 4 * 4 * N), "gs_row_sums")
            self._ck(L.gs_guard_flag_out(st, _p(b["info"]), sp + 4 * (4 * N + 16), flat.data_ptr() + 4 * vp._flag_off), "gs_guard_flag_out")
        except TrainStepGraph._Stop:
            pass
        finally:
            L.gs_guard_set(None, 0, 0)
            L.gs_rounds_set(None, None, None, None, 0)

    def _tail(self, t: int, lrs):
        import torch.distributed as dist
        L, b, m, vp, opt = nat.lib(), self.buf, self.model, self.vp, self.opt
        st = self._st()
        N, W, H, world = self.N, self.W, self.H, vp.world
        P = vp.record_len()
        send, recv = vp._records()
        _, offs, flat = vp._bucket()
        seg = lambda i, n: flat.data_ptr() + 4 * offs[i]
        w_gather = dist.all_gather_into_tensor(recv, send, group=vp.group, async_op=True)
        vp.collectives += 1
        nat.check(L.gs_guard_set(_p(b["info"]), self.cap, self.cap_tile), "gs_guard_set")
        try:
            nat.check(L.gs_project_bwd(st, 1, N, self.K, int(m.active_sh_degree), _p(m.means), _p(m.quats), _p(m.log_scales), _p(m.sh_0),
                                       _p(m.sh_rest) if self.K > 1 else None, 0, _p(b["viewmats"]), _p(b["Ks"]), W, H, 0.3, 0.01, 1e10, _p(b["radii"]),
                                       _p(b["colors_post"]), self._tpg(), _p(b["cum_tiles"]), _p(b["rows"]), _p(b["row_base"]), _p(b["qmask"]),
                                       seg(0, 3 * N), seg(2, 4 * N), seg(1, 3 * N), seg(3, N), None, None, _p(b["v_abs"]), None, None, None, None,
                                       _p(m.logit_opacities), 1, _p(b["sh_jac"]), _p(b["row_sums"]), seg(4, N), seg(5, N)), "gs_project_bwd")
            if self.scale_reg:
                self._scale_reg(seg(1, 3 * N), nat.check)
            w_sum = dist.all_reduce(flat, op=dist.ReduceOp.SUM, group=vp.group, async_op=True)
            vp.collectives += 1
            w_gather.wait()
            nat.check(L.gs_guard_merge(st, _p(b["info"]), recv.data_ptr() + 4 * (4 * N + 16), world, P), "gs_guard_merge")
            lr = dict(zip([g["name"] for g, _ in opt._plist], lrs))
            m0, v0 = opt.moments_of(m.sh_0)
            mr, vr = opt.moments_of(m.sh_rest) if self.K > 1 else (None, None)
            b1, b2 = opt.defaults["betas"]
            nat.check(L.gs_sh_adam_views(st, world, N, self.K, int(m.active_sh_degree), _p(m.means), recv.data_ptr(), P, _p(m.sh_0), _p(m0), _p(v0),
                                         _p(m.sh_rest) if self.K > 1 else None, _p(mr), _p(vr), float(lr["sh_0"]), float(lr["sh_rest"]), float(b1),
                                         float(b2), float(opt.defaults["eps"]), int(t), 1.0 / world, _p(m.max_radii)), "gs_sh_adam_views")
            w_sum.wait()
            nat.check(L.gs_guard_merge(st, _p(b["info"]), flat.data_ptr() + 4 * vp._flag_off, 1, 0), "gs_guard_merge")
            ns = len(opt._plist)
            grads = {"means": seg(0, 3 * N), "log_scales": seg(1, 3 * N), "quats": seg(2, 4 * N), "logit_opacities": seg(3, N)}
            gptr = (ct.c_void_p * ns)(*[grads.get(g["name"]) for g, _ in opt._plist])
            nat.check(L.gs_adam_step_stats(st, opt.flat_param.numel(), _p(opt.flat_param), _p(opt.exp_avg), _p(opt.exp_avg_sq), ns,
                                           (ct.c_int64 * ns)(*opt._ends), (ct.c_int64 * ns)(*opt._lens), gptr, (ct.c_float * ns)(*lrs), float(b1),
                                           float(b2), float(opt.defaults["eps"]), int(t), 1.0 / world, N, seg(4, N), seg(5, N),
                                           _p(m.grad_norm_accum), _p(m.collecting_counts)), "gs_adam_step_stats")
            nat.check(L.gs_step_applied(st, _p(b["info"]), _p(b["applied"])), "gs_step_applied")
            nat.check(L.gs_step_status(st, _p(b["info"]), _p(b["applied"]), self.status.data_ptr(), _p(b["loss3"]), _p(b["loss_ring"]),
                                       self.LOSS_RING, _p(b["walk_state"])), "gs_step_status")
        finally:
            L.gs_guard_set(None, 0, 0)
            L.gs_rounds_set(None, None, None, None, 0)

    def _poll(self, block: bool):
        super()._poll(block=True)


class HostFeed:

    def __init__(self, runner: "TrainStepGraph", n_slots: int = 2, inputs_ready: bool = False):
        self.r, self.n = runner, max(2, int(n_slots))
        self.inputs_ready = bool(inputs_ready)
        dev = runner.dev
        self.copy_stream = torch.cuda.Stream(dev)
        H, W = runner.H, runner.W
        f32 = dict(dtype=torch.float32, device=dev)
        self.gt = [torch.empty((H, W, 3), **f32) for _ in range(self.n)]
        self.u8 = [None] * self.n
        self.mask = [torch.empty((H, W), **f32) if runner.has_mask else None for _ in range(self.n)]
        self.w2c = [torch.empty((4, 4), **f32) for _ in range(self.n)]
        self.K = [torch.empty((3, 3), **f32) for _ in range(self.n)]
        self.done = [None] * self.n
        self._t255 = torch.full((), 255.0, **f32)
        self.i = 0

    @staticmethod
    def to_target(image: Tensor, dev) -> Tensor:
        x = image.to(dev, non_blocking=False)
        if x.dtype == torch.uint8:
            return torch.div(x.to(torch.float32), torch.full((), 255.0, dtype=torch.float32, device=dev))
        return x.to(torch.float32)

    def step(self, batch: Dict[str, Any]):
        r, j = self.r, self.i % self.n
        self.i += 1
        if (int(batch["width"]), int(batch["height"])) != (r.W, r.H):
            raise ValueError("HostFeed: one frame size per feed (build another for another size)")
        cs = self.copy_stream
        if self.done[j] is not None:
            self.done[j].synchronize()
            cs.wait_event(self.done[j])
        img = batch["image"]
        with torch.cuda.device(r.dev), torch.cuda.stream(cs):
            self.w2c[j].copy_(batch["w2c"], non_blocking=True)
            self.K[j].copy_(batch["K"], non_blocking=True)
            if img.dtype == torch.uint8:
                if self.u8[j] is None:
                    self.u8[j] = torch.empty(tuple(img.shape), dtype=torch.uint8, device=r.dev)
                self.u8[j].copy_(img, non_blocking=True)
                torch.div(self.u8[j].to(torch.float32), self._t255, out=self.gt[j])
            else:
                self.gt[j].copy_(img, non_blocking=True)
            if r.has_mask:
                self.mask[j].copy_(batch["mask"], non_blocking=True)
            ev = torch.cuda.Event()
            ev.record(cs)
        out = r.step({"w2c": self.w2c[j], "K": self.K[j], "width": r.W, "height": r.H}, self.gt[j], self.mask[j] if r.has_mask else None,
                     inputs_ready=self.inputs_ready, ready_event=ev, host_src=batch)
        self.done[j] = torch.cuda.Event()
        self.done[j].record(r.stream)
        return out
```

include/gs_raster.h:

```cpp
#ifndef GS_RASTER_H_
#define GS_RASTER_H_

#include <stddef.h>
#include <stdint.h>

#ifdef __cplusplus
extern "C" {
#endif

#define GS_TILE 16
#define GS_BUCKET 64
#define GS_UNIT 32
#define GS_REC_FLOATS 12
#ifndef GS_ROW_FLOATS
#define GS_ROW_FLOATS 12
#endif

#define GS_WALK_UNITS 0
#define GS_WALK_STORAGE 1
#define GS_WALK_ROWS 3
#define GS_WALK_FLAGS 4
#define GS_WALK_SKIP 5
#define GS_WALK_RANGES 32
#define GS_WALK_RANGE0 32
// ... 63 lines not shown
#define GS_WS_BUCKET_OFFSETS 7
#define GS_WS_TILE_ORDER 8
#define GS_WS_QCNT 9
#define GS_WS_SH_JAC 10
#define GS_WS_LIST_FIRST 11
#define GS_WS_BIN 11
#define GS_WS_COARSE_KEYS 12
#define GS_WS_KEYS_TMP 13
#define GS_WS_SLOT_GID 14
#define GS_WS_FLATTEN_IDS 15
#define GS_WS_SLOTS_BUF 16
#define GS_WS_ISECT_IDS_BUF 17
#define GS_WS_QMASK 18
#define GS_WS_ROW_BASE 19
#define GS_WS_WALK_STATE 20
#define GS_WS_WALK_FIRST 21
#define GS_WS_CKPT 21
#define GS_WS_QLIST 22
#define GS_WS_UNIT_DESC 23
#define GS_WS_ROWS 24
#define GS_WS_SLOTS 25
#define GS_WS_TRAIN 1
#define GS_WS_TWO_LEVEL 2
#define GS_WS_ISECT_IDS 4
int gs_workspace_query(int C, int64_t N, int width, int height, int64_t cap_isects, int64_t coarse_cap, int64_t cap_units,
                       int64_t cap_rows, int bin_shift, int flags, int64_t* offsets, int64_t* arena_bytes);
int gs_workspace_bind(void* stream, void* fixed_base, int64_t fixed_bytes, void* list_base, int64_t list_bytes,
                      void* walk_base, int64_t walk_bytes, const int64_t* offsets, const int64_t* arena_bytes);

int gs_bin_groups(int64_t N);
size_t gs_bin_workspace_bytes(int C, int64_t N, int tile_w, int tile_h);

int gs_project_fwd(void* stream, int C, int64_t N, int K, int sh_degree, const float* means,
                   const float* quats, const float* scales, const float* opacities,
                   const float* colors_in, const float* sh_rest, int colors_per_camera,
                   const float* viewmats, const float* Ks, int width, int height, float eps2d,
                   float near_plane, float far_plane, float radius_clip, int tile_culling, int stage, int activations,
                   int32_t* radii,
                   float* means2d, float* depths, float* conics, float* colors_out, float* rec, uint32_t* bbox,
                   int32_t* tiles_per_gauss, uint32_t* rect_ref, float* sh_jac);

int gs_bin_count(void* stream, int C, int64_t N, int tile_w, int tile_h, const uint32_t* bbox,
                 void* workspace, size_t workspace_bytes, int32_t* isect_offsets,
                 int32_t* bucket_offsets, int32_t* tile_order, int64_t* info_dev, int64_t* info_host);

int gs_bin_emit_sort(void* stream, int C, int64_t N, int tile_w, int tile_h, const uint32_t* bbox,
                     const float* depths, void* workspace, size_t workspace_bytes,
                     const int32_t* isect_offsets, int64_t n_isects, int64_t max_tile_count,
                     uint64_t* keys_tmp, int32_t* slot_gid, int32_t* cum_tiles, int64_t* isect_ids,
                     int32_t* flatten_ids, int32_t* slots);

size_t gs_bins_workspace_bytes(int C, int64_t N, int tile_w, int tile_h, int bin_shift, int64_t coarse_cap);
int gs_bins_count(void* stream, int C, int64_t N, int tile_w, int tile_h, int bin_shift, const uint32_t* bbox,
                  const float* depths, void* workspace, size_t workspace_bytes, uint64_t* coarse_keys,
                  int64_t coarse_cap, int64_t coarse_list_cap, int32_t* cum_tiles, int32_t* isect_offsets,
                  int32_t* bucket_offsets, int32_t* tile_order, int64_t* info_dev, int64_t* info_host);
int gs_bins_lists(void* stream, int C, int64_t N, int tile_w, int tile_h, int bin_shift, const uint32_t* bbox,
                  void* workspace, size_t workspace_bytes, const uint64_t* coarse_keys, int64_t coarse_cap,
                  const int32_t* cum_tiles, const int32_t* isect_offsets, int64_t* isect_ids, int32_t* flatten_ids,
                  int32_t* slots, const int64_t* info_dev);

size_t gs_walk_state_ints(int64_t n_isects);
int gs_blend_fwd(void* stream, int C, int width, int height, const float* rec,
                 const float* backgrounds, const int32_t* isect_offsets, const int32_t* tile_order,
                 const int32_t* flatten_ids, const int32_t* slots, int64_t n_isects, float* render_colors,
                 float* render_alphas, float* ckpt, int32_t* qlist, int32_t* qcnt, uint8_t* qmask,
                 int32_t* unit_desc, int64_t cap_units, int32_t* row_base, int64_t cap_rows, int32_t* walk_state);

size_t gs_unit_classes_ints(int64_t cap_units, int C, int width, int height);
int gs_blend_bwd(void* stream, int C, int width, int height, const float* rec,
                 const int32_t* qlist, const int32_t* qcnt, const int32_t* unit_desc, int64_t cap_units,
                 const float* ckpt, const uint8_t* qmask, const int32_t* row_base, const int32_t* walk_state,
                 const float* render_colors, const float* render_alphas, const float* v_render_colors,
                 const float* v_render_alphas, float* rows, int32_t* unit_classes);

int gs_rec_colors(void* stream, int C, int64_t N, int channels, const float* colors, int colors_per_camera, const int32_t* radii,
                  float* rec);
int gs_blend_fwd_ch(void* stream, int C, int width, int height, int channels, const float* rec,
                    const float* backgrounds, const int32_t* isect_offsets, const int32_t* tile_order,
                    const int32_t* flatten_ids, const int32_t* slots, int64_t n_isects, float* render_colors,
                    float* render_alphas, float* ckpt, int32_t* qlist, int32_t* qcnt, uint8_t* qmask,
                    int32_t* unit_desc, int64_t cap_units, int32_t* row_base, int64_t cap_rows, int32_t* walk_state,
                    float* ckpt_ext);
int gs_blend_bwd_ch(void* stream, int C, int width, int height, int channels, const float* rec,
                    const int32_t* qlist, const int32_t* qcnt, const int32_t* unit_desc, int64_t cap_units,
                    const float* ckpt, const uint8_t* qmask, const int32_t* row_base, const int32_t* walk_state,
                    const float* render_colors, const float* render_alphas, const float* v_render_colors,
                    const float* v_render_alphas, float* rows, int32_t* unit_classes, const float* ckpt_ext);
int gs_channel_grads(void* stream, int C, int64_t N, int channels, int colors_per_camera, const int32_t* radii,
                     const int32_t* tiles_per_gauss, const int32_t* cum_tiles, const float* rows, const int32_t* row_base,
                     const uint8_t* qmask, float* v_colors);

int gs_project_bwd(void* stream, int C, int64_t N, int K, int sh_degree, const float* means,
                   const float* quats, const float* scales, const float* colors_in,
                   const float* sh_rest, int colors_per_camera, const float* viewmats,
                   const float* Ks, int width, int height, float eps2d, float near_plane, float far_plane,
                   const int32_t* radii, const float* colors_post, const int32_t* tiles_per_gauss,
                   const int32_t* cum_tiles, const float* rows, const int32_t* row_base, const uint8_t* qmask,
                   float* v_means, float* v_quats, float* v_scales, float* v_opacities,
                   float* v_colors, float* v_sh_rest, float* v_means2d_abs, float* v_means2d,
                   float* v_conics, float* v_colors_post, float* v_colors_pre,
                   const float* opacities, int activations, const float* sh_jac, const float* row_sums,
                   float* stat_grad_norm, float* stat_count);

size_t gs_cam_partials_doubles(int C, int64_t N);
int gs_project_bwd_cam(void* stream, int C, int64_t N, int K, int sh_degree, const float* means,
                       const float* quats, const float* scales, const float* colors_in,
                       const float* sh_rest, int colors_per_camera, const float* viewmats,
                       const float* Ks, int width, int height, float eps2d, float near_plane, float far_plane,
                       const int32_t* radii, const float* colors_post, const int32_t* tiles_per_gauss,
                       const int32_t* cum_tiles, const float* rows, const int32_t* row_base, const uint8_t* qmask,
                       float* v_means, float* v_quats, float* v_scales, float* v_opacities,
                       float* v_colors, float* v_sh_rest, float* v_means2d_abs, float* v_means2d,
                       float* v_conics, float* v_colors_post, float* v_colors_pre,
                       const float* opacities, int activations, const float* sh_jac, const float* row_sums,
                       float* stat_grad_norm, float* stat_count, double* cam_partials, float* v_viewmats,
                       float* v_campos);

int gs_rec_depth(void* stream, int C, int64_t N, int lane, const float* depths, const int32_t* radii, float* rec);
size_t gs_depth_partials_doubles(int C, int64_t N);
int gs_depth_grads(void* stream, int C, int64_t N, int lane, const float* means, const float* viewmats, const int32_t* radii,
                   const int32_t* tiles_per_gauss, const int32_t* cum_tiles, const float* rows, const int32_t* row_base,
                   const uint8_t* qmask, float* v_means, float* v_depths, double* cam_partials, float* v_viewmats);
int gs_expected_depth_fwd(void* stream, int64_t n_pixels, int channels, const float* acc_colors, const float* alphas,
                          float* out_colors);
int gs_expected_depth_bwd(void* stream, int64_t n_pixels, int channels, const float* acc_colors, const float* alphas,
                          const float* v_out, const float* v_alphas_in, float* v_colors, float* v_alphas);

int gs_row_sums(void* stream, int C, int64_t N, const int32_t* radii, const float* colors_post,
                const int32_t* tiles_per_gauss, const int32_t* cum_tiles, const float* rows, const int32_t* row_base, const uint8_t* qmask,
                float* row_sums, float* v_colors_pre, float* radii_norm, float max_hw, const float* viewmats, float* cam_out);

int gs_sh_grad_views(void* stream, int R, int64_t N, int K, int sh_degree, const float* means,
                     const float* viewmats, const float* v_colors_pre, float* v_colors,
                     float* v_sh_rest);

int gs_sh_adam_views(void* stream, int R, int64_t N, int K, int sh_degree, const float* means, const float* payload,
                     int64_t payload_stride, float* sh_0, float* sh_0_exp_avg, float* sh_0_exp_avg_sq, float* sh_rest,
                     float* sh_rest_exp_avg, float* sh_rest_exp_avg_sq, float lr_sh_0, float lr_sh_rest, float beta1, float beta2,
                     float eps, int64_t step, float grad_scale, float* max_radii);

size_t gs_loss_workspace_floats(int height, int width);
int gs_l1_ssim_fwd(void* stream, int height, int width, float lambda_ssim, const float* render,
                   const float* gt, const float* mask, int clamp_input, float* workspace, float* out3);
int gs_l1_ssim_bwd(void* stream, int height, int width, float lambda_ssim, const float* render,
                   const float* gt, const float* mask, int clamp_input, const float* workspace,
                   const float* v_total, float* v_render);

int gs_l1_ssim_fwd_slots(void* stream, int height, int width, float lambda_ssim, const float* render,
                         const float* const* slots_dev, int has_mask, int clamp_input, float* workspace, float* out3);
int gs_l1_ssim_bwd_slots(void* stream, int height, int width, float lambda_ssim, const float* render,
                         const float* const* slots_dev, int clamp_input, const float* workspace,
                         const float* v_total, float* v_render);

int gs_clamp01(void* stream, int64_t n, const float* x, const float* v_out, float* out);

int gs_adam_step(void* stream, int64_t n, float* params, float* exp_avg, float* exp_avg_sq,
                 int n_segments, const int64_t* seg_ends_host, const int64_t* seg_lens_host,
                 const float* const* seg_grads_host, const float* seg_lrs_host, float beta1,
                 float beta2, float eps, int64_t step, float grad_scale);

int gs_adam_step_stats(void* stream, int64_t n, float* params, float* exp_avg, float* exp_avg_sq,
                       int n_segments, const int64_t* seg_ends_host, const int64_t* seg_lens_host,
                       const float* const* seg_grads_host, const float* seg_lrs_host, float beta1, float beta2,
                       float eps, int64_t step, float grad_scale, int64_t stat_n, const float* stat_src0,
                       const float* stat_src1, float* stat_dst0, float* stat_dst1);

int gs_adam_hyper(void* stream, int n_segments, const float* seg_lrs_host, float beta1, float beta2, int64_t step,
                  float* hyper_dev);
int gs_step_inputs(void* stream, int n_segments, const float* seg_lrs_host, float beta1, float beta2, int64_t step,
                   float* hyper_dev, const float* viewmat_src, float* viewmat_dst, const float* K_src, float* K_dst,
                   const float* gt, const float* mask, const float** slots_dev);
int gs_adam_step_dev(void* stream, int64_t n, float* params, float* exp_avg, float* exp_avg_sq, int n_segments,
                     const int64_t* seg_ends_host, const int64_t* seg_lens_host, const float* const* seg_grads_host,
                     float beta1, float beta2, float eps, float grad_scale, const float* hyper_dev, int64_t* applied_dev);

size_t gs_scan_rows_workspace_ints(int rows, int64_t n);
int gs_scan_rows_i32(void* stream, int rows, int64_t n, const int32_t* in, int32_t* out, int32_t* workspace);
int gs_refine_flags(void* stream, int64_t n, int num_splits, float densify_grad_thresh, float densify_scale_thresh,
                    float prune_radii_ratio_thresh, float prune_scale_thresh, float min_opacity,
                    const float* grad_norm_accum, const float* counts, const float* max_radii, const float* log_scales,
                    const float* logit_opacities, int32_t* flags, int64_t* counters);
int gs_refine_apply(void* stream, int64_t n_old, int num_splits, int K, const int32_t* flags, const int32_t* flags_incl,
                    int64_t tot_old, int64_t tot_child, int64_t tot_clone, const float* noise, const float* old_params,
                    const float* old_exp_avg, const float* old_exp_avg_sq, const int64_t* old_offsets_host, float* new_params,
                    float* new_exp_avg, float* new_exp_avg_sq, const int64_t* new_offsets_host, int32_t* src_scratch,
                    int8_t* tag_scratch);

int gs_project_bwd_adam(void* stream, int64_t N, int K, int sh_degree, float* params, float* exp_avg, float* exp_avg_sq,
                        const int64_t* offsets_host, const float* viewmats, const float* Ks, int width, int height, float eps2d,
                        float near_plane, float far_plane, const int32_t* radii, const float* colors_post,
                        const int32_t* tiles_per_gauss, const int32_t* cum_tiles, const float* rows, const int32_t* row_base, const uint8_t* qmask,
                        float* v_means2d_abs, float beta1, float beta2, float eps, const float* hyper_dev, int64_t* applied_dev,
                        float* max_radii, float* grad_norm_accum, float* counts, const float* sh_jac);

size_t gs_scale_reg_workspace_floats(int64_t N);
int gs_scale_reg(void* stream, int64_t N, const float* log_scales, float max_ratio, float lambda, float* loss3, float* reg_ws,
                 float* v_log_scales);
int gs_project_bwd_adam_reg(void* stream, int64_t N, int K, int sh_degree, float* params, float* exp_avg, float* exp_avg_sq,
                            const int64_t* offsets_host, const float* viewmats, const float* Ks, int width, int height, float eps2d,
                            float near_plane, float far_plane, const int32_t* radii, const float* colors_post,
                            const int32_t* tiles_per_gauss, const int32_t* cum_tiles, const float* rows, const int32_t* row_base,
                            const uint8_t* qmask, float* v_means2d_abs, float beta1, float beta2, float eps, const float* hyper_dev,
                            int64_t* applied_dev, float* max_radii, float* grad_norm_accum, float* counts, const float* sh_jac,
                            float max_ratio, float lambda);

int gs_pack_view_step(void* stream, int64_t n, float max_hw, const float* v_means, const float* v_scales,
                      const float* v_quats, const float* v_opacities, const int32_t* radii, const float* absgrad,
                      float* flat);

int gs_update_statistics(void* stream, int64_t n, float max_hw, const int32_t* radii, const float* absgrad,
                         float* max_radii, float* grad_norm_accum, float* counts);

#ifdef __cplusplus
}
#endif
#endif
```

Measured before the change: 745.3.

## Fold small helper kernels into neighbouring launches to cut launch count

Four launch-reduction ideas are bundled. Tile classification for the sort work lists moves into an extra block of the tile-scan kernel, so the tile path no longer launches class_items. The row-base scan computes its own prefix when chunk counts are small, dropping the single-block chunk scan. The loss reduction runs as an extra block of the SSIM backward kernel, and the fwd/bwd loss is exposed as one call. The first-unit checkpoint store is skipped and reads from row 0 instead. This trades redundant prefix work per block and racy ordering assumptions for fewer serial launches.

Result: no change. 751.8, median of 6 (+0.9%).

```diff
diff --git a/easy_gaussian_splatting_amd/csrc/gs_binning.hip b/easy_gaussian_splatting_amd/csrc/gs_binning.hip
--- a/easy_gaussian_splatting_amd/csrc/gs_binning.hip
+++ b/easy_gaussian_splatting_amd/csrc/gs_binning.hip
@@ -125,6 +125,18 @@
 }
 
 constexpr int kScanItems = 16;
+constexpr int kSegLen = 8192;
+constexpr int kSegMax = 8;
+
+__device__ __forceinline__ void class_item(int i, int n, int n_lists, int32_t* __restrict__ items, int32_t* __restrict__ counts) {
+    if (n > 1024 && n <= 4096) items[atomicAdd(&counts[0], 1)] = i;
+    else if (n > 4096 && n <= kSegLen) items[n_lists + atomicAdd(&counts[1], 1)] = i;
+    else if (n > kSegLen && n <= kSegLen * kSegMax) {
+        const int ns = (n + kSegLen - 1) / kSegLen;
+        const int p = atomicAdd(&counts[2], ns);
+        for (int sg = 0; sg < ns; ++sg) items[2 * n_lists + p + sg] = i * kSegMax + sg;
+    }
+}
 __global__ __launch_bounds__(kBinThreads) void bin_tilescan_kernel(
     int n_tiles_total, int n_groups_total, const uint32_t* __restrict__ tile_cnt,
     const uint32_t* __restrict__ grp_tot, int32_t* __restrict__ isect_offsets,
@@ -135,8 +147,16 @@
     __shared__ unsigned long long scratch[17];
     const int chunk = kBinThreads * kScanItems;
     if (round_idle(rblk, phase)) return;
+    if (blockIdx.x == 3) {
+        if (!sort_counts) return;
+        if (threadIdx.x < 64) sort_counts[threadIdx.x] = 0;
+        __threadfence();
+        __syncthreads();
+        for (int i = threadIdx.x; i < n_tiles_total; i += kBinThreads)
+            class_item(i, (int)tile_cnt[i], n_tiles_total, sort_counts + 64, sort_counts);
+        return;
+    }
     if (blockIdx.x == 2) {
-        if (sort_counts && threadIdx.x < 64) sort_counts[threadIdx.x] = 0;
         unsigned long long gcarry = 0;
         for (int base = 0; base < n_groups_total; base += kBinThreads) {
             const int i = base + threadIdx.x;
@@ -366,9 +386,6 @@
 };
 __device__ __forceinline__ bool sort_off(const SortArgs& a) { return guard_tripped(a.guard) || round_idle(a.rblk, a.phase); }
 
-constexpr int kSegLen = 8192;
-constexpr int kSegMax = 8;
-
 template <bool IN_LDS>
 __global__ void tile_sort_kernel(const SortArgs a) {
     extern __shared__ __attribute__((aligned(16))) unsigned long long skeys[];
@@ -544,14 +561,7 @@
     if (guard_tripped(guard) || round_idle(rblk, phase)) return;
     const int i = blockIdx.x * blockDim.x + threadIdx.x;
     if (i >= n_lists) return;
-    const int n = offsets[i + 1] - offsets[i];
-    if (n > 1024 && n <= 4096) items[atomicAdd(&counts[0], 1)] = i;
-    else if (n > 4096 && n <= kSegLen) items[n_lists + atomicAdd(&counts[1], 1)] = i;
-    else if (n > kSegLen && n <= kSegLen * kSegMax) {
-        const int ns = (n + kSegLen - 1) / kSegLen;
-        const int p = atomicAdd(&counts[2], ns);
-        for (int sg = 0; sg < ns; ++sg) items[2 * n_lists + p + sg] = i * kSegMax + sg;
-    }
+    class_item(i, offsets[i + 1] - offsets[i], n_lists, items, counts);
 }
 
 static size_t sort_items_bytes(int64_t n_lists) {
@@ -1035,7 +1045,7 @@
 
 #define GS_SORT1K_THREADS 256
 #define GS_SORT4K_THREADS 256
-static int launch_list_sorts(hipStream_t st, SortArgs& a, unsigned grid, int64_t max_tile_count, int32_t* items_ws) {
+static int launch_list_sorts(hipStream_t st, SortArgs& a, unsigned grid, int64_t max_tile_count, int32_t* items_ws, bool lists_built) {
     int lo_excl = 0;
     int32_t* counts = items_ws;
     int32_t* items = items_ws + 64;
@@ -1047,8 +1057,10 @@
         GS_LAUNCH_CHECK("tile_radix_sort_kernel");
     }
     if (max_tile_count <= 1024) return GS_OK;
-    hipLaunchKernelGGL(class_items_kernel, dim3((grid + 255) / 256), dim3(256), 0, st, (int)grid, a.isect_offsets, items, counts, a.guard, a.rblk, a.phase);
-    GS_LAUNCH_CHECK("class_items_kernel");
+    if (!lists_built) {
+        hipLaunchKernelGGL(class_items_kernel, dim3((grid + 255) / 256), dim3(256), 0, st, (int)grid, a.isect_offsets, items, counts, a.guard, a.rblk, a.phase);
+        GS_LAUNCH_CHECK("class_items_kernel");
+    }
     {
         a.lo_excl = 1024; a.hi_incl = 4096;
         const size_t lds_k = 2 * sizeof(uint64_t) * 4096 + radix_lds * (GS_SORT4K_THREADS / 64);
@@ -1121,7 +1133,7 @@
     GS_LAUNCH_CHECK("bin_colscan_kernel");
     const Guard gd = current_guard();
     GS_REQUIRE(gd.info == nullptr || gd.info == info_dev, "the guard set by gs_guard_set must be this call's info_dev");
-    hipLaunchKernelGGL(bin_tilescan_kernel, dim3(3), dim3(kBinThreads), 0, st, (int)ct, C * L.groups, tile_cnt,
+    hipLaunchKernelGGL(bin_tilescan_kernel, dim3(4), dim3(kBinThreads), 0, st, (int)ct, C * L.groups, tile_cnt,
                        grp_tot, isect_offsets, bucket_offsets, grp_base, info_dev, tile_order, gd.cap_isects, gd.cap_tile,
                        (int64_t)0, (int32_t*)(ws + L.items_off), current_info_mirror(), gd.per_call, rblk, phase);
     GS_LAUNCH_CHECK("bin_tilescan_kernel");
@@ -1170,7 +1182,7 @@
     a.guard = current_guard().info;
     a.coarse = 0; a.seg = 0; a.merged = nullptr; a.rblk = rblk; a.phase = phase;
     static_assert(2 + kSegMax == 10, "bin_layout sizes the work lists for kSegMax == 8");
-    return launch_list_sorts(st, a, (unsigned)(C * tiles), max_tile_count, (int32_t*)(ws + L.items_off));
+    return launch_list_sorts(st, a, (unsigned)(C * tiles), max_tile_count, (int32_t*)(ws + L.items_off), true);
 }
 
 extern "C" size_t gs_bins_workspace_bytes(int C, int64_t N, int tile_w, int tile_h, int bin_shift, int64_t coarse_cap) {
@@ -1264,7 +1276,7 @@
         a.isect_ids = nullptr; a.flatten_ids = nullptr; a.slots = nullptr;
         a.guard = info_dev; a.coarse = 1; a.seg = 0; a.rblk = rblk; a.phase = phase;
         a.merged = (unsigned long long*)(ws + L.staged_off);
-        if (int rc = launch_list_sorts(st, a, (unsigned)cb, list_cap < coarse_cap ? list_cap : coarse_cap, (int32_t*)(ws + L.items_off))) return rc;
+        if (int rc = launch_list_sorts(st, a, (unsigned)cb, list_cap < coarse_cap ? list_cap : coarse_cap, (int32_t*)(ws + L.items_off), false)) return rc;
     }
     RefineArgs r;
     fill_refine_args(r, L, C, tile_w, tile_h, ws, coarse_keys, bbox, info_dev);
diff --git a/easy_gaussian_splatting_amd/csrc/gs_blend.hip b/easy_gaussian_splatting_amd/csrc/gs_blend.hip
--- a/easy_gaussian_splatting_amd/csrc/gs_blend.hip
+++ b/easy_gaussian_splatting_amd/csrc/gs_blend.hip
@@ -289,8 +289,10 @@
                                 }
                                 const int su = pool_next++;
                                 --pool_left;
-                                a.ckpt[(size_t)su * 64 + lane] = make_float4(px_live(T[k]) ? T[k] : -1.f, cr[k], cg[k], cb[k]);
-                                if constexpr (NC == 4) ckpt_ext[(size_t)su * 64 + lane] = ca[k];
+                                if (pos != 0) {
+                                    a.ckpt[(size_t)su * 64 + lane] = make_float4(px_live(T[k]) ? T[k] : -1.f, cr[k], cg[k], cb[k]);
+                                    if constexpr (NC == 4) ckpt_ext[(size_t)su * 64 + lane] = ca[k];
+                                }
                                 if (lane == 0) ulog[log_n] = make_int2(su, (pos / kUnit) * 4 + k);
                                 ++log_n;
                                 if (lane == 0) uring[4 * k + ((pos / kUnit) & 3)] = su;
@@ -379,6 +381,7 @@
     blend_fwd_body<CKPT, WAVES, 0, NC>(a, ckpt_ext);
 }
 
+constexpr int kSelfPrefixChunks = 1024;
 struct RowScanArgs {
     const uint8_t* qmask;
     int32_t* row_base;
@@ -422,6 +425,24 @@
     int32_t block_tot;
     block_excl_scan_add<int32_t>(tot, scratch, &block_tot);
     if (threadIdx.x == 0) a.walk[GS_WALK_WORDS + blockIdx.x] = block_tot;
+}
+
+__device__ __forceinline__ void row_scan_publish(const RowScanArgs& a, const int32_t total) {
+    int32_t fullest = 0;
+    for (int r = 0; r < GS_WALK_RANGES; ++r) fullest = max(fullest, a.walk[GS_WALK_RANGE0 + 32 * r]);
+    a.walk[kWalkStorage] = GS_WALK_RANGES * fullest;
+    a.walk[kWalkRows] = total;
+    int fl = a.walk[kWalkFlags];
+    if (a.flags && (fl & GS_FLAG_UNITS)) atomicOr(a.flags, (unsigned long long)GS_FLAG_UNITS);
+    if ((int64_t)total > a.cap_rows) {
+        fl |= GS_FLAG_ROWS;
+        a.walk[kWalkFlags] = fl;
+        if (a.flags) atomicOr(a.flags, (unsigned long long)GS_FLAG_ROWS);
+    }
+    if (a.mirror) {
+        a.mirror[0] = a.walk[kWalkUnits]; a.mirror[1] = a.walk[kWalkStorage]; a.mirror[2] = total; a.mirror[3] = fl;
+        __threadfence_system();
+    }
 }
 
 __global__ __launch_bounds__(1024) void row_chunk_scan_kernel(const RowScanArgs a) {
@@ -437,25 +458,10 @@
     int32_t total;
     int32_t run = block_excl_scan_add<int32_t>(mine, scratch, &total);
     for (int j = j0; j < j1; ++j) { const int32_t c = part[j]; part[j] = run; run += c; }
-    if (threadIdx.x == 0) {
-        int32_t fullest = 0;
-        for (int r = 0; r < GS_WALK_RANGES; ++r) fullest = max(fullest, a.walk[GS_WALK_RANGE0 + 32 * r]);
-        a.walk[kWalkStorage] = GS_WALK_RANGES * fullest;
-        a.walk[kWalkRows] = total;
-        int fl = a.walk[kWalkFlags];
-        if (a.flags && (fl & GS_FLAG_UNITS)) atomicOr(a.flags, (unsigned long long)GS_FLAG_UNITS);
-        if ((int64_t)total > a.cap_rows) {
-            fl |= GS_FLAG_ROWS;
-            a.walk[kWalkFlags] = fl;
-            if (a.flags) atomicOr(a.flags, (unsigned long long)GS_FLAG_ROWS);
-        }
-        if (a.mirror) {
-            a.mirror[0] = a.walk[kWalkUnits]; a.mirror[1] = a.walk[kWalkStorage]; a.mirror[2] = total; a.mirror[3] = fl;
-            __threadfence_system();
-        }
-    }
-}
-
+    if (threadIdx.x == 0) row_scan_publish(a, total);
+}
+
+template <bool SELF>
 __global__ __launch_bounds__(kScanThreads) void row_base_kernel(const RowScanArgs a) {
     __shared__ int32_t scratch[20];
     if (a.walk[kWalkSkip] != 0) return;
@@ -463,15 +469,25 @@
     const int64_t c0 = (int64_t)blockIdx.x * kScanChunk;
     if (c0 > n) return;
     const int64_t i0 = c0 + (int64_t)threadIdx.x * kScanPerThread;
+    const int32_t* part = a.walk + GS_WALK_WORDS;
+    int32_t before;
+    if (SELF) {
+        int32_t mine = 0;
+        for (int j = (int)threadIdx.x; j < (int)blockIdx.x; j += kScanThreads) mine += part[j];
+        block_excl_scan_add<int32_t>(mine, scratch, &before);
+    } else {
+        before = part[blockIdx.x];
+    }
     uint32_t w[8];
     const int32_t tot = row_counts32(a.qmask, i0, n, w);
     int32_t block_tot;
-    const int32_t run = block_excl_scan_add<int32_t>(tot, scratch, &block_tot) + a.walk[GS_WALK_WORDS + blockIdx.x];
+    const int32_t run = block_excl_scan_add<int32_t>(tot, scratch, &block_tot) + before;
     int32_t first16 = 0;
 #pragma unroll
     for (int j = 0; j < 4; ++j) first16 += (int32_t)((w[j] * 0x01010101u) >> 24);
     if (i0 <= n) a.row_base[i0 >> 4] = run;
     if (i0 + 16 <= n) a.row_base[(i0 >> 4) + 1] = run + first16;
+    if (SELF && threadIdx.x == 0 && (int64_t)blockIdx.x == n / kScanChunk) row_scan_publish(a, before + block_tot);
 }
 
 struct BlendBwdArgs {
@@ -561,7 +577,8 @@
     const int tyi = tt / a.tw, txi = tt - tyi * a.tw;
     const int qx0 = txi * GS_TILE + 8 * (q & 1), qy0 = tyi * GS_TILE + 8 * (q >> 1);
     const float fx0 = (float)qx0 + 0.5f, fy0 = (float)qy0 + 0.5f;
-    const float4* ckp = a.ckpt + (size_t)su * 64;
+    const size_t ck_row = first_unit ? (size_t)0 : (size_t)su * 64;
+    const float4* ckp = a.ckpt + ck_row;
 
     const int n_sub = valid ? a.qcnt[tq] : 0;
     int2 gs[E];
@@ -598,7 +615,7 @@
         l_cb[i] = NC > 2 ? a.out_colors[NC * o + 2] : 0.f;
         l_va[i] = vap[o];
         l_ck[i] = ckp[p];
-        if constexpr (NC == 4) { l_v3[i] = a.v_colors[NC * o + 3]; l_c3[i] = a.out_colors[NC * o + 3]; l_k3[i] = ckpt_ext[(size_t)su * 64 + p]; }
+        if constexpr (NC == 4) { l_v3[i] = a.v_colors[NC * o + 3]; l_c3[i] = a.out_colors[NC * o + 3]; l_k3[i] = ckpt_ext[ck_row + p]; }
     }
     const int n_in = min(kPipeLanes * E, n_sub - ud.y * kUnit);
     float4 rq[E][3];
@@ -863,8 +880,12 @@
         s.flags = a.flags; s.guard = a.guard; s.mirror = current_walk_mirror();
         const unsigned chunks = (unsigned)(n_isects / kScanChunk + 1);
         hipLaunchKernelGGL(row_count_kernel, dim3(chunks), dim3(kScanThreads), 0, st, s);
-        hipLaunchKernelGGL(row_chunk_scan_kernel, dim3(1), dim3(1024), 0, st, s);
-        hipLaunchKernelGGL(row_base_kernel, dim3(chunks), dim3(kScanThreads), 0, st, s);
+        if (chunks <= (unsigned)kSelfPrefixChunks) {
+            hipLaunchKernelGGL(row_base_kernel<true>, dim3(chunks), dim3(kScanThreads), 0, st, s);
+        } else {
+            hipLaunchKernelGGL(row_chunk_scan_kernel, dim3(1), dim3(1024), 0, st, s);
+            hipLaunchKernelGGL(row_base_kernel<false>, dim3(chunks), dim3(kScanThreads), 0, st, s);
+        }
         GS_LAUNCH_CHECK("row_base_kernel");
     } else {
         if constexpr (NC != 3) hipLaunchKernelGGL((chan_fwd_kernel<false, kFwdWaves, NC>), grid, block, 0, st, a, nullptr);
diff --git a/easy_gaussian_splatting_amd/csrc/gs_loss.hip b/easy_gaussian_splatting_amd/csrc/gs_loss.hip
--- a/easy_gaussian_splatting_amd/csrc/gs_loss.hip
+++ b/easy_gaussian_splatting_amd/csrc/gs_loss.hip
@@ -26,6 +26,8 @@
     float* partial;
     const float* gout;
     float* v_render;
+    int reduce_blocks;
+    float* out3;
 };
 
 __device__ __forceinline__ int clampi(int v, int lo, int hi) { return v < lo ? lo : (v > hi ? hi : v); }
@@ -198,9 +200,8 @@
     }
 }
 
-__global__ __launch_bounds__(256) void loss_reduce_kernel(int nblocks, const float* __restrict__ partial, int H, int W,
-                                                          float lambda_ssim, float* __restrict__ out) {
-    __shared__ double red[2][4];
+__device__ __forceinline__ void loss_reduce_block(int nblocks, const float* __restrict__ partial, int H, int W,
+                                                  float lambda_ssim, float* __restrict__ out, double (*red)[4]) {
     double s0 = 0.0, s1 = 0.0;
     for (int i = threadIdx.x; i < nblocks; i += 256) { s0 += partial[2 * i]; s1 += partial[2 * i + 1]; }
 #pragma unroll
@@ -216,9 +217,20 @@
     }
 }
 
+__global__ __launch_bounds__(256) void loss_reduce_kernel(int nblocks, const float* __restrict__ partial, int H, int W,
+                                                          float lambda_ssim, float* __restrict__ out) {
+    __shared__ double red[2][4];
+    loss_reduce_block(nblocks, partial, H, W, lambda_ssim, out, red);
+}
+
+template <bool REDUCE>
 __global__ __launch_bounds__(256) void l1_ssim_bwd_kernel(const LossArgs a) {
     constexpr float kWin[11] = GS_WIN_TAPS;
     extern __shared__ __attribute__((aligned(16))) float lds[];
+    if (REDUCE && blockIdx.x == gridDim.x - 1) {
+        loss_reduce_block(a.reduce_blocks, a.partial, a.H, a.W, a.lambda_ssim, a.out3, reinterpret_cast<double(*)[4]>(lds));
+        return;
+    }
     float* sm = lds;
     float* hp = lds;
     int x0, y0, ch;
@@ -372,7 +384,8 @@
 }
 
 static int loss_fwd_launch(void* stream, int height, int width, float lambda_ssim, const float* render, const float* gt,
-                           const float* mask, const float* const* slots, bool has_mask, int clamp_input, float* workspace, float* out3) {
+                           const float* mask, const float* const* slots, bool has_mask, int clamp_input, float* workspace, float* out3,
+                           bool reduce = true) {
     GS_REQUIRE(height > 2 * kHalo && width > 2 * kHalo, "image must be larger than the 11x11 window");
     GS_REQUIRE((int64_t)height * width <= kLossMaxPixels && width <= kLossMaxWidth && height <= (1 << 24),
                "image too large for the loss kernels' 32-bit byte offsets (H * W <= 2^28, W <= 2^20, H <= 2^24: row indices go through 24-bit multiplies)");
@@ -381,12 +394,14 @@
     a.H = height; a.W = width; a.lambda_ssim = lambda_ssim; a.render = render; a.gt = gt; a.mask = mask; a.slots = slots;
     a.clamp_input = clamp_input != 0;
     a.maps = workspace; a.partial = workspace + 9 * (size_t)height * width; a.gout = nullptr; a.v_render = nullptr;
+    a.reduce_blocks = 0; a.out3 = nullptr;
     const int blocks = (int)loss_grid(loss_tile_count(height, width)).x;
     const size_t lds = sizeof(float) * (2 * kLR * kLRP + 4 * kLR * kHP);
     hipStream_t st = (hipStream_t)stream;
     if (has_mask) hipLaunchKernelGGL(l1_ssim_fwd_kernel<true>, dim3((unsigned)blocks), dim3(256), lds, st, a);
     else hipLaunchKernelGGL(l1_ssim_fwd_kernel<false>, dim3((unsigned)blocks), dim3(256), lds, st, a);
     GS_LAUNCH_CHECK("l1_ssim_fwd_kernel");
+    if (!reduce) return GS_OK;
     hipLaunchKernelGGL(loss_reduce_kernel, dim3(1), dim3(256), 0, st, blocks, a.partial, height, width, lambda_ssim, out3);
     GS_LAUNCH_CHECK("loss_reduce_kernel");
     return GS_OK;
@@ -394,7 +409,7 @@
 
 static int loss_bwd_launch(void* stream, int height, int width, float lambda_ssim, const float* render, const float* gt,
                            const float* mask, const float* const* slots, int clamp_input, const float* workspace,
-                           const float* v_total, float* v_render) {
+                           const float* v_total, float* v_render, float* out3 = nullptr) {
     GS_REQUIRE(height > 2 * kHalo && width > 2 * kHalo, "image must be larger than the 11x11 window");
     GS_REQUIRE((int64_t)height * width <= kLossMaxPixels && width <= kLossMaxWidth && height <= (1 << 24),
                "image too large for the loss kernels' 32-bit byte offsets (H * W <= 2^28, W <= 2^20, H <= 2^24: row indices go through 24-bit multiplies)");
@@ -403,8 +418,15 @@
     a.H = height; a.W = width; a.lambda_ssim = lambda_ssim; a.render = render; a.gt = gt; a.mask = mask; a.slots = slots;
     a.clamp_input = clamp_input != 0;
     a.maps = const_cast<float*>(workspace); a.partial = nullptr; a.gout = v_total; a.v_render = v_render;
+    a.reduce_blocks = 0; a.out3 = out3;
     const size_t lds = sizeof(float) * (3 * kLR * kLRP);
-    hipLaunchKernelGGL(l1_ssim_bwd_kernel, dim3(3 * loss_grid(loss_tile_count(height, width)).x), dim3(256), lds, (hipStream_t)stream, a);
+    const unsigned fwd_blocks = loss_grid(loss_tile_count(height, width)).x;
+    if (out3) {
+        a.partial = const_cast<float*>(workspace) + 9 * (size_t)height * width; a.reduce_blocks = (int)fwd_blocks;
+        hipLaunchKernelGGL(l1_ssim_bwd_kernel<true>, dim3(3 * fwd_blocks + 1), dim3(256), lds, (hipStream_t)stream, a);
+    } else {
+        hipLaunchKernelGGL(l1_ssim_bwd_kernel<false>, dim3(3 * fwd_blocks), dim3(256), lds, (hipStream_t)stream, a);
+    }
     GS_LAUNCH_CHECK("l1_ssim_bwd_kernel");
     return GS_OK;
 }
@@ -432,3 +454,15 @@
     GS_REQUIRE(slots_dev != nullptr, "slots_dev is required");
     return loss_bwd_launch(stream, height, width, lambda_ssim, render, nullptr, nullptr, slots_dev, clamp_input, workspace, v_total, v_render);
 }
+
+extern "C" int gs_l1_ssim_fwd_bwd_slots(void* stream, int height, int width, float lambda_ssim, const float* render,
+                                        const float* const* slots_dev, int has_mask, int clamp_input, float* workspace,
+                                        float* out3, const float* v_total, float* v_render) {
+    GS_REQUIRE(slots_dev != nullptr, "slots_dev is required");
+    GS_REQUIRE(v_total && v_render && out3, "null pointer");
+    const int rc = loss_fwd_launch(stream, height, width, lambda_ssim, render, nullptr, nullptr, slots_dev, has_mask != 0, clamp_input,
+                                   workspace, out3, false);
+    if (rc != GS_OK) return rc;
+    return loss_bwd_launch(stream, height, width, lambda_ssim, render, nullptr, nullptr, slots_dev, clamp_input, workspace, v_total,
+                           v_render, out3);
+}
diff --git a/easy_gaussian_splatting_amd/train_graph.py b/easy_gaussian_splatting_amd/train_graph.py
--- a/easy_gaussian_splatting_amd/train_graph.py
+++ b/easy_gaussian_splatting_amd/train_graph.py
@@ -513,10 +513,8 @@
         try:
             self._enqueue_forward()
             lam = float(self.lc.lambda_ssim)
-            self._ck(L.gs_l1_ssim_fwd_slots(st, H, W, lam, _p(b["render_colors"]), _p(b["img_slots"]), int(self.has_mask), 1, _p(b["loss_ws"]),
-                                             _p(b["loss3"])), "gs_l1_ssim_fwd_slots")
-            self._ck(L.gs_l1_ssim_bwd_slots(st, H, W, lam, _p(b["render_colors"]), _p(b["img_slots"]), 1, _p(b["loss_ws"]),
-                                             _p(b["one"]), _p(b["v_render"])), "gs_l1_ssim_bwd_slots")
+            self._ck(L.gs_l1_ssim_fwd_bwd_slots(st, H, W, lam, _p(b["render_colors"]), _p(b["img_slots"]), int(self.has_mask), 1, _p(b["loss_ws"]),
+                                                 _p(b["loss3"]), _p(b["one"]), _p(b["v_render"])), "gs_l1_ssim_fwd_bwd_slots")
             if self.scale_reg and self.fuse_adam:
                 self._scale_reg(None)
             self._ck(L.gs_blend_bwd(st, 1, W, H, _p(b["rec"]), _p(b["qlist"]), _p(b["qcnt"]), _p(b["unit_desc"]), self.cap_units,
@@ -793,10 +791,8 @@
         try:
             self._enqueue_forward()
             lam = float(self.lc.lambda_ssim)
-            self._ck(L.gs_l1_ssim_fwd_slots(st, H, W, lam, _p(b["render_colors"]), _p(b["img_slots"]), int(self.has_mask), 1, _p(b["loss_ws"]),
-                                             _p(b["loss3"])), "gs_l1_ssim_fwd_slots")
-            self._ck(L.gs_l1_ssim_bwd_slots(st, H, W, lam, _p(b["render_colors"]), _p(b["img_slots"]), 1, _p(b["loss_ws"]),
-                                             _p(b["one"]), _p(b["v_render"])), "gs_l1_ssim_bwd_slots")
+            self._ck(L.gs_l1_ssim_fwd_bwd_slots(st, H, W, lam, _p(b["render_colors"]), _p(b["img_slots"]), int(self.has_mask), 1, _p(b["loss_ws"]),
+                                                 _p(b["loss3"]), _p(b["one"]), _p(b["v_render"])), "gs_l1_ssim_fwd_bwd_slots")
             self._ck(L.gs_blend_bwd(st, 1, W, H, _p(b["rec"]), _p(b["qlist"]), _p(b["qcnt"]), _p(b["unit_desc"]), self.cap_units,
                                      _p(b["ckpt"]), _p(b["qmask"]), _p(b["row_base"]), _p(b["walk_state"]),
                                      _p(b["render_colors"]), _p(b["render_alphas"]), _p(b["v_render"]), None, _p(b["rows"]), _p(b["unit_cls"])), "gs_blend_bwd")
diff --git a/include/gs_raster.h b/include/gs_raster.h
--- a/include/gs_raster.h
+++ b/include/gs_raster.h
@@ -239,6 +239,9 @@
 int gs_l1_ssim_bwd_slots(void* stream, int height, int width, float lambda_ssim, const float* render,
                          const float* const* slots_dev, int clamp_input, const float* workspace,
                          const float* v_total, float* v_render);
+int gs_l1_ssim_fwd_bwd_slots(void* stream, int height, int width, float lambda_ssim, const float* render,
+                             const float* const* slots_dev, int has_mask, int clamp_input, float* workspace,
+                             float* out3, const float* v_total, float* v_render);
 
 int gs_clamp01(void* stream, int64_t n, const float* x, const float* v_out, float* out);
 
```
